# TritonDataCenter/node-cueball

Hardware: AMD Instinct MI355X
Metric: pool claims/sec (8-backend synthetic TCP set) (higher is better)
Workload: dtype n/a; 1 GPU; model=ConnectionPool claim/release (config: headline), global_batch=20000, seq_len=1, parallelism=1 worker processes (event loops), backends=8, spares=8, maximum=16, concurrency=16

## Files before the change

cueball_amd/_native/speed.cpp:

```cpp

#define PY_SSIZE_T_CLEAN
#include <Python.h>
#include <structmember.h>
#include <cmath>
#include <cstring>
#include <ctime>

#include "lathist.h"

#ifndef CUEBALL_HANDLE_HOOKS
#define CUEBALL_HANDLE_HOOKS 1
#endif
#ifndef CUEBALL_SLOT_HOOKS
#define CUEBALL_SLOT_HOOKS 1
#endif
#ifndef CUEBALL_LAZY_SCOPES
#define CUEBALL_LAZY_SCOPES 1
#endif
#ifndef CUEBALL_VECTORCALL
#define CUEBALL_VECTORCALL 1
#endif
#if !defined(Py_TPFLAGS_HAVE_VECTORCALL) && defined(_Py_TPFLAGS_HAVE_VECTORCALL)
#define Py_TPFLAGS_HAVE_VECTORCALL _Py_TPFLAGS_HAVE_VECTORCALL
#endif

namespace {

PyObject *s_stateChanged;
PyObject *s_listener;
PyObject *s_on;
PyObject *s_remove_listener;
PyObject *s_call_soon;
PyObject *s_call_later;
PyObject *s_cancel;
PyObject *s_state_prefix;
PyObject *s_dot;
PyObject *s_underscore;
PyObject *s_flush_name;
PyObject *s_internal;
PyObject *s_is_closed;

PyObject *g_get_loop;
PyObject *g_fsm_error;
PyObject *g_entry_name_cache;
PyObject *g_flush_batches;
PyObject *g_tracer;
PyObject *g_remove_desc;

static inline PyObject *
resolve_loop(PyObject *loop)
{
    if (loop != NULL && loop != Py_None) {
        Py_INCREF(loop);
        return loop;
    }
    return PyObject_CallOneArg(g_get_loop, Py_None);
}


typedef struct {
    PyObject_HEAD
    PyObject *ev_events;
    PyObject *ev_dict;
    PyObject *ev_weakrefs;
    unsigned long ev_gen;
    unsigned long ev_lk_gen;
    long ev_lk_cnt[4];
    Py_ssize_t ev_lk_len[4];
    int ev_lk_ok;
} Emitter;

extern PyTypeObject EmitterType;
extern PyTypeObject ConnErrCbType;
extern PyTypeObject KitCbType;

static inline int
listener_is_own_internal(PyObject *listener)
{
    PyTypeObject *tp = Py_TYPE(listener);
    return tp == &ConnErrCbType || tp == &KitCbType;
}

#define SMALL_LIST_KEEP 8

static inline int
list_append_keep(PyObject *ls, PyObject *item)
{
    PyListObject *l = (PyListObject *)ls;
    Py_ssize_t n = Py_SIZE(l);
    if (n < l->allocated) {
        Py_INCREF(item);
        l->ob_item[n] = item;
        Py_SET_SIZE(l, n + 1);
        return 0;
    }
    return PyList_Append(ls, item);
}

static inline int
list_remove_at_keep(PyObject *ls, Py_ssize_t i)
{
    PyListObject *l = (PyListObject *)ls;
    Py_ssize_t n = Py_SIZE(l);
    if (l->allocated > SMALL_LIST_KEEP)
        return PyList_SetSlice(ls, i, i + 1, NULL);
    PyObject *item = l->ob_item[i];
    for (Py_ssize_t j = i; j + 1 < n; j++)
        l->ob_item[j] = l->ob_item[j + 1];
    Py_SET_SIZE(l, n - 1);
    Py_DECREF(item);
    return 0;
}

int
Emitter_init(PyObject *self_, PyObject *args, PyObject *kwds)
{
    Emitter *self = (Emitter *)self_;
    (void)args; (void)kwds;
    if (self->ev_events == NULL) {
        self->ev_events = PyDict_New();
        if (self->ev_events == NULL)
            return -1;
    }
    return 0;
}

int
Emitter_traverse(PyObject *self_, visitproc visit, void *arg)
{
    Emitter *self = (Emitter *)self_;
    Py_VISIT(self->ev_events);
    Py_VISIT(self->ev_dict);
    return 0;
}

int
Emitter_clear_(PyObject *self_)
{
    Emitter *self = (Emitter *)self_;
    Py_CLEAR(self->ev_events);
    Py_CLEAR(self->ev_dict);
    return 0;
}

void
Emitter_dealloc(PyObject *self_)
{
    Emitter *self = (Emitter *)self_;
    PyTypeObject *tp = Py_TYPE(self_);
    PyObject_GC_UnTrack(self_);
    if (self->ev_weakrefs != NULL)
        PyObject_ClearWeakRefs(self_);
    Emitter_clear_(self_);
    tp->tp_free(self_);
}

PyObject *
emitter_add(Emitter *self, PyObject *event, PyObject *listener)
{
    if (self->ev_events == NULL) {
        self->ev_events = PyDict_New();
        if (self->ev_events == NULL)
            return NULL;
    }
    PyObject *ls = PyDict_GetItemWithError(self->ev_events, event);
    if (ls == NULL) {
        if (PyErr_Occurred())
            return NULL;
        ls = PyList_New(0);
        if (ls == NULL)
            return NULL;
        if (PyDict_SetItem(self->ev_events, event, ls) < 0) {
            Py_DECREF(ls);
// ... 670 lines not shown
PyObject *
Scope_dispose(PyObject *self_, PyObject *noargs)
{
    Scope *self = (Scope *)self_;
    (void)noargs;
    self->sc_active = 0;
    PyObject *regs[3 * SCOPE_INLINE_REGS];
    int nreg = self->sc_nreg;
    self->sc_nreg = 0;
    for (int i = 0; i < 3 * nreg; i++)
        regs[i] = self->sc_reg[i];
    PyObject *ls = self->sc_listeners;
    self->sc_listeners = NULL;
    int failed = 0;
    for (int i = 0; i < nreg; i++) {
        if (!failed &&
            scope_unregister(regs[3 * i], regs[3 * i + 1],
                             regs[3 * i + 2]) < 0)
            failed = 1;
        Py_DECREF(regs[3 * i]);
        Py_DECREF(regs[3 * i + 1]);
        Py_DECREF(regs[3 * i + 2]);
    }
    if (failed) {
        Py_XDECREF(ls);
        return NULL;
    }
    if (ls != NULL) {
        Py_ssize_t n = PyList_GET_SIZE(ls);
        for (Py_ssize_t i = 0; i + 2 < n; i += 3) {
            if (scope_unregister(PyList_GET_ITEM(ls, i),
                                 PyList_GET_ITEM(ls, i + 1),
                                 PyList_GET_ITEM(ls, i + 2)) < 0) {
                Py_DECREF(ls);
                return NULL;
            }
        }
        Py_DECREF(ls);
    }
    PyObject *ts = self->sc_timers;
    self->sc_timers = NULL;
    if (ts != NULL) {
        Py_ssize_t n = PyList_GET_SIZE(ts);
        for (Py_ssize_t i = 0; i < n; i++) {
            PyObject *r = PyObject_CallMethodObjArgs(
                PyList_GET_ITEM(ts, i), s_cancel, NULL);
            if (r == NULL) {
                Py_DECREF(ts);
                return NULL;
            }
            Py_DECREF(r);
        }
        Py_DECREF(ts);
    }
    Py_RETURN_NONE;
}

PyObject *
Scope_get_active(PyObject *self_, void *closure)
{
    (void)closure;
    return PyBool_FromLong(((Scope *)self_)->sc_active);
}

int
Scope_traverse(PyObject *self_, visitproc visit, void *arg)
{
    Scope *self = (Scope *)self_;
    Py_VISIT(self->sc_fsm);
    Py_VISIT(self->sc_listeners);
    Py_VISIT(self->sc_timers);
    for (int i = 0; i < 3 * self->sc_nreg; i++)
        Py_VISIT(self->sc_reg[i]);
    return 0;
}

int
Scope_clear_(PyObject *self_)
{
    Scope *self = (Scope *)self_;
    Py_CLEAR(self->sc_fsm);
    Py_CLEAR(self->sc_listeners);
    Py_CLEAR(self->sc_timers);
    int nreg = self->sc_nreg;
    self->sc_nreg = 0;
    for (int i = 0; i < 3 * nreg; i++)
        Py_CLEAR(self->sc_reg[i]);
    return 0;
}

void
Scope_dealloc(PyObject *self_)
{
    PyObject_GC_UnTrack(self_);
    Scope_clear_(self_);
    if (scope_freelist_n < SCOPE_FREELIST_MAX)
        scope_freelist[scope_freelist_n++] = (Scope *)self_;
    else
        PyObject_GC_Del(self_);
}

PyMethodDef Scope_methods[] = {
    {"on", (PyCFunction)(void (*)(void))Scope_on, METH_FASTCALL, NULL},
    {"timeout", (PyCFunction)(void (*)(void))Scope_timeout, METH_FASTCALL,
     NULL},
    {"interval", (PyCFunction)(void (*)(void))Scope_interval,
     METH_FASTCALL, NULL},
    {"immediate", Scope_immediate, METH_O, NULL},
    {"callback", Scope_callback, METH_O, NULL},
    {"valid_transitions", Scope_valid_transitions, METH_O, NULL},
    {"goto_state", Scope_goto_state, METH_O, NULL},
    {"_dispose", Scope_dispose, METH_NOARGS, NULL},
    {NULL, NULL, 0, NULL},
};

PyGetSetDef Scope_getset[] = {
    {(char *)"active", Scope_get_active, NULL, NULL, NULL},
    {NULL, NULL, NULL, NULL, NULL},
};

PyTypeObject ScopeType = {
    PyVarObject_HEAD_INIT(NULL, 0)
    "cueball_amd._speed.StateScope",
    sizeof(Scope),
    0,
    Scope_dealloc,
    0, 0, 0, 0, 0, 0, 0, 0, 0, 0, 0, 0, 0, 0,
    Py_TPFLAGS_DEFAULT | Py_TPFLAGS_HAVE_GC,
    "FSM state scope (native)",
    Scope_traverse,
    Scope_clear_,
    0, 0, 0, 0,
    Scope_methods,
    0,
    Scope_getset,
};


struct FSMOb {
    Emitter base;
    PyObject *f_loop;
    PyObject *f_state;
    PyObject *f_scope;
    PyObject *f_valid;
    PyObject *f_pending;
    PyObject **f_eq;
    Py_ssize_t f_eq_head, f_eq_len, f_eq_cap;
    PyObject *f_eq_inl[4];
    PyObject *f_hist[8];
    unsigned long f_hist_n;
    PyObject *f_flush_bound;
    PyObject *f_fastkit;
    PyObject *f_watchkit;
    int f_entering;
    int f_emit_scheduled;
};

int slotkit_maybe_entry(PyObject *kit_, FSMOb *fsm, PyObject *target);
int slotkit_smgr_hook(PyObject *kit_, PyObject *st, unsigned long serial);
unsigned long slotkit_slot_serial(PyObject *kit_);
int ch_emit_state_changed(FSMOb *self, PyObject *st);

static inline Scope *
fsm_need_scope(FSMOb *self)
{
    if (self->f_scope == NULL)
        self->f_scope = (PyObject *)scope_new((PyObject *)self);
    return (Scope *)self->f_scope;
}

extern PyObject *t_empty;
extern PyTypeObject CHType;
extern PyTypeObject CTType;
void ch_terminal_cleanup(FSMOb *self);

typedef PyObject *(*ch_entry_fn)(PyObject *, PyObject *);
ch_entry_fn ch_direct_entry(FSMOb *self, PyObject *target);

extern PyTypeObject FSMType;

PyObject *
fsm_get_loop_of(FSMOb *fsm)
{
    return fsm->f_loop;
}

#define FSM_EQ_INLINE 4
#define FSM_HISTORY 8

static void
fsm_eq_compact(FSMOb *f)
{
    if (f->f_eq_head == 0)
        return;
    Py_ssize_t n = f->f_eq_len - f->f_eq_head;
    memmove(f->f_eq, f->f_eq + f->f_eq_head, n * sizeof(PyObject *));
    f->f_eq_head = 0;
    f->f_eq_len = n;
}

static int
fsm_eq_push(FSMOb *f, PyObject *st)
{
    if (f->f_eq == NULL) {
        f->f_eq = f->f_eq_inl;
        f->f_eq_cap = FSM_EQ_INLINE;
        f->f_eq_head = f->f_eq_len = 0;
    }
    if (f->f_eq_len == f->f_eq_cap) {
        if (f->f_eq_head > 0) {
            fsm_eq_compact(f);
        } else {
            Py_ssize_t ncap = f->f_eq_cap * 2;
            PyObject **items;
            if (f->f_eq == f->f_eq_inl) {
                items = (PyObject **)PyMem_Malloc(
                    ncap * sizeof(PyObject *));
                if (items != NULL)
                    memcpy(items, f->f_eq_inl, sizeof(f->f_eq_inl));
            } else {
                items = (PyObject **)PyMem_Realloc(
                    f->f_eq, ncap * sizeof(PyObject *));
            }
            if (items == NULL) {
                PyErr_NoMemory();
                return -1;
            }
            f->f_eq = items;
            f->f_eq_cap = ncap;
        }
    }
    Py_INCREF(st);
    f->f_eq[f->f_eq_len++] = st;
    return 0;
}

static void
fsm_eq_clear(FSMOb *f)
{
    PyObject **items = f->f_eq;
    Py_ssize_t head = f->f_eq_head, len = f->f_eq_len;
    f->f_eq = NULL;
    f->f_eq_head = f->f_eq_len = f->f_eq_cap = 0;
    if (items == NULL)
        return;
    for (Py_ssize_t i = head; i < len; i++)
        Py_DECREF(items[i]);
    if (items != f->f_eq_inl)
        PyMem_Free(items);
}

int fsm_schedule_flush(FSMOb *self);

#define FSM_FLUSH_CAP 64

int
fsm_flush_core(FSMOb *self)
{
    self->f_emit_scheduled = 0;
    int n = 0;
    int is_handle = PyObject_TypeCheck((PyObject *)self, &CHType);
    while (self->f_eq_head < self->f_eq_len && n++ < FSM_FLUSH_CAP) {
        PyObject *st = self->f_eq[self->f_eq_head++];
        if (self->f_eq_head == self->f_eq_len)
            self->f_eq_head = self->f_eq_len = 0;
        int r;
        if (is_handle) {
            r = ch_emit_state_changed(self, st);
        } else {
            PyObject *eargs[2] = {s_stateChanged, st};
            unsigned long serial = self->f_watchkit == NULL ? 0
                : slotkit_slot_serial(self->f_watchkit);
            r = emitter_emit_core(&self->base, eargs[0], eargs + 1, 1);
            if (r >= 0 && serial != 0 && self->f_watchkit != NULL &&
                slotkit_smgr_hook(self->f_watchkit, st, serial) < 0)
                r = -1;
        }
        Py_DECREF(st);
        if (r < 0) {
            fsm_eq_compact(self);
            return -1;
        }
    }
    fsm_eq_compact(self);
    if (self->f_eq_len > 0 && !self->f_emit_scheduled)
        return fsm_schedule_flush(self);
    return 0;
}

PyObject *
FSM_flush_state_changed(PyObject *self_, PyObject *noargs)
{
    (void)noargs;
    if (fsm_flush_core((FSMOb *)self_) < 0)
        return NULL;
    Py_RETURN_NONE;
}

#define FLUSH_DRAIN_CAP 48

typedef struct {
    PyObject_HEAD
    PyObject *fb_loop;
    PyObject *fb_list;
    Py_ssize_t fb_pos;
    vectorcallfunc fb_vectorcall;
} FlushBatch;

extern PyTypeObject FlushBatchType;

static void
flushbatch_detach(FlushBatch *self)
{
    PyObject *cur = PyDict_GetItemWithError(g_flush_batches, self->fb_loop);
    if (cur == (PyObject *)self)
        (void)PyDict_DelItem(g_flush_batches, self->fb_loop);
    else if (cur == NULL)
        PyErr_Clear();
}

static PyObject *
flushbatch_run(PyObject *self_)
{
    FlushBatch *self = (FlushBatch *)self_;
    int rounds = 0;
    while (self->fb_pos < PyList_GET_SIZE(self->fb_list) &&
           rounds < FLUSH_DRAIN_CAP) {
        FSMOb *fsm = (FSMOb *)PyList_GET_ITEM(self->fb_list,
                                              self->fb_pos);
        self->fb_pos++;
        rounds++;
        if (fsm_flush_core(fsm) < 0) {
            for (Py_ssize_t i = self->fb_pos;
                 i < PyList_GET_SIZE(self->fb_list); i++) {
                FSMOb *f = (FSMOb *)PyList_GET_ITEM(self->fb_list, i);
                f->f_emit_scheduled = 0;
            }
            flushbatch_detach(self);
            return NULL;
        }
    }
    if (self->fb_pos < PyList_GET_SIZE(self->fb_list)) {
        if (PyList_SetSlice(self->fb_list, 0, self->fb_pos, NULL) < 0) {
            flushbatch_detach(self);
            return NULL;
        }
        self->fb_pos = 0;
        PyObject *h = PyObject_CallMethodObjArgs(
            self->fb_loop, s_call_soon, self_, NULL);
        if (h == NULL) {
            flushbatch_detach(self);
            return NULL;
        }
        Py_DECREF(h);
        Py_RETURN_NONE;
    }
    flushbatch_detach(self);
    Py_RETURN_NONE;
}

PyObject *
FlushBatch_call(PyObject *self_, PyObject *args, PyObject *kwds)
{
    (void)args; (void)kwds;
    return flushbatch_run(self_);
}

static PyObject *
FlushBatch_vectorcall(PyObject *self_, PyObject *const *args, size_t nargsf,
                      PyObject *kwnames)
{
    (void)args; (void)nargsf; (void)kwnames;
    return flushbatch_run(self_);
}

int
FlushBatch_traverse(PyObject *self_, visitproc visit, void *arg)
{
    FlushBatch *self = (FlushBatch *)self_;
    Py_VISIT(self->fb_loop);
    Py_VISIT(self->fb_list);
    return 0;
}

int
FlushBatch_clear_(PyObject *self_)
{
    FlushBatch *self = (FlushBatch *)self_;
    Py_CLEAR(self->fb_loop);
    Py_CLEAR(self->fb_list);
    return 0;
}

void
FlushBatch_dealloc(PyObject *self_)
{
    PyObject_GC_UnTrack(self_);
    FlushBatch_clear_(self_);
    PyObject_GC_Del(self_);
}

PyTypeObject FlushBatchType = {
    PyVarObject_HEAD_INIT(NULL, 0)
    "cueball_amd._speed._FlushBatch",
    sizeof(FlushBatch),
    0,
    FlushBatch_dealloc,
    0, 0, 0, 0, 0, 0, 0, 0, 0,
    FlushBatch_call,
    0, 0, 0, 0,
    Py_TPFLAGS_DEFAULT | Py_TPFLAGS_HAVE_GC,
    0,
    FlushBatch_traverse,
    FlushBatch_clear_,
};

int
fsm_queue_state_changed(FSMOb *self, PyObject *state)
{
    if (fsm_eq_push(self, state) < 0)
        return -1;
    return fsm_schedule_flush(self);
}

int
fsm_schedule_flush(FSMOb *self)
{
    if (self->f_emit_scheduled)
        return 0;
    self->f_emit_scheduled = 1;
    PyObject *batch = PyDict_GetItemWithError(g_flush_batches, self->f_loop);
    if (batch == NULL) {
        if (PyErr_Occurred())
            return -1;
        FlushBatch *fb = PyObject_GC_New(FlushBatch, &FlushBatchType);
        if (fb == NULL)
            return -1;
        Py_INCREF(self->f_loop);
        fb->fb_loop = self->f_loop;
        fb->fb_pos = 0;
        fb->fb_vectorcall = FlushBatch_vectorcall;
        fb->fb_list = PyList_New(0);
        PyObject_GC_Track((PyObject *)fb);
        if (fb->fb_list == NULL) {
            Py_DECREF(fb);
            return -1;
        }
        if (PyDict_SetItem(g_flush_batches, self->f_loop,
                           (PyObject *)fb) < 0) {
            Py_DECREF(fb);
            return -1;
        }
        PyObject *h = PyObject_CallMethodObjArgs(
            self->f_loop, s_call_soon, (PyObject *)fb, NULL);
        if (h == NULL) {
            Py_DECREF(fb);
            return -1;
        }
        Py_DECREF(h);
        batch = (PyObject *)fb;
        Py_DECREF(fb);
    }
    if (PyList_Append(((FlushBatch *)batch)->fb_list,
                      (PyObject *)self) < 0)
        return -1;
    return 0;
}

PyObject *
entry_attr_name(PyObject *state)
{
    PyObject *name = PyDict_GetItemWithError(g_entry_name_cache, state);
    if (name != NULL) {
        Py_INCREF(name);
        return name;
    }
    if (PyErr_Occurred())
        return NULL;
    PyObject *replaced = PyObject_CallMethod(state, "replace", "OO",
                                             s_dot, s_underscore);
    if (replaced == NULL)
        return NULL;
    name = PyUnicode_Concat(s_state_prefix, replaced);
    Py_DECREF(replaced);
    if (name == NULL)
        return NULL;
    PyUnicode_InternInPlace(&name);
    if (PyDict_SetItem(g_entry_name_cache, state, name) < 0) {
        Py_DECREF(name);
        return NULL;
    }
    return name;
}

int
check_valid(FSMOb *self, PyObject *from, PyObject *state)
{
    if (self->f_valid == NULL)
        return 0;
    int c = PySequence_Contains(self->f_valid, state);
    if (c < 0)
        return -1;
    if (!c) {
        PyErr_Format(g_fsm_error,
                     "%s: invalid transition %R -> %R (valid: %R)",
                     Py_TYPE(self)->tp_name,
                     from ? from : Py_None, state, self->f_valid);
        return -1;
    }
    return 0;
}

int
fsm_enter_loop(FSMOb *self, PyObject *state)
{
    PyObject *next_state = state;
    Py_INCREF(next_state);
    while (next_state != NULL) {
        PyObject *target = next_state;
        next_state = NULL;
        if (self->f_scope != NULL) {
            PyObject *old = self->f_scope;
            self->f_scope = NULL;
            PyObject *r = Scope_dispose(old, NULL);
            Py_DECREF(old);
            if (r == NULL) {
                Py_DECREF(target);
                return -1;
            }
            Py_DECREF(r);
        }
        Py_CLEAR(self->f_valid);
        Py_INCREF(target);
        Py_XSETREF(self->f_state, target);
        Py_INCREF(target);
        Py_XSETREF(self->f_hist[self->f_hist_n % FSM_HISTORY], target);
        self->f_hist_n++;
#if !CUEBALL_LAZY_SCOPES
        if (fsm_need_scope(self) == NULL) {
            Py_DECREF(target);
            return -1;
        }
#endif

        if (g_tracer != NULL && g_tracer != Py_None) {
            PyObject *targs[2] = {(PyObject *)self, target};
            PyObject *tr = PyObject_Vectorcall(g_tracer, targs, 2, NULL);
            if (tr == NULL) {
                Py_DECREF(target);
                return -1;
            }
            Py_DECREF(tr);
        }

        int handled = 0;
        if (self->f_fastkit != NULL) {
            self->f_entering = 1;
            handled = slotkit_maybe_entry(self->f_fastkit, self, target);
            self->f_entering = 0;
            if (handled < 0) {
                Py_DECREF(target);
                return -1;
            }
        }
        PyObject *r;
        ch_entry_fn direct = handled ? NULL : ch_direct_entry(self, target);
        if (handled) {
            r = Py_None;
            Py_INCREF(r);
        } else if (direct != NULL) {
            self->f_entering = 1;
            r = direct((PyObject *)self, NULL);
            self->f_entering = 0;
        } else {
            PyObject *attr = entry_attr_name(target);
            if (attr == NULL) {
                Py_DECREF(target);
                return -1;
            }
            PyObject *entry = PyObject_GetAttr((PyObject *)self, attr);
            Py_DECREF(attr);
            if (entry == NULL) {
                PyErr_Clear();
                PyErr_Format(g_fsm_error,
                             "%s has no state-entry function for %R",
                             Py_TYPE(self)->tp_name, target);
                Py_DECREF(target);
                return -1;
            }
            PyObject *scope = (PyObject *)fsm_need_scope(self);
            if (scope == NULL) {
                Py_DECREF(entry);
                Py_DECREF(target);
                return -1;
            }
            Py_INCREF(scope);
            self->f_entering = 1;
            r = PyObject_CallOneArg(entry, scope);
            Py_DECREF(entry);
            Py_DECREF(scope);
            self->f_entering = 0;
        }
        PyObject *pend = self->f_pending;
        self->f_pending = NULL;
        if (r == NULL) {
            Py_XDECREF(pend);
            Py_DECREF(target);
            return -1;
        }
        Py_DECREF(r);
        if (fsm_queue_state_changed(self, target) < 0) {
            Py_XDECREF(pend);
            Py_DECREF(target);
            return -1;
        }
        if (pend != NULL) {
            if (check_valid(self, target, pend) < 0) {
                Py_DECREF(pend);
                Py_DECREF(target);
                return -1;
            }
            next_state = pend;
        }
        Py_DECREF(target);
    }
    if (self->f_valid == t_empty &&
        PyObject_TypeCheck((PyObject *)self, &CHType))
        ch_terminal_cleanup(self);
    return 0;
}

int
fsm_goto_state(FSMOb *self, PyObject *state)
{
    if (check_valid(self, self->f_state, state) < 0)
        return -1;
    if (self->f_entering) {
        if (self->f_pending != NULL) {
            int eq = PyObject_RichCompareBool(self->f_pending, state, Py_EQ);
            if (eq < 0)
                return -1;
            if (!eq) {
                PyErr_Format(g_fsm_error,
                             "%s: conflicting deferred transitions %R and "
                             "%R from %R", Py_TYPE(self)->tp_name,
                             self->f_pending, state,
                             self->f_state ? self->f_state : Py_None);
                return -1;
            }
            return 0;
        }
        Py_INCREF(state);
        self->f_pending = state;
        return 0;
    }
    return fsm_enter_loop(self, state);
}

int
FSM_init(PyObject *self_, PyObject *args, PyObject *kwds)
{
    FSMOb *self = (FSMOb *)self_;
    PyObject *initial = NULL, *loop = Py_None;
    static const char *kwlist[] = {"initial_state", "loop", NULL};
    if (!PyArg_ParseTupleAndKeywords(args, kwds, "U|O",
                                     const_cast<char **>(kwlist),
                                     &initial, &loop))
        return -1;
    if (Emitter_init(self_, NULL, NULL) < 0)
        return -1;
    PyObject *resolved = resolve_loop(loop);
    if (resolved == NULL)
        return -1;
    Py_XSETREF(self->f_loop, resolved);
    Py_CLEAR(self->f_state);
    Py_CLEAR(self->f_valid);
    Py_CLEAR(self->f_pending);
    self->f_entering = 0;
    return fsm_goto_state(self, initial);
}

PyObject *
FSM_get_state(PyObject *self_, PyObject *noargs)
{
    FSMOb *self = (FSMOb *)self_;
    (void)noargs;
    if (self->f_state == NULL) {
        PyErr_SetString(g_fsm_error, "FSM has no state yet");
        return NULL;
    }
    Py_INCREF(self->f_state);
    return self->f_state;
}

PyObject *
FSM_is_in_state(PyObject *self_, PyObject *state)
{
    FSMOb *self = (FSMOb *)self_;
    if (self->f_state == NULL)
        Py_RETURN_FALSE;
    int eq = PyUnicode_Compare(self->f_state, state);
    if (eq == -1 && PyErr_Occurred())
        return NULL;
    if (eq == 0)
        Py_RETURN_TRUE;
    Py_ssize_t sl = PyUnicode_GET_LENGTH(state);
    Py_ssize_t cl = PyUnicode_GET_LENGTH(self->f_state);
    if (cl > sl) {
        int m = PyUnicode_Tailmatch(self->f_state, state, 0, sl, -1);
        if (m < 0)
            return NULL;
        if (m && PyUnicode_ReadChar(self->f_state, sl) == '.')
            Py_RETURN_TRUE;
    }
    Py_RETURN_FALSE;
}

PyObject *
FSM_get_state_history(PyObject *self_, PyObject *noargs)
{
    FSMOb *self = (FSMOb *)self_;
    (void)noargs;
    Py_ssize_t count = self->f_hist_n < FSM_HISTORY
        ? (Py_ssize_t)self->f_hist_n : FSM_HISTORY;
    PyObject *out = PyList_New(count);
    if (out == NULL)
        return NULL;
    unsigned long first = self->f_hist_n - (unsigned long)count;
    for (Py_ssize_t i = 0; i < count; i++) {
        PyObject *st = self->f_hist[(first + (unsigned long)i) %
                                    FSM_HISTORY];
        Py_INCREF(st);
        PyList_SET_ITEM(out, i, st);
    }
    return out;
}

PyObject *
FSM_goto_state_py(PyObject *self_, PyObject *state)
{
    if (!PyUnicode_Check(state)) {
        PyErr_SetString(PyExc_TypeError, "state must be a str");
        return NULL;
    }
    if (fsm_goto_state((FSMOb *)self_, state) < 0)
        return NULL;
    Py_RETURN_NONE;
}

PyObject *
FSM_get__fsm_state(PyObject *self_, void *closure)
{
    FSMOb *self = (FSMOb *)self_;
    (void)closure;
    if (self->f_state == NULL)
        Py_RETURN_NONE;
    Py_INCREF(self->f_state);
    return self->f_state;
}

PyObject *
FSM_get__fsm_valid(PyObject *self_, void *closure)
{
    FSMOb *self = (FSMOb *)self_;
    (void)closure;
    if (self->f_valid == NULL)
        Py_RETURN_NONE;
    Py_INCREF(self->f_valid);
    return self->f_valid;
}

int
FSM_set__fsm_valid(PyObject *self_, PyObject *value, void *closure)
{
    FSMOb *self = (FSMOb *)self_;
    (void)closure;
    if (value == NULL || value == Py_None) {
        Py_CLEAR(self->f_valid);
        return 0;
    }
// ... 22 lines not shown
} IntervalOb;

extern PyTypeObject IntervalType;

PyObject *
Interval_call(PyObject *self_, PyObject *args, PyObject *kwds)
{
    IntervalOb *self = (IntervalOb *)self_;
    (void)args; (void)kwds;
    if (self->iv_stopped || !((Scope *)self->iv_scope)->sc_active)
        Py_RETURN_NONE;
    PyObject *r = PyObject_CallNoArgs(self->iv_cb);
    if (r == NULL)
        return NULL;
    Py_DECREF(r);
    if (!self->iv_stopped && ((Scope *)self->iv_scope)->sc_active) {
        FSMOb *fsm = (FSMOb *)((Scope *)self->iv_scope)->sc_fsm;
        PyObject *h = PyObject_CallMethodObjArgs(
            fsm->f_loop, s_call_later, self->iv_secs, self_, NULL);
        if (h == NULL)
            return NULL;
        Py_XSETREF(self->iv_handle, h);
    }
    Py_RETURN_NONE;
}

PyObject *
Interval_cancel(PyObject *self_, PyObject *noargs)
{
    IntervalOb *self = (IntervalOb *)self_;
    (void)noargs;
    self->iv_stopped = 1;
    if (self->iv_handle != NULL) {
        PyObject *r = PyObject_CallMethodObjArgs(self->iv_handle, s_cancel,
                                                 NULL);
        if (r == NULL)
            return NULL;
        Py_DECREF(r);
    }
    Py_RETURN_NONE;
}

int
Interval_traverse(PyObject *self_, visitproc visit, void *arg)
{
    IntervalOb *self = (IntervalOb *)self_;
    Py_VISIT(self->iv_scope);
    Py_VISIT(self->iv_cb);
    Py_VISIT(self->iv_handle);
    return 0;
}

int
Interval_clear_(PyObject *self_)
{
    IntervalOb *self = (IntervalOb *)self_;
    Py_CLEAR(self->iv_scope);
    Py_CLEAR(self->iv_cb);
    Py_CLEAR(self->iv_secs);
    Py_CLEAR(self->iv_handle);
    return 0;
}

void
Interval_dealloc(PyObject *self_)
{
    PyObject_GC_UnTrack(self_);
    Interval_clear_(self_);
    PyObject_GC_Del(self_);
}

PyMethodDef Interval_methods[] = {
    {"cancel", Interval_cancel, METH_NOARGS, NULL},
    {NULL, NULL, 0, NULL},
};

PyTypeObject IntervalType = {
    PyVarObject_HEAD_INIT(NULL, 0)
    "cueball_amd._speed._Interval",
    sizeof(IntervalOb),
    0,
    Interval_dealloc,
    0, 0, 0, 0, 0, 0, 0, 0, 0,
    Interval_call,
    0, 0, 0, 0,
    Py_TPFLAGS_DEFAULT | Py_TPFLAGS_HAVE_GC,
    0,
    Interval_traverse,
    Interval_clear_,
    0, 0, 0, 0,
    Interval_methods,
};

PyObject *
Scope_interval(PyObject *self_, PyObject *const *args, Py_ssize_t nargs)
{
    Scope *self = (Scope *)self_;
    if (nargs != 2) {
        PyErr_SetString(PyExc_TypeError, "S.interval(ms, cb)");
        return NULL;
    }
    if (scope_check_active(self, "S.interval()") < 0)
        return NULL;
    double ms = PyFloat_AsDouble(args[0]);
    if (ms == -1.0 && PyErr_Occurred())
        return NULL;
    IntervalOb *iv = PyObject_GC_New(IntervalOb, &IntervalType);
    if (iv == NULL)
        return NULL;
    Py_INCREF(self_);
    iv->iv_scope = self_;
    Py_INCREF(args[1]);
    iv->iv_cb = args[1];
    iv->iv_secs = PyFloat_FromDouble(ms / 1000.0);
    iv->iv_handle = NULL;
    iv->iv_stopped = 0;
    PyObject_GC_Track((PyObject *)iv);
    if (iv->iv_secs == NULL) {
        Py_DECREF(iv);
        return NULL;
    }
    FSMOb *fsm = (FSMOb *)self->sc_fsm;
    PyObject *h = PyObject_CallMethodObjArgs(fsm->f_loop, s_call_later,
                                             iv->iv_secs, (PyObject *)iv,
                                             NULL);
    if (h == NULL) {
        Py_DECREF(iv);
        return NULL;
    }
    iv->iv_handle = h;
    int rc = scope_add_timer(self, (PyObject *)iv);
    Py_DECREF(iv);
    if (rc < 0)
        return NULL;
    Py_RETURN_NONE;
}

int
FSM_traverse(PyObject *self_, visitproc visit, void *arg)
{
    FSMOb *self = (FSMOb *)self_;
    Py_VISIT(self->f_loop);
    Py_VISIT(self->f_state);
    Py_VISIT(self->f_scope);
    Py_VISIT(self->f_valid);
    Py_VISIT(self->f_pending);
    for (Py_ssize_t i = self->f_eq_head; i < self->f_eq_len; i++)
        Py_VISIT(self->f_eq[i]);
    for (int i = 0; i < FSM_HISTORY; i++)
        Py_VISIT(self->f_hist[i]);
    Py_VISIT(self->f_flush_bound);
    Py_VISIT(self->f_fastkit);
    Py_VISIT(self->f_watchkit);
    return Emitter_traverse(self_, visit, arg);
}

int
FSM_clear_(PyObject *self_)
{
    FSMOb *self = (FSMOb *)self_;
    Py_CLEAR(self->f_loop);
    Py_CLEAR(self->f_state);
    Py_CLEAR(self->f_scope);
    Py_CLEAR(self->f_valid);
    Py_CLEAR(self->f_pending);
    fsm_eq_clear(self);
    for (int i = 0; i < FSM_HISTORY; i++)
        Py_CLEAR(self->f_hist[i]);
    self->f_hist_n = 0;
    Py_CLEAR(self->f_flush_bound);
    Py_CLEAR(self->f_fastkit);
    Py_CLEAR(self->f_watchkit);
    return Emitter_clear_(self_);
}

void
FSM_dealloc(PyObject *self_)
{
    FSMOb *self = (FSMOb *)self_;
    PyTypeObject *tp = Py_TYPE(self_);
    PyObject_GC_UnTrack(self_);
    if (self->base.ev_weakrefs != NULL)
        PyObject_ClearWeakRefs(self_);
    FSM_clear_(self_);
    tp->tp_free(self_);
}

static PyObject *
FSM_set_fast_kit(PyObject *self_, PyObject *kit)
{
    FSMOb *self = (FSMOb *)self_;
    if (kit == Py_None) {
        Py_CLEAR(self->f_fastkit);
    } else {
        Py_INCREF(kit);
        Py_XSETREF(self->f_fastkit, kit);
    }
    Py_RETURN_NONE;
}

PyMethodDef FSM_methods[] = {
    {"get_state", FSM_get_state, METH_NOARGS, NULL},
    {"is_in_state", FSM_is_in_state, METH_O, NULL},
    {"get_state_history", FSM_get_state_history, METH_NOARGS, NULL},
    {"goto_state", FSM_goto_state_py, METH_O, NULL},
    {"_flush_state_changed", FSM_flush_state_changed, METH_NOARGS, NULL},
    {"_set_fast_kit", FSM_set_fast_kit, METH_O, NULL},
    {NULL, NULL, 0, NULL},
};

PyMemberDef FSM_members[] = {
    {(char *)"_loop", T_OBJECT, offsetof(FSMOb, f_loop), READONLY, NULL},
    {NULL, 0, 0, 0, NULL},
};

PyGetSetDef FSM_getset[] = {
    {(char *)"_fsm_state", FSM_get__fsm_state, NULL, NULL, NULL},
    {(char *)"_fsm_valid", FSM_get__fsm_valid, FSM_set__fsm_valid, NULL,
     NULL},
    {NULL, NULL, NULL, NULL, NULL},
};

PyTypeObject FSMType = {
    PyVarObject_HEAD_INIT(NULL, 0)
    "cueball_amd._speed.FSM",
    sizeof(FSMOb),
    0,
    FSM_dealloc,
    0, 0, 0, 0, 0, 0, 0, 0, 0, 0, 0, 0, 0, 0,
    Py_TPFLAGS_DEFAULT | Py_TPFLAGS_BASETYPE | Py_TPFLAGS_HAVE_GC,
    "Moore machine (native)",
    FSM_traverse,
    FSM_clear_,
    0, 0, 0, 0,
    FSM_methods,
    FSM_members,
    FSM_getset,
    &EmitterType,
    0, 0, 0,
    0,
    FSM_init,
    0,
    PyType_GenericNew,
};


typedef struct {
    FSMOb base;
    PyObject *sl_handle;
    PyObject *sl_prev_handle;
    PyObject *sl_wanted;
    PyObject *sl_monitor;
    PyObject *sl_idleq_node;
    PyObject *sl_initq_node;
} SlotOb;

extern PyTypeObject SlotBaseType;

static inline int
slot_field_set(PyObject **field)
{
    return *field != NULL && *field != Py_None;
}

static inline int
slot_field_true(PyObject **field)
{
    PyObject *v = *field;
    if (v == Py_True)
        return 1;
    if (v == NULL || v == Py_False || v == Py_None)
        return 0;
    Py_INCREF(v);
    int t = PyObject_IsTrue(v);
    Py_DECREF(v);
    return t;
}

static inline void
slot_field_store(PyObject **field, PyObject *value)
{
    Py_XINCREF(value);
    Py_XSETREF(*field, value);
}

int
Slot_traverse(PyObject *self_, visitproc visit, void *arg)
{
    SlotOb *self = (SlotOb *)self_;
    Py_VISIT(self->sl_handle);
    Py_VISIT(self->sl_prev_handle);
    Py_VISIT(self->sl_wanted);
    Py_VISIT(self->sl_monitor);
    Py_VISIT(self->sl_idleq_node);
    Py_VISIT(self->sl_initq_node);
    return FSM_traverse(self_, visit, arg);
}

int
Slot_clear_(PyObject *self_)
{
    SlotOb *self = (SlotOb *)self_;
    Py_CLEAR(self->sl_handle);
    Py_CLEAR(self->sl_prev_handle);
    Py_CLEAR(self->sl_wanted);
    Py_CLEAR(self->sl_monitor);
    Py_CLEAR(self->sl_idleq_node);
    Py_CLEAR(self->sl_initq_node);
    return FSM_clear_(self_);
}

void
Slot_dealloc(PyObject *self_)
{
    SlotOb *self = (SlotOb *)self_;
    PyTypeObject *tp = Py_TYPE(self_);
    PyObject_GC_UnTrack(self_);
    if (self->base.base.ev_weakrefs != NULL)
        PyObject_ClearWeakRefs(self_);
    Slot_clear_(self_);
    tp->tp_free(self_);
}

PyMemberDef Slot_members[] = {
    {(char *)"csf_handle", T_OBJECT, offsetof(SlotOb, sl_handle), 0, NULL},
    {(char *)"csf_prev_handle", T_OBJECT, offsetof(SlotOb, sl_prev_handle),
     0, NULL},
    {(char *)"csf_wanted", T_OBJECT, offsetof(SlotOb, sl_wanted), 0, NULL},
    {(char *)"csf_monitor", T_OBJECT, offsetof(SlotOb, sl_monitor), 0,
     NULL},
    {(char *)"p_idleq_node", T_OBJECT, offsetof(SlotOb, sl_idleq_node), 0,
     NULL},
    {(char *)"p_initq_node", T_OBJECT, offsetof(SlotOb, sl_initq_node), 0,
     NULL},
    {NULL, 0, 0, 0, NULL},
};

PyTypeObject SlotBaseType = {
    PyVarObject_HEAD_INIT(NULL, 0)
    "cueball_amd._speed.SlotBase",
    sizeof(SlotOb),
    0,
    Slot_dealloc,
    0, 0, 0, 0, 0, 0, 0, 0, 0, 0, 0, 0, 0, 0,
    Py_TPFLAGS_DEFAULT | Py_TPFLAGS_BASETYPE | Py_TPFLAGS_HAVE_GC,
    "connection slot FSM (native fields)",
    Slot_traverse,
    Slot_clear_,
    0, 0, 0, 0,
    0,
    Slot_members,
    0,
    &FSMType,
    0, 0, 0,
    0,
    0,
    0,
    PyType_GenericNew,
};



typedef struct {
    PyObject_HEAD
    lathist::Hist h;
} LatHistOb;

extern PyTypeObject LatHistType;

static PyObject *
LatHist_new(PyTypeObject *type, PyObject *args, PyObject *kwds)
{
// ... 228 lines not shown
{
#if defined(CLOCK_MONOTONIC)
    if (pl->pl_direct) {
        struct timespec ts;
        if (clock_gettime(CLOCK_MONOTONIC, &ts) == 0)
            return (double)ts.tv_sec * 1000.0 + (double)ts.tv_nsec * 1e-6;
    }
#endif
    PyObject *t = PyObject_CallMethodObjArgs(pl->pl_loop, s_time, NULL);
    if (t == NULL) {
        *err = 1;
        return 0.0;
    }
    double secs = PyFloat_AsDouble(t);
    Py_DECREF(t);
    if (secs == -1.0 && PyErr_Occurred()) {
        *err = 1;
        return 0.0;
    }
    return secs * 1000.0;
}

static PyObject *
PoolLat_new(PyTypeObject *type, PyObject *args, PyObject *kwds)
{
    PyObject *loop;
    int direct = 0;
    static const char *kwlist[] = {"loop", "direct", NULL};
    if (!PyArg_ParseTupleAndKeywords(args, kwds, "O|p",
                                     const_cast<char **>(kwlist),
                                     &loop, &direct))
        return NULL;
    PoolLatOb *self = PyObject_GC_New(PoolLatOb, type);
    if (self == NULL)
        return NULL;
    Py_INCREF(loop);
    self->pl_loop = loop;
#if defined(CLOCK_MONOTONIC)
    self->pl_direct = direct;
#else
    self->pl_direct = 0;
#endif
    self->pl_wait = (LatHistOb *)LatHist_new(&LatHistType, NULL, NULL);
    self->pl_hold = (LatHistOb *)LatHist_new(&LatHistType, NULL, NULL);
    self->pl_connect = (LatHistOb *)LatHist_new(&LatHistType, NULL, NULL);
    PyObject_GC_Track((PyObject *)self);
    if (self->pl_wait == NULL || self->pl_hold == NULL ||
        self->pl_connect == NULL) {
        Py_DECREF((PyObject *)self);
        return NULL;
    }
    return (PyObject *)self;
}

static int
PoolLat_traverse(PyObject *self_, visitproc visit, void *arg)
{
    Py_VISIT(((PoolLatOb *)self_)->pl_loop);
    return 0;
}

static int
PoolLat_clear_(PyObject *self_)
{
    Py_CLEAR(((PoolLatOb *)self_)->pl_loop);
    return 0;
}

static void
PoolLat_dealloc(PyObject *self_)
{
    PoolLatOb *self = (PoolLatOb *)self_;
    PyObject_GC_UnTrack(self_);
    Py_CLEAR(self->pl_loop);
    Py_CLEAR(self->pl_wait);
    Py_CLEAR(self->pl_hold);
    Py_CLEAR(self->pl_connect);
    PyObject_GC_Del(self_);
}

static PyMemberDef PoolLat_members[] = {
    {(char *)"loop", T_OBJECT, offsetof(PoolLatOb, pl_loop), READONLY,
     NULL},
    {(char *)"wait", T_OBJECT, offsetof(PoolLatOb, pl_wait), READONLY,
     NULL},
    {(char *)"hold", T_OBJECT, offsetof(PoolLatOb, pl_hold), READONLY,
     NULL},
    {(char *)"connect", T_OBJECT, offsetof(PoolLatOb, pl_connect),
     READONLY, NULL},
    {(char *)"direct", T_INT, offsetof(PoolLatOb, pl_direct), READONLY,
     NULL},
    {NULL, 0, 0, 0, NULL},
};

PyTypeObject PoolLatType = {
    PyVarObject_HEAD_INIT(NULL, 0)
    "cueball_amd._speed.PoolLatency",
    sizeof(PoolLatOb),
};

static void
latency_types_init(void)
{
    LatHistType.tp_flags = Py_TPFLAGS_DEFAULT;
    LatHistType.tp_methods = LatHist_methods;
    LatHistType.tp_getset = LatHist_getset;
    LatHistType.tp_new = LatHist_new;

    PoolLatType.tp_dealloc = PoolLat_dealloc;
    PoolLatType.tp_flags = Py_TPFLAGS_DEFAULT | Py_TPFLAGS_HAVE_GC;
    PoolLatType.tp_traverse = PoolLat_traverse;
    PoolLatType.tp_clear = PoolLat_clear_;
    PoolLatType.tp_members = PoolLat_members;
    PoolLatType.tp_new = PoolLat_new;
}


PyObject *g_err_claim_timeout;
PyObject *g_err_cueball;
PyObject *g_err_misused;
PyObject *g_capture_stack;

PyObject *s_claim;
PyObject *s_warn;
PyObject *s_incr;
PyObject *s_claim_timeout_evt;
PyObject *s_is_in_state;
PyObject *s_time;
PyObject *s_waiting, *s_claiming, *s_claimed, *s_released, *s_closed,
         *s_cancelled, *s_failed, *s_idle, *s_error_evt;
PyObject *t_waiting_valid;
PyObject *t_claiming_valid;
PyObject *t_claimed_valid;
PyObject *t_empty;
PyObject *s_leak_events[4];

int g_stack_on = 1;
PyObject *g_stack_placeholder;
PyObject *g_inf;

static inline PyObject *
capture_stack(void)
{
    if (!g_stack_on && g_stack_placeholder != NULL) {
        Py_INCREF(g_stack_placeholder);
        return g_stack_placeholder;
    }
    return PyObject_CallNoArgs(g_capture_stack);
}

extern PyObject *s_busy_st;
PyObject *slotkit_conn_err_cb(PyObject *slot, PyObject *handle);

typedef struct {
    FSMOb base;
    PyObject *chb_pool;
    PyObject *chb_claim_stack;
    PyObject *chb_callback;
    PyObject *chb_log;
    PyObject *chb_slot;
    PyObject *chb_release_stack;
    PyObject *chb_connection;
    PyObject *chb_last_error;
    PyObject *chb_waiter_node;
    PoolLatOb *chb_lat;
    double chb_claim_timeout;
    double chb_started;
    double chb_claimed_at;
    long chb_pre[4];
    int chb_have_pre;
    int chb_throw_error;
    int chb_cancelled;
    int chb_leak_check;
    int chb_pinger;
    int chb_lat_open;
    PyObject *chb_idleq, *chb_waiters, *chb_initq;
    int chb_tk_on;
    int chb_tk_err_on_empty;
    unsigned long chb_bk_serial;
    Py_ssize_t chb_bk_pos;
} CHOb;

extern PyTypeObject CHType;

long
c_count_listeners(PyObject *emitter, PyObject *event)
{
    if (!PyObject_TypeCheck(emitter, &EmitterType))
        return -2;
    Emitter *em = (Emitter *)emitter;
    if (em->ev_events == NULL)
        return 0;
    PyObject *ls = PyDict_GetItemWithError(em->ev_events, event);
    if (ls == NULL)
        return PyErr_Occurred() ? -1 : 0;
    long count = 0;
    Py_ssize_t n = PyList_GET_SIZE(ls);
    for (Py_ssize_t i = 0; i < n; i++) {
        PyObject *h = PyList_GET_ITEM(ls, i);
        if (!PyCallable_Check(h))
            continue;
        PyObject *marker = NULL;
        if (_PyObject_LookupAttr(h, s_internal, &marker) < 0)
            return -1;
        if (marker != NULL) {
            int truthy = PyObject_IsTrue(marker);
            Py_DECREF(marker);
            if (truthy < 0)
                return -1;
            if (truthy)
                continue;
        }
        PyObject *target = NULL;
        if (Py_TYPE(h) == &OnceWrapperType) {
            target = ((OnceWrapper *)h)->ow_listener;
            Py_INCREF(target);
        } else if (_PyObject_LookupAttr(h, s_listener, &target) < 0) {
            return -1;
        }
        if (target != NULL && target != h) {
            if (_PyObject_LookupAttr(target, s_internal, &marker) < 0) {
                Py_DECREF(target);
                return -1;
            }
            if (marker != NULL) {
                int truthy = PyObject_IsTrue(marker);
                Py_DECREF(marker);
                if (truthy < 0) {
                    Py_DECREF(target);
                    return -1;
                }
                if (truthy) {
                    Py_DECREF(target);
                    continue;
                }
            }
        }
        Py_XDECREF(target);
        count++;
    }
    return count;
}

int
emitter_leak_counts(PyObject *conn, long out[4])
{
    if (!PyObject_TypeCheck(conn, &EmitterType))
        return -2;
    Emitter *em = (Emitter *)conn;
    Py_ssize_t lens[4];
    for (int i = 0; i < 4; i++) {
        PyObject *ls = NULL;
        if (em->ev_events != NULL) {
            ls = PyDict_GetItemWithError(em->ev_events, s_leak_events[i]);
            if (ls == NULL && PyErr_Occurred())
                return -1;
        }
        lens[i] = (ls != NULL && PyList_Check(ls)) ? PyList_GET_SIZE(ls)
                                                   : -1;
    }
    if (em->ev_lk_ok && em->ev_lk_gen == em->ev_gen &&
        memcmp(lens, em->ev_lk_len, sizeof(lens)) == 0) {
        memcpy(out, em->ev_lk_cnt, sizeof(em->ev_lk_cnt));
        return 0;
    }
    unsigned long gen = em->ev_gen;
    for (int i = 0; i < 4; i++) {
        long c = c_count_listeners(conn, s_leak_events[i]);
        if (c < 0)
            return -1;
        out[i] = c;
    }
    em->ev_lk_ok = 0;
    if (gen == em->ev_gen) {
        memcpy(em->ev_lk_cnt, out, sizeof(em->ev_lk_cnt));
        memcpy(em->ev_lk_len, lens, sizeof(lens));
        em->ev_lk_gen = gen;
        em->ev_lk_ok = 1;
    }
    return 0;
}

typedef struct {
    PyObject_HEAD
    PyObject *ce_handle;
} ConnErrCb;

extern PyTypeObject ConnErrCbType;

PyObject *conn_err_fire(CHOb *h, PyObject *err);

PyObject *
ConnErrCb_call(PyObject *self_, PyObject *args, PyObject *kwds)
{
    CHOb *h = (CHOb *)((ConnErrCb *)self_)->ce_handle;
    (void)kwds;
    PyObject *err = (PyTuple_GET_SIZE(args) > 0)
        ? PyTuple_GET_ITEM(args, 0) : Py_None;
    return conn_err_fire(h, err);
}

PyObject *
conn_err_fire(CHOb *h, PyObject *err)
{
    long cnt = c_count_listeners(h->chb_connection, s_error_evt);
    if (cnt == -1)
        return NULL;
    if (cnt == 0 && h->chb_throw_error) {
        if (PyExceptionInstance_Check(err)) {
            PyErr_SetObject((PyObject *)Py_TYPE(err), err);
        } else {
            PyErr_SetObject(PyExc_RuntimeError, err);
        }
        return NULL;
    }
    PyObject *msg = PyUnicode_FromString(
        "connection emitted error while claimed");
    if (msg == NULL)
        return NULL;
    PyObject *r = PyObject_CallMethodObjArgs(h->chb_log, s_warn, msg,
                                             NULL);
    Py_DECREF(msg);
    if (r == NULL)
        return NULL;
    Py_DECREF(r);
    PyObject *evt = PyUnicode_FromString("error-while-claimed");
    if (evt == NULL)
        return NULL;
    r = PyObject_CallMethodObjArgs(h->chb_pool, s_incr, evt, NULL);
    Py_DECREF(evt);
    if (r == NULL)
        return NULL;
    Py_DECREF(r);
    Py_RETURN_NONE;
}

int
ConnErrCb_traverse(PyObject *self_, visitproc visit, void *arg)
{
    Py_VISIT(((ConnErrCb *)self_)->ce_handle);
    return 0;
}

int
ConnErrCb_clear_(PyObject *self_)
{
    Py_CLEAR(((ConnErrCb *)self_)->ce_handle);
    return 0;
}

void
ConnErrCb_dealloc(PyObject *self_)
{
    PyObject_GC_UnTrack(self_);
    ConnErrCb_clear_(self_);
    PyObject_GC_Del(self_);
}

PyObject *
ConnErrCb_get_internal(PyObject *self_, void *closure)
{
    (void)self_; (void)closure;
    Py_RETURN_TRUE;
}

PyGetSetDef ConnErrCb_getset[] = {
    {(char *)"_cueball_internal", ConnErrCb_get_internal, NULL, NULL, NULL},
    {NULL, NULL, NULL, NULL, NULL},
};

PyTypeObject ConnErrCbType = {
    PyVarObject_HEAD_INIT(NULL, 0)
    "cueball_amd._speed._ConnErrCb",
    sizeof(ConnErrCb),
    0,
    ConnErrCb_dealloc,
    0, 0, 0, 0, 0, 0, 0, 0, 0,
    ConnErrCb_call,
    0, 0, 0, 0,
    Py_TPFLAGS_DEFAULT | Py_TPFLAGS_HAVE_GC,
    0,
    ConnErrCb_traverse,
    ConnErrCb_clear_,
    0, 0, 0, 0, 0, 0,
    ConnErrCb_getset,
};

typedef struct {
    PyObject_HEAD
    PyObject *fc_handle;
} FailCb;

extern PyTypeObject FailCbType;

PyObject *
FailCb_call(PyObject *self_, PyObject *args, PyObject *kwds)
{
    CHOb *h = (CHOb *)((FailCb *)self_)->fc_handle;
    (void)args; (void)kwds;
    PyObject *err = h->chb_last_error ? h->chb_last_error : Py_None;
    return PyObject_CallOneArg(h->chb_callback, err);
}

int
FailCb_traverse(PyObject *self_, visitproc visit, void *arg)
{
    Py_VISIT(((FailCb *)self_)->fc_handle);
    return 0;
}

int
FailCb_clear_(PyObject *self_)
{
    Py_CLEAR(((FailCb *)self_)->fc_handle);
    return 0;
}

void
FailCb_dealloc(PyObject *self_)
{
    PyObject_GC_UnTrack(self_);
    FailCb_clear_(self_);
    PyObject_GC_Del(self_);
}

PyTypeObject FailCbType = {
    PyVarObject_HEAD_INIT(NULL, 0)
    "cueball_amd._speed._FailCb",
    sizeof(FailCb),
    0,
    FailCb_dealloc,
    0, 0, 0, 0, 0, 0, 0, 0, 0,
    FailCb_call,
    0, 0, 0, 0,
    Py_TPFLAGS_DEFAULT | Py_TPFLAGS_HAVE_GC,
    0,
    FailCb_traverse,
    FailCb_clear_,
};


int
ch_state_is(CHOb *self, PyObject *state)
{
    return self->base.f_state == state ||
        (self->base.f_state != NULL &&
         PyUnicode_Compare(self->base.f_state, state) == 0);
}

PyObject *
ch_err_format(PyObject *cls, const char *msg)
{
    PyErr_SetString(cls, msg);
    return NULL;
}


PyObject *
CH_try_(PyObject *self_, PyObject *slot)
{
    CHOb *self = (CHOb *)self_;
    if (!ch_state_is(self, s_waiting))
        return ch_err_format(g_fsm_error,
            "ClaimHandle.try_ only in \"waiting\"");
    PyObject *r = PyObject_CallMethodObjArgs(slot, s_is_in_state, s_idle,
                                             NULL);
    if (r == NULL)
        return NULL;
    int idle = PyObject_IsTrue(r);
    Py_DECREF(r);
    if (!idle)
        return ch_err_format(g_fsm_error,
            "ClaimHandle.try_ needs an idle slot");
// ... 50 lines not shown
ch_do_claim_timeout(CHOb *self)
{
    PyObject *err = PyObject_CallOneArg(g_err_claim_timeout,
                                        self->chb_pool);
    if (err == NULL)
        return -1;
    Py_XSETREF(self->chb_last_error, err);
    PyObject *r = PyObject_CallMethodObjArgs(
        self->chb_pool, s_incr, s_claim_timeout_evt, NULL);
    if (r == NULL)
        return -1;
    Py_DECREF(r);
    return fsm_goto_state(&self->base, s_failed);
}

PyObject *
CH_timeout(PyObject *self_, PyObject *noargs)
{
    CHOb *self = (CHOb *)self_;
    (void)noargs;
    if (!ch_state_is(self, s_waiting))
        return ch_err_format(g_fsm_error, "timeout only in waiting");
    if (ch_do_claim_timeout(self) < 0)
        return NULL;
    Py_RETURN_NONE;
}

PyObject *
CH__on_claim_timeout(PyObject *self_, PyObject *noargs)
{
    return CH_timeout(self_, noargs);
}

PyObject *
CH_fail(PyObject *self_, PyObject *err)
{
    CHOb *self = (CHOb *)self_;
    if (ch_state_is(self, s_waiting)) {
        Py_INCREF(err);
        Py_XSETREF(self->chb_last_error, err);
        if (fsm_goto_state(&self->base, s_failed) < 0)
            return NULL;
    }
    Py_RETURN_NONE;
}

int
ch_relinquish(CHOb *self, PyObject *target_state)
{
    if (!ch_state_is(self, s_claimed)) {
        if (ch_state_is(self, s_released) || ch_state_is(self, s_closed)) {
            PyObject *by = NULL;
            PyObject *stack = self->chb_release_stack;
            if (stack != NULL && PyList_Check(stack) &&
                PyList_GET_SIZE(stack) >= 1) {
                by = PyList_GET_ITEM(stack, PyList_GET_SIZE(stack) - 1);
            }
            PyObject *msg = PyUnicode_FromFormat(
                "Connection not claimed by this handle, released by %S",
                by ? by : Py_None);
            if (msg == NULL)
                return -1;
            PyObject *err = PyObject_CallOneArg(g_err_cueball, msg);
            Py_DECREF(msg);
            if (err == NULL)
                return -1;
            PyErr_SetObject(g_err_cueball, err);
            Py_DECREF(err);
            return -1;
        }
        PyObject *msg = PyUnicode_FromFormat(
            "ClaimHandle.release() called while in state \"%S\"",
            self->base.f_state ? self->base.f_state : Py_None);
        if (msg == NULL)
            return -1;
        PyErr_SetObject(g_err_cueball, msg);
        Py_DECREF(msg);
        return -1;
    }
    PyObject *stack = capture_stack();
    if (stack == NULL)
        return -1;
    Py_XSETREF(self->chb_release_stack, stack);
    return fsm_goto_state(&self->base, target_state);
}

PyObject *
CH_release(PyObject *self_, PyObject *noargs)
{
    (void)noargs;
    if (ch_relinquish((CHOb *)self_, s_released) < 0)
        return NULL;
    Py_RETURN_NONE;
}

PyObject *
CH_close(PyObject *self_, PyObject *noargs)
{
    (void)noargs;
    if (ch_relinquish((CHOb *)self_, s_closed) < 0)
        return NULL;
    Py_RETURN_NONE;
}

PyObject *
CH_disable_release_leak_check(PyObject *self_, PyObject *noargs)
{
    (void)noargs;
    ((CHOb *)self_)->chb_leak_check = 0;
    Py_RETURN_NONE;
}


PyObject *
CH_state_waiting(PyObject *self_, PyObject *scope)
{
    CHOb *self = (CHOb *)self_;
    Py_INCREF(t_waiting_valid);
    Py_XSETREF(self->base.f_valid, t_waiting_valid);
    Py_CLEAR(self->chb_slot);
    self->chb_bk_serial = 0;
    if (isfinite(self->chb_claim_timeout)) {
        if (scope == NULL)
            scope = (PyObject *)fsm_need_scope(&self->base);
        if (scope == NULL)
            return NULL;
        PyObject *ms = PyFloat_FromDouble(self->chb_claim_timeout);
        if (ms == NULL)
            return NULL;
        PyObject *cb = PyObject_GetAttrString(self_, "_on_claim_timeout");
        if (cb == NULL) {
            Py_DECREF(ms);
            return NULL;
        }
        PyObject *args[2] = {ms, cb};
        PyObject *r = Scope_timeout(scope, args, 2);
        Py_DECREF(ms);
        Py_DECREF(cb);
        if (r == NULL)
            return NULL;
        Py_DECREF(r);
    }
    Py_RETURN_NONE;
}

PyObject *
CH_state_claiming(PyObject *self_, PyObject *scope)
{
    CHOb *self = (CHOb *)self_;
    (void)scope;
    Py_INCREF(t_claiming_valid);
    Py_XSETREF(self->base.f_valid, t_claiming_valid);
    PyObject *slot = self->chb_slot;
    if (slot != NULL && PyObject_TypeCheck(slot, &SlotBaseType) &&
        ((FSMOb *)slot)->f_fastkit != NULL) {
        FSMOb *sf = (FSMOb *)slot;
        PyObject *fs = sf->f_state;
        if (!(fs == s_idle ||
              (fs != NULL && PyUnicode_Compare(fs, s_idle) == 0))) {
            PyErr_SetString(g_fsm_error, "claim only in idle");
            return NULL;
        }
        if (slot_field_set(&((SlotOb *)slot)->sl_handle)) {
            PyErr_SetString(g_fsm_error, "slot already has a handle");
            return NULL;
        }
        slot_field_store(&((SlotOb *)slot)->sl_handle, self_);
        if (fsm_goto_state(sf, s_busy_st) < 0)
            return NULL;
        Py_RETURN_NONE;
    }
    PyObject *r = PyObject_CallMethodObjArgs(slot, s_claim,
                                             self_, NULL);
    if (r == NULL)
        return NULL;
    Py_DECREF(r);
    Py_RETURN_NONE;
}

PyObject *
CH_state_claimed(PyObject *self_, PyObject *scope)
{
    CHOb *self = (CHOb *)self_;
    Py_INCREF(t_claimed_valid);
    Py_XSETREF(self->base.f_valid, t_claimed_valid);

    if (self->chb_cancelled) {
        if (fsm_goto_state(&self->base, s_released) < 0)
            return NULL;
        Py_RETURN_NONE;
    }

    PyObject *conn = self->chb_connection;
    int lk = emitter_leak_counts(conn, self->chb_pre);
    if (lk == -1)
        return NULL;
    if (lk == -2)
        self->chb_pre[0] = self->chb_pre[1] = self->chb_pre[2] =
            self->chb_pre[3] = 0;
    self->chb_have_pre = 1;

    PyObject *ec = slotkit_conn_err_cb(self->chb_slot, self_);
    if (ec != NULL) {
        Py_INCREF(ec);
    } else {
        ConnErrCb *nec = PyObject_GC_New(ConnErrCb, &ConnErrCbType);
        if (nec == NULL)
            return NULL;
        Py_INCREF(self_);
        nec->ce_handle = self_;
        PyObject_GC_Track((PyObject *)nec);
        ec = (PyObject *)nec;
    }
    if (scope == NULL)
        scope = (PyObject *)fsm_need_scope(&self->base);
    if (scope == NULL) {
        Py_DECREF(ec);
        return NULL;
    }
    PyObject *args[3] = {conn, s_error_evt, ec};
    PyObject *r = Scope_on(scope, args, 3);
    Py_DECREF(ec);
    if (r == NULL)
        return NULL;
    Py_DECREF(r);

    if (self->chb_lat != NULL && !self->chb_pinger) {
        int err = 0;
        double now = poollat_now_ms(self->chb_lat, &err);
        if (err)
            return NULL;
        self->chb_lat->pl_wait->h.record_ms(now - self->chb_started);
        self->chb_claimed_at = now;
        self->chb_lat_open = 1;
    }

    PyObject *cbargs[3] = {Py_None, self_, conn};
    r = PyObject_Vectorcall(self->chb_callback, cbargs, 3, NULL);
    if (r == NULL)
        return NULL;
    Py_DECREF(r);
    Py_RETURN_NONE;
}

static int
ch_record_hold(CHOb *self)
{
    if (!self->chb_lat_open)
        return 0;
    self->chb_lat_open = 0;
    int err = 0;
    double now = poollat_now_ms(self->chb_lat, &err);
    if (err)
        return -1;
    self->chb_lat->pl_hold->h.record_ms(now - self->chb_claimed_at);
    return 0;
}

PyObject *
CH_state_released(PyObject *self_, PyObject *scope)
{
    CHOb *self = (CHOb *)self_;
    (void)scope;
    Py_INCREF(t_empty);
    Py_XSETREF(self->base.f_valid, t_empty);
    if (ch_record_hold(self) < 0)
        return NULL;
    if (!self->chb_leak_check || !self->chb_have_pre)
        Py_RETURN_NONE;
    PyObject *conn = self->chb_connection;
    long after[4];
    int lk = emitter_leak_counts(conn, after);
    if (lk == -1)
        return NULL;
    if (lk == -2)
        Py_RETURN_NONE;
    for (int i = 0; i < 4; i++) {
        long c = after[i];
        if (c > self->chb_pre[i]) {
            PyObject *msg = PyUnicode_FromFormat(
                "connection claimer looks like it leaked event handlers "
                "(event=%S before=%ld after=%ld)",
                s_leak_events[i], self->chb_pre[i], c);
            if (msg == NULL)
                return NULL;
            PyObject *r = PyObject_CallMethodObjArgs(self->chb_log, s_warn,
                                                     msg, NULL);
            Py_DECREF(msg);
            if (r == NULL)
                return NULL;
            Py_DECREF(r);
        }
    }
    Py_RETURN_NONE;
}

PyObject *
CH_state_closed(PyObject *self_, PyObject *scope)
{
    CHOb *self = (CHOb *)self_;
    (void)scope;
    Py_INCREF(t_empty);
    Py_XSETREF(self->base.f_valid, t_empty);
    if (ch_record_hold(self) < 0)
        return NULL;
    Py_RETURN_NONE;
}

PyObject *
CH_state_cancelled(PyObject *self_, PyObject *scope)
{
    CHOb *self = (CHOb *)self_;
    (void)scope;
    Py_INCREF(t_empty);
    Py_XSETREF(self->base.f_valid, t_empty);
    Py_RETURN_NONE;
}

PyObject *
CH_state_failed(PyObject *self_, PyObject *scope)
{
    CHOb *self = (CHOb *)self_;
    (void)scope;
    Py_INCREF(t_empty);
    Py_XSETREF(self->base.f_valid, t_empty);
    FailCb *fc = PyObject_GC_New(FailCb, &FailCbType);
    if (fc == NULL)
        return NULL;
    Py_INCREF(self_);
    fc->fc_handle = self_;
    PyObject_GC_Track((PyObject *)fc);
    PyObject *h = PyObject_CallMethodObjArgs(self->base.f_loop,
                                             s_call_soon,
                                             (PyObject *)fc, NULL);
    Py_DECREF(fc);
    if (h == NULL)
        return NULL;
    Py_DECREF(h);
    Py_RETURN_NONE;
}


PyObject *
CH_get_misused(PyObject *self_, void *closure)
{
    (void)self_; (void)closure;
    PyObject *err = PyObject_CallNoArgs(g_err_misused);
    if (err == NULL)
        return NULL;
    PyErr_SetObject(g_err_misused, err);
    Py_DECREF(err);
    return NULL;
}

PyObject *
CH_on(PyObject *self_, PyObject *const *args, Py_ssize_t nargs)
{
    if (nargs >= 1 && PyUnicode_Check(args[0])) {
        if (PyUnicode_CompareWithASCIIString(args[0], "readable") == 0 ||
            PyUnicode_CompareWithASCIIString(args[0], "close") == 0) {
            PyObject *err = PyObject_CallNoArgs(g_err_misused);
            if (err == NULL)
                return NULL;
            PyErr_SetObject(g_err_misused, err);
            Py_DECREF(err);
            return NULL;
        }
    }
    return Emitter_on(self_, args, nargs);
}

PyObject *
CH_once(PyObject *self_, PyObject *const *args, Py_ssize_t nargs)
{
    if (nargs >= 1 && PyUnicode_Check(args[0])) {
        if (PyUnicode_CompareWithASCIIString(args[0], "readable") == 0 ||
            PyUnicode_CompareWithASCIIString(args[0], "close") == 0) {
            PyObject *err = PyObject_CallNoArgs(g_err_misused);
            if (err == NULL)
                return NULL;
            PyErr_SetObject(g_err_misused, err);
            Py_DECREF(err);
            return NULL;
        }
    }
    return Emitter_once(self_, args, nargs);
}

PyObject *
CH_remove_listener(PyObject *self_, PyObject *const *args, Py_ssize_t nargs)
{
    CHOb *self = (CHOb *)self_;
    if (nargs != 2) {
        PyErr_SetString(PyExc_TypeError, "remove_listener(event, listener)");
        return NULL;
    }
    Py_ssize_t at;
    if (emitter_remove_core(&self->base.base, args, &at) < 0)
        return NULL;
    if (at >= 0 && at < self->chb_bk_pos &&
        (args[0] == s_stateChanged ||
         (PyUnicode_Check(args[0]) &&
          PyUnicode_Compare(args[0], s_stateChanged) == 0)))
        self->chb_bk_pos--;
    Py_RETURN_NONE;
}

PyObject *
CH_remove_all_listeners(PyObject *self_, PyObject *const *args,
                        Py_ssize_t nargs)
{
    ((CHOb *)self_)->chb_bk_pos = 0;
    return Emitter_remove_all_listeners(self_, args, nargs);
}


int
CH_traverse(PyObject *self_, visitproc visit, void *arg)
{
    CHOb *self = (CHOb *)self_;
    Py_VISIT(self->chb_pool);
    Py_VISIT(self->chb_claim_stack);
    Py_VISIT(self->chb_callback);
    Py_VISIT(self->chb_log);
    Py_VISIT(self->chb_slot);
    Py_VISIT(self->chb_release_stack);
    Py_VISIT(self->chb_connection);
    Py_VISIT(self->chb_last_error);
    Py_VISIT(self->chb_waiter_node);
    Py_VISIT((PyObject *)self->chb_lat);
    Py_VISIT(self->chb_idleq);
    Py_VISIT(self->chb_waiters);
    Py_VISIT(self->chb_initq);
    return FSM_traverse(self_, visit, arg);
}

int
CH_clear_(PyObject *self_)
{
    CHOb *self = (CHOb *)self_;
    Py_CLEAR(self->chb_pool);
    Py_CLEAR(self->chb_claim_stack);
    Py_CLEAR(self->chb_callback);
    Py_CLEAR(self->chb_log);
    Py_CLEAR(self->chb_slot);
    Py_CLEAR(self->chb_release_stack);
    Py_CLEAR(self->chb_connection);
    Py_CLEAR(self->chb_last_error);
    Py_CLEAR(self->chb_waiter_node);
    Py_CLEAR(self->chb_lat);
    Py_CLEAR(self->chb_idleq);
    Py_CLEAR(self->chb_waiters);
    Py_CLEAR(self->chb_initq);
    return FSM_clear_(self_);
}

void
CH_dealloc(PyObject *self_)
{
    CHOb *self = (CHOb *)self_;
    PyTypeObject *tp = Py_TYPE(self_);
    PyObject_GC_UnTrack(self_);
    if (self->base.base.ev_weakrefs != NULL)
        PyObject_ClearWeakRefs(self_);
    CH_clear_(self_);
    tp->tp_free(self_);
}

PyObject *
CH__setup(PyObject *self_, PyObject *const *args, Py_ssize_t nargs)
{
    CHOb *self = (CHOb *)self_;
    if (nargs != 7) {
        PyErr_SetString(PyExc_TypeError,
            "_setup(pool, stack, cb, log, timeout, throw_error, loop)");
        return NULL;
    }
    Py_INCREF(args[0]); Py_XSETREF(self->chb_pool, args[0]);
    Py_INCREF(args[1]); Py_XSETREF(self->chb_claim_stack, args[1]);
    Py_INCREF(args[2]); Py_XSETREF(self->chb_callback, args[2]);
    Py_INCREF(args[3]); Py_XSETREF(self->chb_log, args[3]);
    self->chb_claim_timeout = PyFloat_AsDouble(args[4]);
    if (self->chb_claim_timeout == -1.0 && PyErr_Occurred())
        return NULL;
    int throw_error = PyObject_IsTrue(args[5]);
    if (throw_error < 0)
        return NULL;
    self->chb_throw_error = throw_error;
    self->chb_cancelled = 0;
    self->chb_leak_check = 1;
    self->chb_pinger = 0;
    self->chb_have_pre = 0;
    self->chb_lat_open = 0;
    PyObject *lat = NULL;
    if (_PyObject_LookupAttr(args[0], s_p_lat, &lat) < 0)
        return NULL;
    if (lat != NULL && Py_TYPE(lat) != &PoolLatType)
        Py_CLEAR(lat);
    Py_XSETREF(self->chb_lat, (PoolLatOb *)lat);

    PyObject *resolved = resolve_loop(args[6]);
    if (resolved == NULL)
        return NULL;
    Py_XSETREF(self->base.f_loop, resolved);
#if !CUEBALL_HANDLE_HOOKS
    if (Emitter_init(self_, NULL, NULL) < 0)
        return NULL;
#endif
    self->chb_tk_on = 0;
    self->chb_bk_serial = 0;
    if (fsm_goto_state(&self->base, s_waiting) < 0)
        return NULL;
    if (self->chb_lat != NULL && self->chb_lat->pl_direct &&
        self->chb_lat->pl_loop == self->base.f_loop) {
        int err = 0;
        self->chb_started = poollat_now_ms(self->chb_lat, &err);
        if (err)
            return NULL;
        Py_RETURN_NONE;
    }
    PyObject *t = PyObject_CallMethodObjArgs(self->base.f_loop, s_time,
                                             NULL);
    if (t == NULL)
        return NULL;
    double secs = PyFloat_AsDouble(t);
    Py_DECREF(t);
    if (secs == -1.0 && PyErr_Occurred())
        return NULL;
    self->chb_started = secs * 1000.0;
    Py_RETURN_NONE;
}

PyMethodDef CH_methods[] = {
    {"_setup", (PyCFunction)(void (*)(void))CH__setup, METH_FASTCALL, NULL},
    {"try_", CH_try_, METH_O, NULL},
    {"accept", CH_accept, METH_O, NULL},
    {"reject", CH_reject, METH_NOARGS, NULL},
    {"cancel", CH_cancel, METH_NOARGS, NULL},
    {"timeout", CH_timeout, METH_NOARGS, NULL},
    {"_on_claim_timeout", CH__on_claim_timeout, METH_NOARGS, NULL},
    {"fail", CH_fail, METH_O, NULL},
    {"release", CH_release, METH_NOARGS, NULL},
    {"close", CH_close, METH_NOARGS, NULL},
    {"disable_release_leak_check", CH_disable_release_leak_check,
     METH_NOARGS, NULL},
    {"on", (PyCFunction)(void (*)(void))CH_on, METH_FASTCALL, NULL},
    {"once", (PyCFunction)(void (*)(void))CH_once, METH_FASTCALL, NULL},
    {"remove_listener", (PyCFunction)(void (*)(void))CH_remove_listener,
     METH_FASTCALL, NULL},
    {"remove_all_listeners",
     (PyCFunction)(void (*)(void))CH_remove_all_listeners, METH_FASTCALL,
     NULL},
    {"state_waiting", CH_state_waiting, METH_O, NULL},
    {"state_claiming", CH_state_claiming, METH_O, NULL},
    {"state_claimed", CH_state_claimed, METH_O, NULL},
    {"state_released", CH_state_released, METH_O, NULL},
    {"state_closed", CH_state_closed, METH_O, NULL},
    {"state_cancelled", CH_state_cancelled, METH_O, NULL},
    {"state_failed", CH_state_failed, METH_O, NULL},
    {NULL, NULL, 0, NULL},
};

PyMemberDef CH_members[] = {
    {(char *)"ch_pool", T_OBJECT, offsetof(CHOb, chb_pool), 0, NULL},
    {(char *)"ch_claim_stack", T_OBJECT, offsetof(CHOb, chb_claim_stack),
     0, NULL},
    {(char *)"ch_callback", T_OBJECT, offsetof(CHOb, chb_callback), 0,
     NULL},
    {(char *)"ch_log", T_OBJECT, offsetof(CHOb, chb_log), 0, NULL},
    {(char *)"ch_slot", T_OBJECT, offsetof(CHOb, chb_slot), 0, NULL},
    {(char *)"ch_release_stack", T_OBJECT,
     offsetof(CHOb, chb_release_stack), 0, NULL},
    {(char *)"ch_connection", T_OBJECT, offsetof(CHOb, chb_connection),
     0, NULL},
    {(char *)"ch_last_error", T_OBJECT, offsetof(CHOb, chb_last_error),
     0, NULL},
    {(char *)"ch_waiter_node", T_OBJECT, offsetof(CHOb, chb_waiter_node),
     0, NULL},
    {(char *)"ch_claim_timeout", T_DOUBLE,
     offsetof(CHOb, chb_claim_timeout), 0, NULL},
    {(char *)"ch_started", T_DOUBLE, offsetof(CHOb, chb_started), 0, NULL},
    {(char *)"ch_cancelled", T_INT, offsetof(CHOb, chb_cancelled), 0,
     NULL},
    {(char *)"ch_throw_error", T_INT, offsetof(CHOb, chb_throw_error), 0,
     NULL},
    {(char *)"ch_do_release_leak_check", T_INT,
     offsetof(CHOb, chb_leak_check), 0, NULL},
    {(char *)"ch_pinger", T_INT, offsetof(CHOb, chb_pinger), 0, NULL},
    {NULL, 0, 0, 0, NULL},
};

PyGetSetDef CH_getset[] = {
    {(char *)"readable", CH_get_misused, NULL, NULL, NULL},
    {(char *)"writable", CH_get_misused, NULL, NULL, NULL},
    {NULL, NULL, NULL, NULL, NULL},
};

PyTypeObject CHType = {
    PyVarObject_HEAD_INIT(NULL, 0)
    "cueball_amd._speed.ClaimHandleBase",
    sizeof(CHOb),
    0,
    CH_dealloc,
    0, 0, 0, 0, 0, 0, 0, 0, 0, 0, 0, 0, 0, 0,
    Py_TPFLAGS_DEFAULT | Py_TPFLAGS_BASETYPE | Py_TPFLAGS_HAVE_GC,
    "pool claim handle (native core)",
    CH_traverse,
    CH_clear_,
    0, 0, 0, 0,
    CH_methods,
    CH_members,
    CH_getset,
    &FSMType,
    0, 0, 0,
    0,
    0,
    0,
    PyType_GenericNew,
};

struct ChEntry {
    PyObject **ce_state;
    const char *ce_method;
    ch_entry_fn ce_fn;
    PyObject *ce_attr;
    PyObject *ce_desc;
};

ChEntry ch_entries[] = {
    {&s_waiting, "state_waiting", CH_state_waiting, NULL, NULL},
    {&s_claiming, "state_claiming", CH_state_claiming, NULL, NULL},
    {&s_claimed, "state_claimed", CH_state_claimed, NULL, NULL},
    {&s_released, "state_released", CH_state_released, NULL, NULL},
    {&s_closed, "state_closed", CH_state_closed, NULL, NULL},
    {&s_cancelled, "state_cancelled", CH_state_cancelled, NULL, NULL},
    {&s_failed, "state_failed", CH_state_failed, NULL, NULL},
};
const int ch_n_entries = (int)(sizeof(ch_entries) / sizeof(ch_entries[0]));

int
ch_entries_init(void)
{
    for (int i = 0; i < ch_n_entries; i++) {
        ChEntry *e = &ch_entries[i];
        e->ce_attr = PyUnicode_InternFromString(e->ce_method);
        if (e->ce_attr == NULL)
            return -1;
        e->ce_desc = PyDict_GetItemWithError(CHType.tp_dict, e->ce_attr);
        if (e->ce_desc == NULL)
            return -1;
        Py_INCREF(e->ce_desc);
    }
    return 0;
}

ch_entry_fn
ch_direct_entry(FSMOb *self, PyObject *target)
{
    PyTypeObject *tp = Py_TYPE(self);
    if (!PyType_IsSubtype(tp, &CHType))
        return NULL;
    for (int i = 0; i < ch_n_entries; i++) {
        ChEntry *e = &ch_entries[i];
        if (*e->ce_state != target)
            continue;
        if (_PyType_Lookup(tp, e->ce_attr) != e->ce_desc)
            return NULL;
        PyObject *d = self->base.ev_dict;
        if (d != NULL && PyDict_GET_SIZE(d) > 0 &&
            PyDict_GetItemWithError(d, e->ce_attr) != NULL)
            return NULL;
        if (PyErr_Occurred())
            PyErr_Clear();
        return e->ce_fn;
    }
    return NULL;
}

PyObject *
speed_set_stack_traces(PyObject *mod, PyObject *const *args,
                       Py_ssize_t nargs)
{
    (void)mod;
    if (nargs != 2) {
        PyErr_SetString(PyExc_TypeError,
                        "_set_stack_traces(enabled, placeholder)");
        return NULL;
    }
    int on = PyObject_IsTrue(args[0]);
    if (on < 0)
        return NULL;
    g_stack_on = on;
    Py_INCREF(args[1]);
    Py_XSETREF(g_stack_placeholder, args[1]);
    Py_RETURN_NONE;
}

PyObject *
speed_set_claim_helpers(PyObject *mod, PyObject *const *args,
                        Py_ssize_t nargs)
{
    (void)mod;
    if (nargs != 4) {
        PyErr_SetString(PyExc_TypeError,
            "_set_claim_helpers(ClaimTimeoutError, CueballError, "
            "ClaimHandleMisusedError, capture_stack)");
        return NULL;
    }
    Py_INCREF(args[0]); Py_XSETREF(g_err_claim_timeout, args[0]);
    Py_INCREF(args[1]); Py_XSETREF(g_err_cueball, args[1]);
    Py_INCREF(args[2]); Py_XSETREF(g_err_misused, args[2]);
    Py_INCREF(args[3]); Py_XSETREF(g_capture_stack, args[3]);
    Py_RETURN_NONE;
}


PyObject *
speed_set_helpers(PyObject *mod, PyObject *const *args, Py_ssize_t nargs)
{
    (void)mod;
    if (nargs != 2) {
        PyErr_SetString(PyExc_TypeError, "_set_helpers(get_loop, FSMError)");
        return NULL;
    }
    Py_INCREF(args[0]);
    Py_XSETREF(g_get_loop, args[0]);
    Py_INCREF(args[1]);
    Py_XSETREF(g_fsm_error, args[1]);
    Py_RETURN_NONE;
}

PyObject *
speed_count_listeners(PyObject *mod, PyObject *const *args,
                      Py_ssize_t nargs)
{
    (void)mod;
    if (nargs != 2) {
        PyErr_SetString(PyExc_TypeError, "count_listeners(emitter, event)");
        return NULL;
    }
    if (!PyObject_TypeCheck(args[0], &EmitterType)) {
        PyErr_SetString(PyExc_TypeError, "emitter must be an EventEmitter");
        return NULL;
    }
    Emitter *em = (Emitter *)args[0];
    if (em->ev_events == NULL)
        return PyLong_FromLong(0);
    PyObject *ls = PyDict_GetItemWithError(em->ev_events, args[1]);
    if (ls == NULL)
        return PyErr_Occurred() ? NULL : PyLong_FromLong(0);
    Py_ssize_t n = PyList_GET_SIZE(ls);
    long count = 0;
    for (Py_ssize_t i = 0; i < n; i++) {
        PyObject *h = PyList_GET_ITEM(ls, i);
        if (!PyCallable_Check(h))
            continue;
        PyObject *marker = NULL;
        if (_PyObject_LookupAttr(h, s_internal, &marker) < 0)
            return NULL;
        if (marker != NULL) {
            int truthy = PyObject_IsTrue(marker);
            Py_DECREF(marker);
            if (truthy < 0)
                return NULL;
            if (truthy)
                continue;
        }
        PyObject *target = NULL;
        if (Py_TYPE(h) == &OnceWrapperType) {
            target = ((OnceWrapper *)h)->ow_listener;
            Py_INCREF(target);
        } else if (_PyObject_LookupAttr(h, s_listener, &target) < 0) {
            return NULL;
        }
        if (target != NULL && target != h) {
            if (_PyObject_LookupAttr(target, s_internal, &marker) < 0) {
                Py_DECREF(target);
                return NULL;
            }
            if (marker != NULL) {
                int truthy = PyObject_IsTrue(marker);
                Py_DECREF(marker);
                if (truthy < 0) {
                    Py_DECREF(target);
                    return NULL;
                }
                if (truthy) {
                    Py_DECREF(target);
                    continue;
                }
            }
        }
        Py_XDECREF(target);
        count++;
    }
    return PyLong_FromLong(count);
}


typedef struct NQueue NQueue;

typedef struct QNode {
    PyObject_HEAD
    PyObject *value;
    struct QNode *q_next;
    struct QNode *q_prev;
    NQueue *q_queue;
} QNode;

struct NQueue {
    PyObject_HEAD
    QNode *q_first;
    QNode *q_last;
    Py_ssize_t q_len;
// ... 201 lines not shown
        n = nxt;
    }
    Py_RETURN_NONE;
}

static PyObject *
NQueue_iter(PyObject *self_)
{
    NQueue *q = (NQueue *)self_;
    PyObject *list = PyList_New(0);
    if (list == NULL)
        return NULL;
    for (QNode *n = q->q_first; n != NULL; n = n->q_next) {
        if (PyList_Append(list, n->value ? n->value : Py_None) < 0) {
            Py_DECREF(list);
            return NULL;
        }
    }
    PyObject *it = PyObject_GetIter(list);
    Py_DECREF(list);
    return it;
}

static Py_ssize_t
NQueue_len(PyObject *self_)
{
    return ((NQueue *)self_)->q_len;
}

static PyObject *
NQueue_get_len(PyObject *self_, void *closure)
{
    (void)closure;
    return PyLong_FromSsize_t(((NQueue *)self_)->q_len);
}

static int
NQueue_traverse(PyObject *self_, visitproc visit, void *arg)
{
    NQueue *q = (NQueue *)self_;
    for (QNode *n = q->q_first; n != NULL; n = n->q_next)
        Py_VISIT((PyObject *)n);
    return 0;
}

static int
NQueue_clear_(PyObject *self_)
{
    NQueue *q = (NQueue *)self_;
    while (q->q_first != NULL) {
        QNode *n = q->q_first;
        Py_INCREF((PyObject *)n);
        nqueue_unlink(q, n);
        Py_DECREF((PyObject *)n);
    }
    return 0;
}

static void
NQueue_dealloc(PyObject *self_)
{
    PyObject_GC_UnTrack(self_);
    NQueue_clear_(self_);
    PyObject_GC_Del(self_);
}

static PyObject *
NQueue_new(PyTypeObject *type, PyObject *args, PyObject *kwds)
{
    (void)args; (void)kwds;
    NQueue *q = PyObject_GC_New(NQueue, type);
    if (q == NULL)
        return NULL;
    q->q_first = NULL;
    q->q_last = NULL;
    q->q_len = 0;
    PyObject_GC_Track((PyObject *)q);
    return (PyObject *)q;
}

static PyMethodDef NQueue_methods[] = {
    {"push", NQueue_push, METH_O, NULL},
    {"shift", NQueue_shift, METH_NOARGS, NULL},
    {"peek", NQueue_peek, METH_NOARGS, NULL},
    {"is_empty", NQueue_is_empty, METH_NOARGS, NULL},
    {"for_each", NQueue_for_each, METH_O, NULL},
    {NULL, NULL, 0, NULL},
};

static PyGetSetDef NQueue_getset[] = {
    {"_len", NQueue_get_len, NULL, NULL, NULL},
    {"length", NQueue_get_len, NULL, NULL, NULL},
    {NULL, NULL, NULL, NULL, NULL},
};

static PySequenceMethods NQueue_as_sequence = {
    NQueue_len,
};

PyTypeObject NQueueType = {
    PyVarObject_HEAD_INIT(NULL, 0)
    "cueball_amd._speed.Queue",
    sizeof(NQueue),
};

static void
queue_types_init(void)
{
    QNodeType.tp_dealloc = QNode_dealloc;
    QNodeType.tp_flags = Py_TPFLAGS_DEFAULT | Py_TPFLAGS_HAVE_GC;
    QNodeType.tp_traverse = QNode_traverse;
    QNodeType.tp_clear = QNode_clear_;
    QNodeType.tp_methods = QNode_methods;
    QNodeType.tp_getset = QNode_getset;

    NQueueType.tp_dealloc = NQueue_dealloc;
    NQueueType.tp_as_sequence = &NQueue_as_sequence;
    NQueueType.tp_flags = Py_TPFLAGS_DEFAULT | Py_TPFLAGS_HAVE_GC;
    NQueueType.tp_traverse = NQueue_traverse;
    NQueueType.tp_clear = NQueue_clear_;
    NQueueType.tp_iter = NQueue_iter;
    NQueueType.tp_methods = NQueue_methods;
    NQueueType.tp_getset = NQueue_getset;
    NQueueType.tp_new = NQueue_new;
}


PyObject *s_running_st;
PyObject *s_p_idleq_node;
PyObject *s_p_total_conns;
PyObject *s_p_busy_hwm;
PyObject *s_p_demand_hwm;
PyObject *s_ticket_slow;
PyObject *s_p_idleq;
PyObject *s_p_waiters;
PyObject *s_p_initq;

typedef struct {
    PyObject *ct_pool;
    PyObject *ct_handle;
    NQueue *ct_idleq;
    NQueue *ct_waiters;
    NQueue *ct_initq;
    int ct_err_on_empty;
} TicketCore;

typedef struct {
    PyObject_HEAD
    TicketCore core;
} CTOb;

extern PyTypeObject CTType;

static void
ct_bind_queues(TicketCore *t, PyObject *pool)
{
    PyObject *iq = PyObject_GetAttr(pool, s_p_idleq);
    PyObject *wq = iq ? PyObject_GetAttr(pool, s_p_waiters) : NULL;
    PyObject *nq = wq ? PyObject_GetAttr(pool, s_p_initq) : NULL;
    if (nq == NULL) {
        PyErr_Clear();
        Py_XDECREF(iq);
        Py_XDECREF(wq);
        return;
    }
    if (PyObject_TypeCheck(iq, &NQueueType) &&
        PyObject_TypeCheck(wq, &NQueueType) &&
        PyObject_TypeCheck(nq, &NQueueType)) {
        t->ct_idleq = (NQueue *)iq;
        t->ct_waiters = (NQueue *)wq;
        t->ct_initq = (NQueue *)nq;
    } else {
        Py_DECREF(iq);
        Py_DECREF(wq);
        Py_DECREF(nq);
    }
}

static int
ct_note_demand(TicketCore *t)
{
    Py_ssize_t nw = t->ct_waiters->q_len;
    Py_ssize_t ni = t->ct_initq->q_len;
    Py_ssize_t spares = t->ct_idleq->q_len + ni - nw;
    if (spares < 0)
        spares = 0;
    PyObject *tot = PyObject_GetAttr(t->ct_pool, s_p_total_conns);
    if (tot == NULL)
        return -1;
    long total = PyLong_AsLong(tot);
    Py_DECREF(tot);
    if (total == -1 && PyErr_Occurred())
        return -1;
    long busy = total - (long)spares;
    if (busy < 0)
        busy = 0;
    long extras = (long)(nw - ni);
    if (extras < 0)
        extras = 0;

    PyObject *cur = PyObject_GetAttr(t->ct_pool, s_p_busy_hwm);
    if (cur == NULL)
        return -1;
    long curv = PyLong_AsLong(cur);
    Py_DECREF(cur);
    if (curv == -1 && PyErr_Occurred())
        return -1;
    if (busy > curv) {
        PyObject *nv = PyLong_FromLong(busy);
        if (nv == NULL)
            return -1;
        int r = PyObject_SetAttr(t->ct_pool, s_p_busy_hwm, nv);
        Py_DECREF(nv);
        if (r < 0)
            return -1;
    }
    cur = PyObject_GetAttr(t->ct_pool, s_p_demand_hwm);
    if (cur == NULL)
        return -1;
    curv = PyLong_AsLong(cur);
    Py_DECREF(cur);
    if (curv == -1 && PyErr_Occurred())
        return -1;
    if (busy + extras > curv) {
        PyObject *nv = PyLong_FromLong(busy + extras);
        if (nv == NULL)
            return -1;
        int r = PyObject_SetAttr(t->ct_pool, s_p_demand_hwm, nv);
        Py_DECREF(nv);
        if (r < 0)
            return -1;
    }
    return 0;
}

PyObject *s_p_counters;
PyObject *s_p_rebal_scheduled;
PyObject *s_max_claim_queue;
PyObject *s_queued_claim;
extern PyObject *s_rebalance;

static int
ct_enqueue_waiter(TicketCore *t)
{
    QNode *n = nqueue_push(t->ct_waiters, t->ct_handle);
    if (n == NULL)
        return -1;
    Py_XSETREF(((CHOb *)t->ct_handle)->chb_waiter_node, (PyObject *)n);
    if (ct_note_demand(t) < 0)
        return -1;

    PyObject *counters = PyObject_GetAttr(t->ct_pool, s_p_counters);
    if (counters == NULL)
        return -1;
    if (!PyDict_Check(counters)) {
        Py_DECREF(counters);
        PyErr_SetString(PyExc_TypeError, "p_counters must be a dict");
        return -1;
    }
    PyObject *cur = PyDict_GetItemWithError(counters, s_max_claim_queue);
    if (cur == NULL && PyErr_Occurred()) {
        Py_DECREF(counters);
        return -1;
    }
    long curv = -1;
    if (cur != NULL) {
        curv = PyLong_AsLong(cur);
        if (curv == -1 && PyErr_Occurred()) {
            Py_DECREF(counters);
            return -1;
        }
    }
    if ((long)t->ct_waiters->q_len > curv) {
        PyObject *nv = PyLong_FromSsize_t(t->ct_waiters->q_len);
        if (nv == NULL || PyDict_SetItem(counters, s_max_claim_queue,
                                         nv) < 0) {
            Py_XDECREF(nv);
            Py_DECREF(counters);
            return -1;
        }
        Py_DECREF(nv);
    }
    cur = PyDict_GetItemWithError(counters, s_queued_claim);
    if (cur == NULL && PyErr_Occurred()) {
        Py_DECREF(counters);
        return -1;
    }
    long qc = 0;
    if (cur != NULL) {
        qc = PyLong_AsLong(cur);
        if (qc == -1 && PyErr_Occurred()) {
            Py_DECREF(counters);
            return -1;
        }
    }
    PyObject *nv = PyLong_FromLong(qc + 1);
    if (nv == NULL ||
        PyDict_SetItem(counters, s_queued_claim, nv) < 0) {
        Py_XDECREF(nv);
        Py_DECREF(counters);
        return -1;
    }
    Py_DECREF(nv);
    Py_DECREF(counters);

    PyObject *sched = PyObject_GetAttr(t->ct_pool, s_p_rebal_scheduled);
    if (sched == NULL)
        return -1;
    int pending = PyObject_IsTrue(sched);
    Py_DECREF(sched);
    if (pending < 0)
        return -1;
    if (!pending) {
        PyObject *r = PyObject_CallMethodObjArgs(t->ct_pool,
                                                 s_rebalance, NULL);
        if (r == NULL)
            return -1;
        Py_DECREF(r);
    }
    return 0;
}

static int
ct_slow(TicketCore *t)
{
    PyObject *r = PyObject_CallMethodObjArgs(
        t->ct_pool, s_ticket_slow, t->ct_handle,
        t->ct_err_on_empty ? Py_True : Py_False, NULL);
    if (r == NULL)
        return -1;
    Py_DECREF(r);
    return 0;
}

static int
ct_try_next(TicketCore *t)
{
    CHOb *h = (CHOb *)t->ct_handle;
    if (!ch_state_is(h, s_waiting))
        return 0;
    if (t->ct_idleq == NULL)
        return ct_slow(t);
    PyObject *pst = ((FSMOb *)t->ct_pool)->f_state;
    if (!(pst == s_running_st ||
          (pst != NULL && PyUnicode_Compare(pst, s_running_st) == 0)))
        return ct_slow(t);

    NQueue *q = t->ct_idleq;
    while (q->q_len > 0) {
        QNode *n = q->q_first;
        PyObject *fsm = n->value;
        Py_XINCREF(fsm);
        Py_INCREF((PyObject *)n);
        nqueue_unlink(q, n);
        Py_DECREF((PyObject *)n);
        if (fsm == NULL)
            continue;
        if (PyObject_TypeCheck(fsm, &SlotBaseType)) {
            slot_field_store(&((SlotOb *)fsm)->sl_idleq_node, Py_None);
        } else if (PyObject_SetAttr(fsm, s_p_idleq_node, Py_None) < 0) {
            Py_DECREF(fsm);
            return -1;
        }
        int isidle;
        if (PyObject_TypeCheck(fsm, &FSMType)) {
            PyObject *fs = ((FSMOb *)fsm)->f_state;
            isidle = (fs == s_idle ||
                      (fs != NULL &&
                       PyUnicode_Compare(fs, s_idle) == 0));
        } else {
            PyObject *r = PyObject_CallMethodObjArgs(
                fsm, s_is_in_state, s_idle, NULL);
            if (r == NULL) {
                Py_DECREF(fsm);
                return -1;
            }
            isidle = PyObject_IsTrue(r);
            Py_DECREF(r);
        }
        if (!isidle) {
            Py_DECREF(fsm);
            continue;
        }
        PyObject *r = CH_try_((PyObject *)h, fsm);
        Py_DECREF(fsm);
        if (r == NULL)
            return -1;
        Py_DECREF(r);
        return ct_note_demand(t);
    }
    if (!t->ct_err_on_empty)
        return ct_enqueue_waiter(t);
    return ct_slow(t);
}

static int
ch_ticket_try_next(CHOb *h)
{
    TicketCore v = {h->chb_pool, (PyObject *)h, (NQueue *)h->chb_idleq,
                    (NQueue *)h->chb_waiters, (NQueue *)h->chb_initq,
                    h->chb_tk_err_on_empty};
    PyObject *pool = v.ct_pool;
    Py_INCREF(pool);
    int r = ct_try_next(&v);
    Py_DECREF(pool);
    return r;
}

static PyObject *
CT_call(PyObject *self_, PyObject *args, PyObject *kwds)
{
    TicketCore *t = &((CTOb *)self_)->core;
    (void)kwds;
    PyObject *st;
    if (PyTuple_GET_SIZE(args) != 1) {
        PyErr_SetString(PyExc_TypeError, "ClaimTicket(state)");
        return NULL;
    }
    st = PyTuple_GET_ITEM(args, 0);
    if (st == s_waiting ||
        (PyUnicode_Check(st) && PyUnicode_Compare(st, s_waiting) == 0)) {
        if (ct_try_next(t) < 0)
            return NULL;
    }
    Py_RETURN_NONE;
}

static int
CT_traverse(PyObject *self_, visitproc visit, void *arg)
{
    TicketCore *t = &((CTOb *)self_)->core;
    Py_VISIT(t->ct_pool);
    Py_VISIT(t->ct_handle);
    Py_VISIT((PyObject *)t->ct_idleq);
    Py_VISIT((PyObject *)t->ct_waiters);
    Py_VISIT((PyObject *)t->ct_initq);
    return 0;
}

static int
CT_clear_(PyObject *self_)
{
    TicketCore *t = &((CTOb *)self_)->core;
    Py_CLEAR(t->ct_pool);
    Py_CLEAR(t->ct_handle);
    Py_CLEAR(t->ct_idleq);
    Py_CLEAR(t->ct_waiters);
    Py_CLEAR(t->ct_initq);
    return 0;
}

static void
CT_dealloc(PyObject *self_)
{
    PyObject_GC_UnTrack(self_);
    CT_clear_(self_);
    PyObject_GC_Del(self_);
}

static PyObject *
CT_new(PyTypeObject *type, PyObject *args, PyObject *kwds)
{
    PyObject *pool, *handle, *err_on_empty;
    (void)kwds;
    if (!PyArg_ParseTuple(args, "OOO", &pool, &handle, &err_on_empty))
        return NULL;
    if (!PyObject_TypeCheck(pool, &FSMType)) {
        PyErr_SetString(PyExc_TypeError, "pool must be a native FSM");
        return NULL;
    }
    if (!PyObject_TypeCheck(handle, &CHType)) {
        PyErr_SetString(PyExc_TypeError,
                        "handle must be a ClaimHandleBase");
        return NULL;
    }
    CTOb *tob = PyObject_GC_New(CTOb, type);
    if (tob == NULL)
        return NULL;
    TicketCore *t = &tob->core;
    Py_INCREF(pool);
    t->ct_pool = pool;
    Py_INCREF(handle);
    t->ct_handle = handle;
    t->ct_idleq = NULL;
    t->ct_waiters = NULL;
    t->ct_initq = NULL;
    t->ct_err_on_empty = PyObject_IsTrue(err_on_empty);
    PyObject_GC_Track((PyObject *)tob);
    ct_bind_queues(t, pool);
    return (PyObject *)tob;
}

PyTypeObject CTType = {
    PyVarObject_HEAD_INIT(NULL, 0)
    "cueball_amd._speed.ClaimTicket",
    sizeof(CTOb),
};

static PyObject *speed_claim_fast(PyObject *mod, PyObject *const *args,
                                  Py_ssize_t nargs);

static PyObject *
speed_pool_claim(PyObject *mod, PyObject *const *args, Py_ssize_t nargs)
{
    (void)mod;
    if (nargs != 5) {
        PyErr_SetString(PyExc_TypeError,
                        "pool_claim(cls, pool, cb, log, loop)");
        return NULL;
    }
    PyObject *pool = args[1];
    if (!PyObject_TypeCheck(pool, &FSMType)) {
        PyErr_SetString(PyExc_TypeError, "pool must be a native FSM");
        return NULL;
    }
    PyObject *counters = PyObject_GetAttr(pool, s_p_counters);
    if (counters == NULL)
        return NULL;
    if (PyDict_Check(counters)) {
        PyObject *cur = PyDict_GetItemWithError(counters, s_claim);
        if (cur == NULL && PyErr_Occurred()) {
            Py_DECREF(counters);
            return NULL;
        }
        long v = 0;
        if (cur != NULL) {
            v = PyLong_AsLong(cur);
            if (v == -1 && PyErr_Occurred()) {
                Py_DECREF(counters);
                return NULL;
            }
        }
        PyObject *nv = PyLong_FromLong(v + 1);
        if (nv == NULL ||
            PyDict_SetItem(counters, s_claim, nv) < 0) {
            Py_XDECREF(nv);
            Py_DECREF(counters);
            return NULL;
        }
        Py_DECREF(nv);
    }
    Py_DECREF(counters);

    PyObject *pst = ((FSMOb *)pool)->f_state;
    int bad = 0;
    if (pst == NULL) {
        bad = 1;
    } else if (!(pst == s_running_st ||
                 PyUnicode_Compare(pst, s_running_st) == 0)) {
        bad = !(PyUnicode_CompareWithASCIIString(pst, "starting") == 0);
    }
    if (bad)
        Py_RETURN_TRUE;

    PyObject *stack = capture_stack();
    if (stack == NULL)
        return NULL;
    PyObject *cfargs[8] = {args[0], pool, stack, args[2], args[3],
                           g_inf, args[4], Py_False};
    PyObject *h = speed_claim_fast(NULL, cfargs, 8);
    Py_DECREF(stack);
    return h;
}

PyObject *CH__setup(PyObject *self_, PyObject *const *args,
                    Py_ssize_t nargs);

static PyObject *
speed_claim_fast(PyObject *mod, PyObject *const *args, Py_ssize_t nargs)
{
    (void)mod;
    if (nargs != 8) {
        PyErr_SetString(PyExc_TypeError,
            "claim_fast(cls, pool, stack, cb, log, timeout, loop, "
            "err_on_empty)");
        return NULL;
    }
    PyTypeObject *cls = (PyTypeObject *)args[0];
    if (!PyType_Check(args[0]) ||
        !PyType_IsSubtype(cls, &CHType)) {
        PyErr_SetString(PyExc_TypeError,
                        "cls must be a ClaimHandleBase subclass");
        return NULL;
    }
    PyObject *pool = args[1];
    if (!PyObject_TypeCheck(pool, &FSMType)) {
        PyErr_SetString(PyExc_TypeError, "pool must be a native FSM");
        return NULL;
    }
    int err_on_empty = PyObject_IsTrue(args[7]);
    if (err_on_empty < 0)
        return NULL;

    PyObject *handle = cls->tp_alloc(cls, 0);
    if (handle == NULL)
        return NULL;
    PyObject *setup_args[7] = {pool, args[2], args[3], args[4],
                               args[5], Py_True, args[6]};
    PyObject *r = CH__setup(handle, setup_args, 7);
    if (r == NULL) {
        Py_DECREF(handle);
        return NULL;
    }
    Py_DECREF(r);

#if CUEBALL_HANDLE_HOOKS
    {
        CHOb *h = (CHOb *)handle;
        TicketCore q = {NULL, NULL, NULL, NULL, NULL, 0};
        ct_bind_queues(&q, pool);
        Py_XSETREF(h->chb_idleq, (PyObject *)q.ct_idleq);
        Py_XSETREF(h->chb_waiters, (PyObject *)q.ct_waiters);
        Py_XSETREF(h->chb_initq, (PyObject *)q.ct_initq);
        h->chb_tk_err_on_empty = err_on_empty;
        h->chb_tk_on = 1;
    }
#else
    CTOb *tob = PyObject_GC_New(CTOb, &CTType);
    if (tob == NULL) {
        Py_DECREF(handle);
        return NULL;
    }
    TicketCore *t = &tob->core;
    Py_INCREF(pool);
    t->ct_pool = pool;
    Py_INCREF(handle);
    t->ct_handle = handle;
    t->ct_idleq = NULL;
    t->ct_waiters = NULL;
    t->ct_initq = NULL;
    t->ct_err_on_empty = err_on_empty;
    PyObject_GC_Track((PyObject *)tob);
    ct_bind_queues(t, pool);
    r = emitter_add((Emitter *)handle, s_stateChanged, (PyObject *)tob);
    Py_DECREF((PyObject *)tob);
    if (r == NULL) {
        Py_DECREF(handle);
        return NULL;
    }
    Py_DECREF(r);
#endif
    return handle;
}

static void
ct_type_init(void)
{
    CTType.tp_dealloc = CT_dealloc;
    CTType.tp_call = CT_call;
    CTType.tp_flags = Py_TPFLAGS_DEFAULT | Py_TPFLAGS_HAVE_GC;
    CTType.tp_traverse = CT_traverse;
    CTType.tp_clear = CT_clear_;
    CTType.tp_new = CT_new;
}

void
ch_terminal_cleanup(FSMOb *self)
{
    PyObject *wn = ((CHOb *)self)->chb_waiter_node;
    if (wn != NULL) {
        ((CHOb *)self)->chb_waiter_node = NULL;
        if (PyObject_TypeCheck(wn, &QNodeType) &&
            ((QNode *)wn)->q_queue != NULL)
            nqueue_unlink(((QNode *)wn)->q_queue, (QNode *)wn);
        Py_DECREF(wn);
    }
    if (self->f_scope != NULL) {
        PyObject *old = self->f_scope;
        self->f_scope = NULL;
        PyObject *r = Scope_dispose(old, NULL);
        Py_DECREF(old);
        if (r == NULL)
            PyErr_Clear();
        else
            Py_DECREF(r);
    }
#if CUEBALL_HANDLE_HOOKS
    ((CHOb *)self)->chb_tk_on = 0;
#else
    Emitter *em = &self->base;
    if (em->ev_events == NULL)
        return;
    PyObject *ls = PyDict_GetItemWithError(em->ev_events, s_stateChanged);
    if (ls == NULL) {
        PyErr_Clear();
        return;
    }
    if (!PyList_Check(ls))
        return;
    for (Py_ssize_t i = PyList_GET_SIZE(ls) - 1; i >= 0; i--) {
        if (PyObject_TypeCheck(PyList_GET_ITEM(ls, i), &CTType)) {
            if (PyList_SetSlice(ls, i, i + 1, NULL) < 0) {
                PyErr_Clear();
                return;
            }
        }
    }
#endif
}


PyObject *s_connected_st;
PyObject *s_busy_st;
PyObject *s_stopping_st;
PyObject *s_stopped_st;
PyObject *s_retrying_st;
PyObject *s_connecting_st;
PyObject *s_killing_st;
PyObject *s_unwanted_evt;
PyObject *s_sm_socket;
PyObject *t_busy_valid;
PyObject *t_idle_valid;

typedef struct SlotKit SlotKit;

enum { KCB_BUSY_SMGR = 0, KCB_BUSY_HDL, KCB_IDLE_SMGR, KCB_IDLE_UNWANTED,
       KCB_CONN_ERR, KCB_N };

typedef struct {
    PyObject_HEAD
    SlotKit *kc_kit;
    int kc_which;
    vectorcallfunc kc_vectorcall;
} KitCb;

struct SlotKit {
    PyObject_HEAD
    FSMOb *k_slot;
    PyObject *k_smgr;
    PyObject *k_observed;
    unsigned long k_busy_serial;
    unsigned long k_idle_serial;
    PyObject *k_cbs[KCB_N];
};

extern PyTypeObject SlotKitType;
extern PyTypeObject KitCbType;

PyObject *
slotkit_conn_err_cb(PyObject *slot, PyObject *handle)
{
    if (slot == NULL || !PyObject_TypeCheck(slot, &SlotBaseType))
        return NULL;
    PyObject *kit = ((FSMOb *)slot)->f_fastkit;
    if (kit == NULL || Py_TYPE(kit) != &SlotKitType ||
        ((SlotKit *)kit)->k_slot != (FSMOb *)slot ||
        ((SlotOb *)slot)->sl_handle != handle)
        return NULL;
    return ((SlotKit *)kit)->k_cbs[KCB_CONN_ERR];
}

static int
kit_goto(SlotKit *k, unsigned long serial, PyObject *state)
{
    if (serial == 0 || k->k_slot->f_hist_n != serial)
        return 0;
    return fsm_goto_state(k->k_slot, state);
}

static int
kit_busy_on_release(SlotKit *k)
{
    unsigned long S = k->k_busy_serial;
    PyObject *st = k->k_observed;
    int wanted = slot_field_true(&((SlotOb *)k->k_slot)->sl_wanted);
    if (wanted < 0)
        return -1;
    if (st == s_connected_st ||
        (st != NULL && PyUnicode_Compare(st, s_connected_st) == 0))
        return kit_goto(k, S, wanted ? s_idle : s_stopping_st);
    if (st == s_closed || PyUnicode_Compare(st, s_closed) == 0)
        return kit_goto(k, S, wanted ? s_connecting_st : s_stopped_st);
    if (st == s_error_evt || PyUnicode_Compare(st, s_error_evt) == 0)
        return kit_goto(k, S, s_retrying_st);
    PyErr_Format(g_fsm_error,
                 "Handle released while smgr was in unhandled state %R",
                 st ? st : Py_None);
    return -1;
}

static int
kit_busy_on_close(SlotKit *k)
{
    unsigned long S = k->k_busy_serial;
    PyObject *st = k->k_observed;
    if (st == s_connected_st ||
        (st != NULL && PyUnicode_Compare(st, s_connected_st) == 0))
        return kit_goto(k, S, s_killing_st);
    return kit_goto(k, S, s_retrying_st);
}

static int
kit_idle_smgr_changed(SlotKit *k, PyObject *st)
{
    unsigned long S = k->k_idle_serial;
    int wanted = slot_field_true(&((SlotOb *)k->k_slot)->sl_wanted);
    if (wanted < 0)
        return -1;
    if (st == s_error_evt || PyUnicode_Compare(st, s_error_evt) == 0)
        return kit_goto(k, S, wanted ? s_retrying_st : s_stopped_st);
    if (st == s_closed || PyUnicode_Compare(st, s_closed) == 0)
        return kit_goto(k, S, wanted ? s_connecting_st : s_stopped_st);
    PyErr_Format(g_fsm_error,
                 "Unhandled smgr state transition: connected => %R", st);
    return -1;
}

static int
kit_idle_unwanted(SlotKit *k)
{
    unsigned long S = k->k_idle_serial;
    PyObject *sst = ((FSMOb *)k->k_smgr)->f_state;
    if (sst == s_connected_st ||
        (sst != NULL && PyUnicode_Compare(sst, s_connected_st) == 0))
        return kit_goto(k, S, s_stopping_st);
    if (sst == s_error_evt || sst == s_closed ||
        (sst != NULL && (PyUnicode_Compare(sst, s_error_evt) == 0 ||
                         PyUnicode_Compare(sst, s_closed) == 0)))
        return kit_goto(k, S, s_stopped_st);
    return 0;
}

static PyObject *
kitcb_fire(PyObject *self_, PyObject *st)
{
    KitCb *cb = (KitCb *)self_;
    SlotKit *k = cb->kc_kit;
    int r = 0;
    switch (cb->kc_which) {
    case KCB_BUSY_SMGR:
        if (st != NULL) {
            Py_INCREF(st);
            Py_XSETREF(k->k_observed, st);
        }
        break;
    case KCB_BUSY_HDL:
        if (st == s_released ||
            (st != NULL && PyUnicode_Compare(st, s_released) == 0))
            r = kit_busy_on_release(k);
        else if (st == s_closed ||
                 (st != NULL && PyUnicode_Compare(st, s_closed) == 0))
            r = kit_busy_on_close(k);
        break;
    case KCB_IDLE_SMGR:
        r = kit_idle_smgr_changed(k, st);
        break;
    case KCB_IDLE_UNWANTED:
        r = kit_idle_unwanted(k);
        break;
    case KCB_CONN_ERR: {
        PyObject *hdl = ((SlotOb *)k->k_slot)->sl_handle;
        if (hdl == NULL || !PyObject_TypeCheck(hdl, &CHType))
            break;
        Py_INCREF(hdl);
        PyObject *res = conn_err_fire((CHOb *)hdl,
                                      st != NULL ? st : Py_None);
        Py_DECREF(hdl);
        return res;
    }
    }
    if (r < 0)
        return NULL;
    Py_RETURN_NONE;
}

static PyObject *
KitCb_call(PyObject *self_, PyObject *args, PyObject *kwds)
{
    (void)kwds;
    return kitcb_fire(self_, PyTuple_GET_SIZE(args) >= 1
                      ? PyTuple_GET_ITEM(args, 0) : NULL);
}

static PyObject *
KitCb_vectorcall(PyObject *self_, PyObject *const *args, size_t nargsf,
                 PyObject *kwnames)
{
    (void)kwnames;
    return kitcb_fire(self_, PyVectorcall_NARGS(nargsf) >= 1 ? args[0]
                                                             : NULL);
}

static int
KitCb_traverse(PyObject *self_, visitproc visit, void *arg)
{
    Py_VISIT((PyObject *)((KitCb *)self_)->kc_kit);
    return 0;
}

static int
KitCb_clear_(PyObject *self_)
{
    Py_CLEAR(((KitCb *)self_)->kc_kit);
    return 0;
}

static void
KitCb_dealloc(PyObject *self_)
{
    PyObject_GC_UnTrack(self_);
    KitCb_clear_(self_);
    PyObject_GC_Del(self_);
}

PyTypeObject KitCbType = {
    PyVarObject_HEAD_INIT(NULL, 0)
    "cueball_amd._speed._SlotKitCb",
    sizeof(KitCb),
};


static int
kit_state_busy(SlotKit *k)
{
    FSMOb *slot = k->k_slot;
    Py_INCREF(t_busy_valid);
    Py_XSETREF(slot->f_valid, t_busy_valid);

    PyObject *hdl = ((SlotOb *)slot)->sl_handle;
    if (hdl == NULL)
        hdl = Py_None;
    Py_INCREF(hdl);
    Py_INCREF(s_connected_st);
    Py_XSETREF(k->k_observed, s_connected_st);
    k->k_busy_serial = slot->f_hist_n;

#if !CUEBALL_SLOT_HOOKS
    {
        Scope *scope = fsm_need_scope(slot);
        if (scope == NULL ||
            scope_on_c(scope, k->k_smgr, s_stateChanged,
                       k->k_cbs[KCB_BUSY_SMGR]) < 0) {
            Py_DECREF(hdl);
            return -1;
        }
    }
#endif
    int armed = 0;
#if CUEBALL_HANDLE_HOOKS
    if (PyObject_TypeCheck(hdl, &CHType)) {
        CHOb *h = (CHOb *)hdl;
        PyObject *ls = h->base.base.ev_events == NULL ? NULL :
            PyDict_GetItemWithError(h->base.base.ev_events, s_stateChanged);
        if (ls == NULL && PyErr_Occurred()) {
            Py_DECREF(hdl);
            return -1;
        }
        h->chb_bk_pos = (ls != NULL && PyList_Check(ls))
            ? PyList_GET_SIZE(ls) : 0;
        h->chb_bk_serial = k->k_busy_serial;
        armed = 1;
    }
#endif
    if (!armed) {
        Scope *scope = fsm_need_scope(slot);
        if (scope == NULL ||
            scope_on_c(scope, hdl, s_stateChanged,
                       k->k_cbs[KCB_BUSY_HDL]) < 0) {
            Py_DECREF(hdl);
            return -1;
        }
    }

    PyObject *sst = ((FSMOb *)k->k_smgr)->f_state;
    int connected = (sst == s_connected_st ||
                     (sst != NULL &&
                      PyUnicode_Compare(sst, s_connected_st) == 0));
    PyObject *r;
    if (connected) {
        PyObject *sock = PyObject_GetAttr(k->k_smgr, s_sm_socket);
        if (sock == NULL) {
            Py_DECREF(hdl);
            return -1;
        }
        r = CH_accept(hdl, sock);
        Py_DECREF(sock);
        Py_DECREF(hdl);
        if (r == NULL)
            return -1;
        Py_DECREF(r);
    } else {
        r = CH_reject(hdl, NULL);
        Py_DECREF(hdl);
        if (r == NULL)
            return -1;
        Py_DECREF(r);
        slot_field_store(&((SlotOb *)slot)->sl_handle, Py_None);
        if (kit_busy_on_release(k) < 0)
            return -1;
    }
    return 1;
}

static int
kit_state_idle(SlotKit *k)
{
    FSMOb *slot = k->k_slot;
    int monitor = slot_field_true(&((SlotOb *)slot)->sl_monitor);
    if (monitor < 0)
        return -1;
    if (monitor)
        return 0;
    int wanted = slot_field_true(&((SlotOb *)slot)->sl_wanted);
    if (wanted < 0)
        return -1;
    if (!wanted)
        return 0;

    Py_INCREF(t_idle_valid);
    Py_XSETREF(slot->f_valid, t_idle_valid);
    k->k_idle_serial = slot->f_hist_n;

    SlotOb *so = (SlotOb *)slot;
    if (slot_field_set(&so->sl_handle)) {
        PyObject *old_prev = so->sl_prev_handle;
        so->sl_prev_handle = so->sl_handle;
        Py_INCREF(Py_None);
        so->sl_handle = Py_None;
        Py_XDECREF(old_prev);
    }

#if !CUEBALL_SLOT_HOOKS
    Scope *scope = fsm_need_scope(slot);
    if (scope == NULL)
        return -1;
    if (scope_on_c(scope, k->k_smgr, s_stateChanged,
                   k->k_cbs[KCB_IDLE_SMGR]) < 0)
        return -1;
    if (scope_on_c(scope, (PyObject *)slot, s_unwanted_evt,
                   k->k_cbs[KCB_IDLE_UNWANTED]) < 0)
        return -1;
#endif
    return 1;
}

int
slotkit_maybe_entry(PyObject *kit_, FSMOb *fsm, PyObject *target)
{
    SlotKit *k = (SlotKit *)kit_;
    if (k->k_slot != fsm)
        return 0;
    if (target == s_busy_st ||
        (PyUnicode_Check(target) &&
         PyUnicode_Compare(target, s_busy_st) == 0))
        return kit_state_busy(k);
    if (target == s_idle ||
        (PyUnicode_Check(target) &&
         PyUnicode_Compare(target, s_idle) == 0))
        return kit_state_idle(k);
    return 0;
}


static inline int
str_is(PyObject *a, PyObject *b)
{
    return a == b || (a != NULL && PyUnicode_Check(a) &&
                      PyUnicode_Compare(a, b) == 0);
}

unsigned long
slotkit_slot_serial(PyObject *kit_)
{
    SlotKit *k = (SlotKit *)kit_;
    if (Py_TYPE(kit_) != &SlotKitType || k->k_slot == NULL)
        return 0;
    return k->k_slot->f_hist_n;
}

int
slotkit_smgr_hook(PyObject *kit_, PyObject *st, unsigned long serial)
{
#if CUEBALL_SLOT_HOOKS
    SlotKit *k = (SlotKit *)kit_;
    if (Py_TYPE(kit_) != &SlotKitType || k->k_slot == NULL)
        return 0;
    unsigned long now = k->k_slot->f_hist_n;
    if (now == 0 || now != serial)
        return 0;
    if (now == k->k_busy_serial) {
        Py_INCREF(st);
        Py_XSETREF(k->k_observed, st);
        return 0;
    }
    if (now == k->k_idle_serial) {
        Py_INCREF(kit_);
        int r = kit_idle_smgr_changed(k, st);
        Py_DECREF(kit_);
        return r;
    }
#else
    (void)kit_; (void)st;
#endif
    return 0;
}

static int
ch_slot_hook(CHOb *h, PyObject *st)
{
    PyObject *slot = h->chb_slot;
    if (h->chb_bk_serial == 0 || slot == NULL ||
        !PyObject_TypeCheck(slot, &SlotBaseType))
        return 0;
    PyObject *kit_ = ((FSMOb *)slot)->f_fastkit;
    if (kit_ == NULL || Py_TYPE(kit_) != &SlotKitType)
        return 0;
    SlotKit *k = (SlotKit *)kit_;
    if (k->k_slot != (FSMOb *)slot ||
        k->k_busy_serial != h->chb_bk_serial ||
        k->k_slot->f_hist_n != h->chb_bk_serial)
        return 0;
    int r = 0;
    Py_INCREF(kit_);
    if (str_is(st, s_released))
        r = kit_busy_on_release(k);
    else if (str_is(st, s_closed))
        r = kit_busy_on_close(k);
    Py_DECREF(kit_);
    return r;
}

int
ch_emit_state_changed(FSMOb *self, PyObject *st)
{
    CHOb *h = (CHOb *)self;
    PyObject *ls = NULL;
    if (self->base.ev_events != NULL) {
        ls = PyDict_GetItemWithError(self->base.ev_events, s_stateChanged);
        if (ls == NULL && PyErr_Occurred())
            return -1;
    }
    Py_ssize_t n = ls != NULL ? PyList_GET_SIZE(ls) : 0;
    int hook = h->chb_bk_serial != 0 &&
        (str_is(st, s_released) || str_is(st, s_closed));
    Py_ssize_t pos = !hook ? -1 : h->chb_bk_pos < n ? h->chb_bk_pos : n;
    PyObject *snap = NULL;
    if (n > 0) {
        snap = PyList_GetSlice(ls, 0, n);
        if (snap == NULL)
            return -1;
    }
    if (h->chb_tk_on && str_is(st, s_waiting)) {
        if (ch_ticket_try_next(h) < 0) {
            Py_XDECREF(snap);
            return -1;
        }
    }
    if (n == 0)
        return hook ? ch_slot_hook(h, st) : 0;
    for (Py_ssize_t i = 0; i <= n; i++) {
        if (i == pos && ch_slot_hook(h, st) < 0) {
            Py_DECREF(snap);
            return -1;
        }
        if (i == n)
            break;
        PyObject *r = PyObject_Vectorcall(PyList_GET_ITEM(snap, i), &st, 1,
                                          NULL);
        if (r == NULL) {
            Py_DECREF(snap);
            return -1;
        }
        Py_DECREF(r);
    }
    Py_DECREF(snap);
    return 1;
}

static PyObject *
Slot_emit(PyObject *self_, PyObject *const *args, Py_ssize_t nargs)
{
    if (nargs < 1) {
        PyErr_SetString(PyExc_TypeError, "emit(event, *args)");
        return NULL;
    }
    FSMOb *slot = (FSMOb *)self_;
    unsigned long serial = slot->f_hist_n;
    int r = emitter_emit_core((Emitter *)self_, args[0], args + 1,
                              nargs - 1);
    if (r < 0)
        return NULL;
#if CUEBALL_SLOT_HOOKS
    PyObject *kit_ = slot->f_fastkit;
    if (kit_ != NULL && Py_TYPE(kit_) == &SlotKitType &&
        str_is(args[0], s_unwanted_evt)) {
        SlotKit *k = (SlotKit *)kit_;
        if (k->k_slot == slot && serial != 0 &&
            slot->f_hist_n == serial && serial == k->k_idle_serial) {
            Py_INCREF(kit_);
            int hr = kit_idle_unwanted(k);
            Py_DECREF(kit_);
            if (hr < 0)
                return NULL;
            r = 1;
        }
    }
#endif
    return PyBool_FromLong(r);
}

static PyObject *
Slot_event_names(PyObject *self_, PyObject *noargs)
{
    PyObject *names = Emitter_event_names(self_, noargs);
#if CUEBALL_SLOT_HOOKS
    if (names == NULL)
        return NULL;
    FSMOb *slot = (FSMOb *)self_;
    PyObject *kit_ = slot->f_fastkit;
    if (kit_ != NULL && Py_TYPE(kit_) == &SlotKitType &&
        ((SlotKit *)kit_)->k_slot == slot && slot->f_hist_n != 0 &&
        slot->f_hist_n == ((SlotKit *)kit_)->k_idle_serial) {
        int has = PySequence_Contains(names, s_unwanted_evt);
        if (has < 0 || (!has && PyList_Append(names, s_unwanted_evt) < 0)) {
            Py_DECREF(names);
            return NULL;
        }
    }
#endif
    return names;
}

static PyMethodDef Slot_methods[] = {
    {"emit", (PyCFunction)(void (*)(void))Slot_emit, METH_FASTCALL, NULL},
    {"event_names", Slot_event_names, METH_NOARGS, NULL},
    {NULL, NULL, 0, NULL},
};


#define CODEL_INTERVAL_MS 100.0

typedef struct {
    PyObject_HEAD
    PyObject *cd_loop;
    double cd_targdelay;
    double cd_first_above_time;
    double cd_drop_next;
    long cd_count;
    int cd_dropping;
    double cd_last_empty;
} CoDelOb;

extern PyTypeObject CoDelType;

static double
codel_now(CoDelOb *self, int *err)
{
    PyObject *t = PyObject_CallMethodObjArgs(self->cd_loop, s_time, NULL);
    if (t == NULL) {
        *err = 1;
        return 0.0;
    }
    double secs = PyFloat_AsDouble(t);
    Py_DECREF(t);
    if (secs == -1.0 && PyErr_Occurred()) {
// ... 153 lines not shown
    CoDel_clear_(self_);
    PyObject_GC_Del(self_);
}

static PyObject *
CoDel_new(PyTypeObject *type, PyObject *args, PyObject *kwds)
{
    PyObject *target, *loop = Py_None;
    static const char *kwlist[] = {"target_claim_delay", "loop", NULL};
    if (!PyArg_ParseTupleAndKeywords(args, kwds, "O|O",
                                     const_cast<char **>(kwlist),
                                     &target, &loop))
        return NULL;
    double targ;
    if (PyFloat_Check(target) || PyLong_Check(target)) {
        targ = PyFloat_AsDouble(target);
        if (targ == -1.0 && PyErr_Occurred())
            return NULL;
    } else {
        PyErr_SetString(PyExc_ValueError,
                        "target_claim_delay must be finite");
        return NULL;
    }
    if (!std::isfinite(targ)) {
        PyErr_SetString(PyExc_ValueError,
                        "target_claim_delay must be finite");
        return NULL;
    }
    PyObject *resolved = PyObject_CallOneArg(g_get_loop, loop);
    if (resolved == NULL)
        return NULL;
    CoDelOb *self = PyObject_GC_New(CoDelOb, type);
    if (self == NULL) {
        Py_DECREF(resolved);
        return NULL;
    }
    self->cd_loop = resolved;
    self->cd_targdelay = targ;
    self->cd_first_above_time = 0.0;
    self->cd_drop_next = 0.0;
    self->cd_count = 0;
    self->cd_dropping = 0;
    self->cd_last_empty = 0.0;
    PyObject_GC_Track((PyObject *)self);
    int err = 0;
    double now = codel_now(self, &err);
    if (err) {
        Py_DECREF((PyObject *)self);
        return NULL;
    }
    self->cd_last_empty = now;
    return (PyObject *)self;
}

static PyMethodDef CoDel_methods[] = {
    {"overloaded", CoDel_overloaded, METH_O, NULL},
    {"can_drop", (PyCFunction)(void (*)(void))CoDel_can_drop,
     METH_FASTCALL, NULL},
    {"get_drop_next", CoDel_get_drop_next, METH_O, NULL},
    {"empty", CoDel_empty, METH_NOARGS, NULL},
    {"get_max_idle", CoDel_get_max_idle, METH_NOARGS, NULL},
    {NULL, NULL, 0, NULL},
};

static PyMemberDef CoDel_members[] = {
    {(char *)"cd_targdelay", T_DOUBLE, offsetof(CoDelOb, cd_targdelay),
     READONLY, NULL},
    {(char *)"cd_first_above_time", T_DOUBLE,
     offsetof(CoDelOb, cd_first_above_time), 0, NULL},
    {(char *)"cd_drop_next", T_DOUBLE, offsetof(CoDelOb, cd_drop_next),
     0, NULL},
    {(char *)"cd_count", T_LONG, offsetof(CoDelOb, cd_count), 0, NULL},
    {(char *)"cd_last_empty", T_DOUBLE,
     offsetof(CoDelOb, cd_last_empty), 0, NULL},
    {NULL, 0, 0, 0, NULL},
};

static PyGetSetDef CoDel_getset[] = {
    {(char *)"cd_dropping", CoDel_get_dropping, NULL, NULL, NULL},
    {NULL, NULL, NULL, NULL, NULL},
};

PyTypeObject CoDelType = {
    PyVarObject_HEAD_INIT(NULL, 0)
    "cueball_amd._speed.ControlledDelay",
    sizeof(CoDelOb),
};

static void
codel_type_init(void)
{
    CoDelType.tp_dealloc = CoDel_dealloc;
    CoDelType.tp_flags = Py_TPFLAGS_DEFAULT | Py_TPFLAGS_HAVE_GC;
    CoDelType.tp_traverse = CoDel_traverse;
    CoDelType.tp_clear = CoDel_clear_;
    CoDelType.tp_methods = CoDel_methods;
    CoDelType.tp_members = CoDel_members;
    CoDelType.tp_getset = CoDel_getset;
    CoDelType.tp_new = CoDel_new;
}


PyObject *s_p_backends;
PyObject *s_p_dead;
PyObject *s_connected_to_backend;
PyObject *s_slot_state_changed;
PyObject *s_remove_node;
PyObject *s_rebalance;
PyObject *s_set_unwanted;

typedef struct {
    PyObject_HEAD
    PyObject *sd_pool;
    PyObject *sd_fsm;
    PyObject *sd_key;
    NQueue *sd_idleq;
    NQueue *sd_waiters;
    PyObject *sd_codel;
    int sd_has_codel;
    vectorcallfunc sd_vectorcall;
} SlotDispatch;

extern PyTypeObject SlotDispatchType;

static int
sd_fallback(SlotDispatch *d, PyObject *st)
{
    PyObject *r = PyObject_CallMethodObjArgs(
        d->sd_pool, s_slot_state_changed, d->sd_fsm, d->sd_key, st,
        NULL);
    if (r == NULL)
        return -1;
    Py_DECREF(r);
    return 0;
}

static PyObject *
slotdispatch_run(PyObject *self_, PyObject *st)
{
    SlotDispatch *d = (SlotDispatch *)self_;
    FSMOb *fsm = (FSMOb *)d->sd_fsm;

    SlotOb *so = (SlotOb *)d->sd_fsm;
    int in_initq = slot_field_set(&so->sl_initq_node);

    if (!in_initq &&
        (st == s_busy_st ||
         (PyUnicode_Check(st) &&
          PyUnicode_Compare(st, s_busy_st) == 0))) {
        if (!slot_field_set(&so->sl_idleq_node)) {
            PyObject *hdl = so->sl_handle;
            int pinger = 0;
            if (hdl != NULL && hdl != Py_None &&
                PyObject_TypeCheck(hdl, &CHType))
                pinger = ((CHOb *)hdl)->chb_pinger;
            if (!pinger)
                Py_RETURN_NONE;
        }
        if (sd_fallback(d, st) < 0)
            return NULL;
        Py_RETURN_NONE;
    }

    if (!in_initq && (!d->sd_has_codel || d->sd_codel != NULL) &&
        (st == s_idle ||
         (PyUnicode_Check(st) &&
          PyUnicode_Compare(st, s_idle) == 0))) {
        PyObject *dead = PyObject_GetAttr(d->sd_pool, s_p_dead);
        if (dead == NULL)
            return NULL;
        int isdead = PyDict_Check(dead) ?
            PyDict_Contains(dead, d->sd_key) : 1;
        Py_DECREF(dead);
        if (isdead != 0) {
            if (isdead < 0)
                return NULL;
            if (sd_fallback(d, st) < 0)
                return NULL;
            Py_RETURN_NONE;
        }
        PyObject *eargs[3] = {s_connected_to_backend, d->sd_key,
                              d->sd_fsm};
        if (emitter_emit_core((Emitter *)d->sd_pool, eargs[0],
                              eargs + 1, 2) < 0)
            return NULL;
        PyObject *fs = fsm->f_state;
        if (!(fs == s_idle ||
              (fs != NULL && PyUnicode_Compare(fs, s_idle) == 0))) {
            if (slot_field_set(&so->sl_idleq_node)) {
                PyObject *idn = so->sl_idleq_node;
                Py_INCREF(idn);
                PyObject *rr = PyObject_CallMethodObjArgs(
                    idn, s_remove_node, NULL);
                Py_DECREF(idn);
                if (rr == NULL)
                    return NULL;
                Py_DECREF(rr);
                slot_field_store(&so->sl_idleq_node, Py_None);
                PyObject *rb = PyObject_CallMethodObjArgs(
                    d->sd_pool, s_rebalance, NULL);
                if (rb == NULL)
                    return NULL;
                Py_DECREF(rb);
            }
            Py_RETURN_NONE;
        }
        {
            PyObject *backends = PyObject_GetAttr(d->sd_pool,
                                                  s_p_backends);
            if (backends == NULL)
                return NULL;
            int wanted = PyDict_Check(backends) ?
                PyDict_Contains(backends, d->sd_key) : 0;
            Py_DECREF(backends);
            if (wanted < 0)
                return NULL;
            if (!wanted) {
                PyObject *su = PyObject_CallMethodObjArgs(
                    d->sd_fsm, s_set_unwanted, NULL);
                if (su == NULL)
                    return NULL;
                Py_DECREF(su);
                Py_RETURN_NONE;
            }
        }
        while (d->sd_waiters->q_len > 0) {
            PyObject *hdl = nqueue_shift_value(d->sd_waiters);
            if (hdl == NULL)
                return NULL;
            if (!PyObject_TypeCheck(hdl, &CHType)) {
                Py_DECREF(hdl);
                continue;
            }
            int drop = 0;
            if (d->sd_codel != NULL) {
                drop = codel_overloaded_c((CoDelOb *)d->sd_codel,
                                          ((CHOb *)hdl)->chb_started);
                if (drop < 0) {
                    Py_DECREF(hdl);
                    return NULL;
                }
            }
            if (!ch_state_is((CHOb *)hdl, s_waiting)) {
                Py_DECREF(hdl);
                continue;
            }
            if (drop) {
                PyObject *r = CH_timeout(hdl, NULL);
                Py_DECREF(hdl);
                if (r == NULL)
                    return NULL;
                Py_DECREF(r);
                continue;
            }
            PyObject *r = CH_try_(hdl, d->sd_fsm);
            Py_DECREF(hdl);
            if (r == NULL)
                return NULL;
            Py_DECREF(r);
            Py_RETURN_NONE;
        }
        if (d->sd_codel != NULL &&
            codel_empty_c((CoDelOb *)d->sd_codel) < 0)
            return NULL;
        QNode *n = nqueue_push(d->sd_idleq, d->sd_fsm);
        if (n == NULL)
            return NULL;
        Py_XSETREF(so->sl_idleq_node, (PyObject *)n);
        Py_RETURN_NONE;
    }

    if (sd_fallback(d, st) < 0)
        return NULL;
    Py_RETURN_NONE;
}

static PyObject *
SlotDispatch_call(PyObject *self_, PyObject *args, PyObject *kwds)
{
    (void)kwds;
    if (PyTuple_GET_SIZE(args) != 1) {
        PyErr_SetString(PyExc_TypeError, "SlotDispatch(state)");
        return NULL;
    }
    return slotdispatch_run(self_, PyTuple_GET_ITEM(args, 0));
}

static PyObject *
SlotDispatch_vectorcall(PyObject *self_, PyObject *const *args,
                        size_t nargsf, PyObject *kwnames)
{
    if (PyVectorcall_NARGS(nargsf) != 1 ||
        (kwnames != NULL && PyTuple_GET_SIZE(kwnames) != 0)) {
        PyErr_SetString(PyExc_TypeError, "SlotDispatch(state)");
        return NULL;
    }
    return slotdispatch_run(self_, args[0]);
}

static int
SlotDispatch_traverse(PyObject *self_, visitproc visit, void *arg)
{
    SlotDispatch *d = (SlotDispatch *)self_;
    Py_VISIT(d->sd_pool);
    Py_VISIT(d->sd_fsm);
    Py_VISIT(d->sd_key);
    Py_VISIT((PyObject *)d->sd_idleq);
    Py_VISIT((PyObject *)d->sd_waiters);
    Py_VISIT(d->sd_codel);
    return 0;
}

static int
SlotDispatch_clear_(PyObject *self_)
{
    SlotDispatch *d = (SlotDispatch *)self_;
    Py_CLEAR(d->sd_pool);
    Py_CLEAR(d->sd_fsm);
    Py_CLEAR(d->sd_key);
    Py_CLEAR(d->sd_idleq);
    Py_CLEAR(d->sd_waiters);
    Py_CLEAR(d->sd_codel);
    return 0;
}

static void
SlotDispatch_dealloc(PyObject *self_)
{
    PyObject_GC_UnTrack(self_);
    SlotDispatch_clear_(self_);
    PyObject_GC_Del(self_);
}

static PyObject *
SlotDispatch_new(PyTypeObject *type, PyObject *args, PyObject *kwds)
{
    PyObject *pool, *fsm, *key, *has_codel;
    (void)kwds;
    if (!PyArg_ParseTuple(args, "OOOO", &pool, &fsm, &key, &has_codel))
        return NULL;
    if (!PyObject_TypeCheck(pool, &EmitterType) ||
        !PyObject_TypeCheck(fsm, &SlotBaseType)) {
        PyErr_SetString(PyExc_TypeError,
                        "SlotDispatch(pool, slot, key, has_codel)");
        return NULL;
    }
    PyObject *iq = PyObject_GetAttrString(pool, "p_idleq");
    PyObject *wq = iq ? PyObject_GetAttrString(pool, "p_waiters") : NULL;
    if (wq == NULL || !PyObject_TypeCheck(iq, &NQueueType) ||
        !PyObject_TypeCheck(wq, &NQueueType)) {
        Py_XDECREF(iq);
        Py_XDECREF(wq);
        if (!PyErr_Occurred())
            PyErr_SetString(PyExc_TypeError,
                            "pool queues must be native");
        return NULL;
    }
    SlotDispatch *d = PyObject_GC_New(SlotDispatch, type);
    if (d == NULL) {
        Py_DECREF(iq);
        Py_DECREF(wq);
        return NULL;
    }
    Py_INCREF(pool);
    d->sd_pool = pool;
    Py_INCREF(fsm);
    d->sd_fsm = fsm;
    Py_INCREF(key);
    d->sd_key = key;
    d->sd_idleq = (NQueue *)iq;
    d->sd_waiters = (NQueue *)wq;
    d->sd_has_codel = PyObject_IsTrue(has_codel);
    d->sd_codel = NULL;
    d->sd_vectorcall = SlotDispatch_vectorcall;
    PyObject_GC_Track((PyObject *)d);
    if (d->sd_has_codel) {
        PyObject *cd = PyObject_GetAttrString(pool, "p_codel");
        if (cd == NULL) {
            PyErr_Clear();
        } else if (PyObject_TypeCheck(cd, &CoDelType)) {
            d->sd_codel = cd;
        } else {
            Py_DECREF(cd);
        }
    }
    return (PyObject *)d;
}

PyTypeObject SlotDispatchType = {
    PyVarObject_HEAD_INIT(NULL, 0)
    "cueball_amd._speed.SlotDispatch",
    sizeof(SlotDispatch),
};


static int
SlotKit_traverse(PyObject *self_, visitproc visit, void *arg)
{
    SlotKit *k = (SlotKit *)self_;
    Py_VISIT((PyObject *)k->k_slot);
    Py_VISIT(k->k_smgr);
    Py_VISIT(k->k_observed);
    for (int i = 0; i < KCB_N; i++)
        Py_VISIT(k->k_cbs[i]);
    return 0;
}

static int
SlotKit_clear_(PyObject *self_)
{
    SlotKit *k = (SlotKit *)self_;
    Py_CLEAR(k->k_slot);
    Py_CLEAR(k->k_smgr);
    Py_CLEAR(k->k_observed);
    for (int i = 0; i < KCB_N; i++)
        Py_CLEAR(k->k_cbs[i]);
    return 0;
}

static void
SlotKit_dealloc(PyObject *self_)
{
    PyObject_GC_UnTrack(self_);
    SlotKit_clear_(self_);
    PyObject_GC_Del(self_);
}

static PyObject *
SlotKit_new(PyTypeObject *type, PyObject *args, PyObject *kwds)
{
    PyObject *slot, *smgr;
    (void)kwds;
    if (!PyArg_ParseTuple(args, "OO", &slot, &smgr))
        return NULL;
    if (!PyObject_TypeCheck(slot, &SlotBaseType) ||
        !PyObject_TypeCheck(smgr, &FSMType)) {
        PyErr_SetString(PyExc_TypeError,
                        "SlotKit(slot, smgr): a SlotBase and a native "
                        "FSM required");
        return NULL;
    }
    SlotKit *k = PyObject_GC_New(SlotKit, type);
    if (k == NULL)
        return NULL;
    Py_INCREF(slot);
    k->k_slot = (FSMOb *)slot;
    Py_INCREF(smgr);
    k->k_smgr = smgr;
    k->k_observed = NULL;
    k->k_busy_serial = 0;
    k->k_idle_serial = 0;
    for (int i = 0; i < KCB_N; i++)
        k->k_cbs[i] = NULL;
    PyObject_GC_Track((PyObject *)k);
    for (int i = 0; i < KCB_N; i++) {
        KitCb *cb = PyObject_GC_New(KitCb, &KitCbType);
        if (cb == NULL) {
            Py_DECREF((PyObject *)k);
            return NULL;
        }
        Py_INCREF((PyObject *)k);
        cb->kc_kit = k;
        cb->kc_which = i;
        cb->kc_vectorcall = KitCb_vectorcall;
        PyObject_GC_Track((PyObject *)cb);
        k->k_cbs[i] = (PyObject *)cb;
    }
#if CUEBALL_SLOT_HOOKS
    Py_INCREF((PyObject *)k);
    Py_XSETREF(((FSMOb *)smgr)->f_watchkit, (PyObject *)k);
#endif
    return (PyObject *)k;
}

PyTypeObject SlotKitType = {
    PyVarObject_HEAD_INIT(NULL, 0)
    "cueball_amd._speed.SlotKit",
    sizeof(SlotKit),
};

static void
slotkit_types_init(void)
{
    KitCbType.tp_dealloc = KitCb_dealloc;
    KitCbType.tp_call = KitCb_call;
    KitCbType.tp_flags = Py_TPFLAGS_DEFAULT | Py_TPFLAGS_HAVE_GC;
    KitCbType.tp_traverse = KitCb_traverse;
    KitCbType.tp_clear = KitCb_clear_;
    KitCbType.tp_getset = ConnErrCb_getset;

    SlotKitType.tp_dealloc = SlotKit_dealloc;
    SlotKitType.tp_flags = Py_TPFLAGS_DEFAULT | Py_TPFLAGS_HAVE_GC;
    SlotKitType.tp_traverse = SlotKit_traverse;
    SlotKitType.tp_clear = SlotKit_clear_;
    SlotKitType.tp_new = SlotKit_new;

    SlotDispatchType.tp_dealloc = SlotDispatch_dealloc;
    SlotDispatchType.tp_call = SlotDispatch_call;
    SlotDispatchType.tp_flags = Py_TPFLAGS_DEFAULT | Py_TPFLAGS_HAVE_GC;
    SlotDispatchType.tp_traverse = SlotDispatch_traverse;
    SlotDispatchType.tp_clear = SlotDispatch_clear_;
    SlotDispatchType.tp_new = SlotDispatch_new;

    SlotBaseType.tp_methods = Slot_methods;
#if CUEBALL_VECTORCALL
    KitCbType.tp_vectorcall_offset = offsetof(KitCb, kc_vectorcall);
    KitCbType.tp_flags |= Py_TPFLAGS_HAVE_VECTORCALL;
    SlotDispatchType.tp_vectorcall_offset =
        offsetof(SlotDispatch, sd_vectorcall);
    SlotDispatchType.tp_flags |= Py_TPFLAGS_HAVE_VECTORCALL;
    FlushBatchType.tp_vectorcall_offset = offsetof(FlushBatch, fb_vectorcall);
    FlushBatchType.tp_flags |= Py_TPFLAGS_HAVE_VECTORCALL;
#endif
}


PyObject *s_p_codel;
PyObject *s_p_claim_log;

typedef struct {
    PyObject_HEAD
    PyObject *cm_func;
    PyObject *cm_handle_cls;
    PyObject *cm_doc;
    PyObject *cm_name;
    PyObject *cm_qualname;
    PyObject *cm_module;
    vectorcallfunc cm_vectorcall;
} ClaimMethod;

extern PyTypeObject ClaimMethodType;

static PyObject *
ClaimMethod_vectorcall(PyObject *self_, PyObject *const *args,
                       size_t nargsf, PyObject *kwnames)
{
    ClaimMethod *cm = (ClaimMethod *)self_;
    if (PyVectorcall_NARGS(nargsf) == 3 &&
        (kwnames == NULL || PyTuple_GET_SIZE(kwnames) == 0)) {
        PyObject *pool = args[0], *opt = args[1], *cb = args[2];
        if (cb != Py_None &&
            (opt == Py_None ||
             (PyDict_CheckExact(opt) && PyDict_GET_SIZE(opt) == 0)) &&
            PyObject_TypeCheck(pool, &FSMType)) {
            PyObject *pst = ((FSMOb *)pool)->f_state;
            int open = pst != NULL &&
                (pst == s_running_st ||
                 PyUnicode_Compare(pst, s_running_st) == 0 ||
                 PyUnicode_CompareWithASCIIString(pst, "starting") == 0);
            PyObject *codel = open ? PyObject_GetAttr(pool, s_p_codel)
                                   : NULL;
            if (open && codel == NULL)
                return NULL;
            Py_XDECREF(codel);
            if (open && codel == Py_None) {
                PyObject *log = PyObject_GetAttr(pool, s_p_claim_log);
                if (log == NULL)
                    return NULL;
                PyObject *pargs[5] = {cm->cm_handle_cls, pool, cb, log,
                                      ((FSMOb *)pool)->f_loop};
                PyObject *h = speed_pool_claim(NULL, pargs, 5);
                Py_DECREF(log);
                return h;
            }
        }
    }
    return PyObject_Vectorcall(cm->cm_func, args, nargsf, kwnames);
}

static PyObject *
ClaimMethod_descr_get(PyObject *self_, PyObject *obj, PyObject *type)
{
    (void)type;
    if (obj == NULL || obj == Py_None) {
        Py_INCREF(self_);
        return self_;
    }
    return PyMethod_New(self_, obj);
}

static int
ClaimMethod_traverse(PyObject *self_, visitproc visit, void *arg)
{
    ClaimMethod *cm = (ClaimMethod *)self_;
    Py_VISIT(cm->cm_func);
    Py_VISIT(cm->cm_handle_cls);
    return 0;
}

static int
ClaimMethod_clear_(PyObject *self_)
{
    ClaimMethod *cm = (ClaimMethod *)self_;
    Py_CLEAR(cm->cm_func);
    Py_CLEAR(cm->cm_handle_cls);
    Py_CLEAR(cm->cm_doc);
    Py_CLEAR(cm->cm_name);
    Py_CLEAR(cm->cm_qualname);
    Py_CLEAR(cm->cm_module);
    return 0;
}

static void
ClaimMethod_dealloc(PyObject *self_)
{
    PyObject_GC_UnTrack(self_);
    ClaimMethod_clear_(self_);
    PyObject_GC_Del(self_);
}

static PyMemberDef ClaimMethod_members[] = {
    {(char *)"__wrapped__", T_OBJECT, offsetof(ClaimMethod, cm_func),
     READONLY, NULL},
    {(char *)"__doc__", T_OBJECT, offsetof(ClaimMethod, cm_doc), READONLY,
     NULL},
    {(char *)"__name__", T_OBJECT, offsetof(ClaimMethod, cm_name), READONLY,
     NULL},
    {(char *)"__qualname__", T_OBJECT, offsetof(ClaimMethod, cm_qualname),
     READONLY, NULL},
    {(char *)"__module__", T_OBJECT, offsetof(ClaimMethod, cm_module),
     READONLY, NULL},
    {NULL, 0, 0, 0, NULL},
};

PyTypeObject ClaimMethodType = {
    PyVarObject_HEAD_INIT(NULL, 0)
    "cueball_amd._speed._ClaimMethod",
    sizeof(ClaimMethod),
};

static void
claim_method_type_init(void)
{
    ClaimMethodType.tp_dealloc = ClaimMethod_dealloc;
    ClaimMethodType.tp_vectorcall_offset =
        offsetof(ClaimMethod, cm_vectorcall);
    ClaimMethodType.tp_call = PyVectorcall_Call;
    ClaimMethodType.tp_flags = Py_TPFLAGS_DEFAULT | Py_TPFLAGS_HAVE_GC |
        Py_TPFLAGS_HAVE_VECTORCALL | Py_TPFLAGS_METHOD_DESCRIPTOR;
    ClaimMethodType.tp_traverse = ClaimMethod_traverse;
    ClaimMethodType.tp_clear = ClaimMethod_clear_;
    ClaimMethodType.tp_members = ClaimMethod_members;
    ClaimMethodType.tp_descr_get = ClaimMethod_descr_get;
}

static PyObject *
speed_claim_method(PyObject *mod, PyObject *const *args, Py_ssize_t nargs)
{
    (void)mod;
    if (nargs != 2 || !PyCallable_Check(args[0]) || !PyType_Check(args[1]) ||
        !PyType_IsSubtype((PyTypeObject *)args[1], &CHType)) {
        PyErr_SetString(PyExc_TypeError,
                        "claim_method(func, ClaimHandleBase subclass)");
        return NULL;
    }
#if !CUEBALL_VECTORCALL
    Py_INCREF(args[0]);
    return args[0];
#else
    ClaimMethod *cm = PyObject_GC_New(ClaimMethod, &ClaimMethodType);
    if (cm == NULL)
        return NULL;
    Py_INCREF(args[0]);
    cm->cm_func = args[0];
    Py_INCREF(args[1]);
    cm->cm_handle_cls = args[1];
    cm->cm_vectorcall = ClaimMethod_vectorcall;
    cm->cm_doc = PyObject_GetAttrString(args[0], "__doc__");
    cm->cm_name = PyObject_GetAttrString(args[0], "__name__");
    cm->cm_qualname = PyObject_GetAttrString(args[0], "__qualname__");
    cm->cm_module = PyObject_GetAttrString(args[0], "__module__");
    PyErr_Clear();
    PyObject_GC_Track((PyObject *)cm);
    return (PyObject *)cm;
#endif
}

PyObject *
speed_set_tracer(PyObject *mod, PyObject *fn)
{
    (void)mod;
    if (fn == Py_None) {
        Py_CLEAR(g_tracer);
    } else {
        Py_INCREF(fn);
        Py_XSETREF(g_tracer, fn);
    }
    Py_RETURN_NONE;
}

PyMethodDef speed_methods[] = {
    {"_set_claim_helpers",
     (PyCFunction)(void (*)(void))speed_set_claim_helpers, METH_FASTCALL,
     NULL},
    {"_set_tracer", speed_set_tracer, METH_O, NULL},
    {"_set_stack_traces",
     (PyCFunction)(void (*)(void))speed_set_stack_traces, METH_FASTCALL,
     NULL},
    {"count_listeners",
     (PyCFunction)(void (*)(void))speed_count_listeners, METH_FASTCALL,
     NULL},
    {"_set_helpers", (PyCFunction)(void (*)(void))speed_set_helpers,
     METH_FASTCALL, NULL},
    {"claim_fast", (PyCFunction)(void (*)(void))speed_claim_fast,
     METH_FASTCALL, NULL},
    {"pool_claim", (PyCFunction)(void (*)(void))speed_pool_claim,
     METH_FASTCALL, NULL},
    {"claim_method", (PyCFunction)(void (*)(void))speed_claim_method,
     METH_FASTCALL, NULL},
    {NULL, NULL, 0, NULL},
};

struct PyModuleDef speedmodule = {
    PyModuleDef_HEAD_INIT,
    "cueball_amd._speed",
    "Native event/FSM runtime core",
    -1,
    speed_methods,
};

}

PyMODINIT_FUNC
PyInit__speed(void)
{
    s_stateChanged = PyUnicode_InternFromString("stateChanged");
    s_listener = PyUnicode_InternFromString("listener");
    s_on = PyUnicode_InternFromString("on");
    s_remove_listener = PyUnicode_InternFromString("remove_listener");
    s_call_soon = PyUnicode_InternFromString("call_soon");
    s_call_later = PyUnicode_InternFromString("call_later");
    s_cancel = PyUnicode_InternFromString("cancel");
    s_state_prefix = PyUnicode_InternFromString("state_");
    s_dot = PyUnicode_InternFromString(".");
    s_underscore = PyUnicode_InternFromString("_");
    s_flush_name = PyUnicode_InternFromString("_flush_state_changed");
    s_internal = PyUnicode_InternFromString("_cueball_internal");
    s_is_closed = PyUnicode_InternFromString("is_closed");
    s_claim = PyUnicode_InternFromString("claim");
    s_warn = PyUnicode_InternFromString("warn");
    s_incr = PyUnicode_InternFromString("_incr_counter");
    s_claim_timeout_evt = PyUnicode_InternFromString("claim-timeout");
    s_is_in_state = PyUnicode_InternFromString("is_in_state");
    s_time = PyUnicode_InternFromString("time");
    s_waiting = PyUnicode_InternFromString("waiting");
    s_claiming = PyUnicode_InternFromString("claiming");
    s_claimed = PyUnicode_InternFromString("claimed");
    s_released = PyUnicode_InternFromString("released");
    s_closed = PyUnicode_InternFromString("closed");
    s_cancelled = PyUnicode_InternFromString("cancelled");
    s_failed = PyUnicode_InternFromString("failed");
    s_idle = PyUnicode_InternFromString("idle");
    s_error_evt = PyUnicode_InternFromString("error");
    t_waiting_valid = PyTuple_Pack(3, s_claiming, s_cancelled, s_failed);
    t_claiming_valid = PyTuple_Pack(3, s_claimed, s_waiting, s_cancelled);
    t_claimed_valid = PyTuple_Pack(2, s_released, s_closed);
    t_empty = PyTuple_New(0);
    s_leak_events[0] = PyUnicode_InternFromString("close");
    s_leak_events[1] = s_error_evt;
    s_leak_events[2] = PyUnicode_InternFromString("readable");
    s_leak_events[3] = PyUnicode_InternFromString("data");
    g_entry_name_cache = PyDict_New();
    if (g_entry_name_cache == NULL)
        return NULL;
    g_flush_batches = PyDict_New();
    if (g_flush_batches == NULL)
        return NULL;

    s_running_st = PyUnicode_InternFromString("running");
    s_p_idleq_node = PyUnicode_InternFromString("p_idleq_node");
    s_p_total_conns = PyUnicode_InternFromString("p_total_conns");
    s_p_busy_hwm = PyUnicode_InternFromString("p_busy_hwm");
    s_p_demand_hwm = PyUnicode_InternFromString("p_demand_hwm");
    s_ticket_slow = PyUnicode_InternFromString("_ticket_slow");
    s_p_idleq = PyUnicode_InternFromString("p_idleq");
    s_p_waiters = PyUnicode_InternFromString("p_waiters");
    s_p_initq = PyUnicode_InternFromString("p_initq");
    s_p_counters = PyUnicode_InternFromString("p_counters");
    s_p_rebal_scheduled = PyUnicode_InternFromString("p_rebal_scheduled");
    s_max_claim_queue = PyUnicode_InternFromString("max-claim-queue");
    s_queued_claim = PyUnicode_InternFromString("queued-claim");
    s_connected_st = PyUnicode_InternFromString("connected");
    s_busy_st = PyUnicode_InternFromString("busy");
    s_stopping_st = PyUnicode_InternFromString("stopping");
    s_stopped_st = PyUnicode_InternFromString("stopped");
    s_retrying_st = PyUnicode_InternFromString("retrying");
    s_connecting_st = PyUnicode_InternFromString("connecting");
    s_killing_st = PyUnicode_InternFromString("killing");
    s_unwanted_evt = PyUnicode_InternFromString("unwanted");
    s_sm_socket = PyUnicode_InternFromString("sm_socket");
    t_busy_valid = PyTuple_Pack(6, s_idle, s_stopping_st, s_stopped_st,
                                s_retrying_st, s_killing_st,
                                s_connecting_st);
    t_idle_valid = PyTuple_Pack(5, s_retrying_st, s_connecting_st,
                                s_stopping_st, s_stopped_st, s_busy_st);
    s_p_backends = PyUnicode_InternFromString("p_backends");
    s_p_dead = PyUnicode_InternFromString("p_dead");
    s_connected_to_backend =
        PyUnicode_InternFromString("connectedToBackend");
    s_slot_state_changed =
        PyUnicode_InternFromString("_slot_state_changed");
    s_remove_node = PyUnicode_InternFromString("remove");
    s_rebalance = PyUnicode_InternFromString("rebalance");
    s_set_unwanted = PyUnicode_InternFromString("set_unwanted");
    queue_types_init();
    ct_type_init();
    slotkit_types_init();
    codel_type_init();
    claim_method_type_init();
    s_p_codel = PyUnicode_InternFromString("p_codel");
    s_p_claim_log = PyUnicode_InternFromString("p_claim_log");
    s_p_lat = PyUnicode_InternFromString("p_lat");
    latency_types_init();
    if (PyType_Ready(&LatHistType) < 0 ||
        PyType_Ready(&PoolLatType) < 0)
        return NULL;
    if (PyType_Ready(&EmitterType) < 0 ||
        PyType_Ready(&OnceWrapperType) < 0 ||
        PyType_Ready(&GuardedCbType) < 0 ||
        PyType_Ready(&ScopeType) < 0 ||
        PyType_Ready(&IntervalType) < 0 ||
        PyType_Ready(&FlushBatchType) < 0 ||
        PyType_Ready(&ConnErrCbType) < 0 ||
        PyType_Ready(&FailCbType) < 0 ||
        PyType_Ready(&CHType) < 0 ||
        PyType_Ready(&FSMType) < 0 ||
        PyType_Ready(&SlotBaseType) < 0 ||
        PyType_Ready(&QNodeType) < 0 ||
        PyType_Ready(&NQueueType) < 0 ||
        PyType_Ready(&CTType) < 0 ||
        PyType_Ready(&KitCbType) < 0 ||
        PyType_Ready(&SlotKitType) < 0 ||
        PyType_Ready(&SlotDispatchType) < 0 ||
        PyType_Ready(&ClaimMethodType) < 0 ||
        PyType_Ready(&CoDelType) < 0)
        return NULL;

    g_remove_desc = PyDict_GetItemString(EmitterType.tp_dict,
                                         "remove_listener");
    if (g_remove_desc == NULL)
        return NULL;
    Py_INCREF(g_remove_desc);
    g_ch_remove_desc = PyDict_GetItemString(CHType.tp_dict,
                                            "remove_listener");
    if (g_ch_remove_desc == NULL)
        return NULL;
    Py_INCREF(g_ch_remove_desc);
    if (ch_entries_init() < 0)
        return NULL;
    g_inf = PyFloat_FromDouble(HUGE_VAL);
    if (g_inf == NULL)
        return NULL;

    PyObject *m = PyModule_Create(&speedmodule);
    if (m == NULL)
        return NULL;
    Py_INCREF(&EmitterType);
    PyModule_AddObject(m, "EventEmitter", (PyObject *)&EmitterType);
    Py_INCREF(&ScopeType);
    PyModule_AddObject(m, "StateScope", (PyObject *)&ScopeType);
    Py_INCREF(&FSMType);
    PyModule_AddObject(m, "FSM", (PyObject *)&FSMType);
    Py_INCREF(&SlotBaseType);
    PyModule_AddObject(m, "SlotBase", (PyObject *)&SlotBaseType);
    Py_INCREF(&CHType);
    PyModule_AddObject(m, "ClaimHandleBase", (PyObject *)&CHType);
    Py_INCREF(&NQueueType);
    PyModule_AddObject(m, "Queue", (PyObject *)&NQueueType);
    Py_INCREF(&QNodeType);
    PyModule_AddObject(m, "QueueNode", (PyObject *)&QNodeType);
    Py_INCREF(&CTType);
    PyModule_AddObject(m, "ClaimTicket", (PyObject *)&CTType);
    Py_INCREF(&SlotKitType);
    PyModule_AddObject(m, "SlotKit", (PyObject *)&SlotKitType);
    Py_INCREF(&SlotDispatchType);
    PyModule_AddObject(m, "SlotDispatch", (PyObject *)&SlotDispatchType);
    Py_INCREF(&CoDelType);
    PyModule_AddObject(m, "ControlledDelay", (PyObject *)&CoDelType);
    Py_INCREF(&LatHistType);
    PyModule_AddObject(m, "LatencyHistogram", (PyObject *)&LatHistType);
    Py_INCREF(&PoolLatType);
    PyModule_AddObject(m, "PoolLatency", (PyObject *)&PoolLatType);
    return m;
}
```

cueball_amd/connection_fsm.py:

```python

from __future__ import annotations

import math
from typing import Any, Callable, Dict, List, Optional

from . import errors as mod_errors
from . import utils as mod_utils
from .events import EventEmitter
from .fsm import FSM, FSMError, StateScope
from .logutil import CueballLogger

__all__ = ["SocketMgrFSM", "ClaimHandle", "ConnectionSlotFSM"]

try:
    import os as _os
    if _os.environ.get("CUEBALL_PURE"):
        _native_count = None
        _SlotKit = None
        _SlotFSMBase = FSM
    else:
        from ._speed import count_listeners as _native_count
        from ._speed import SlotKit as _SlotKit
        from ._speed import SlotBase as _SlotFSMBase
except ImportError:
# ... 707 lines not shown

        def on_unwanted() -> None:
            if self.csf_monitor and smgr.is_in_state("backoff"):
                S.goto_state("stopping")

        S.on(self, "unwanted", on_unwanted)
        smgr.retry()

    _IDLE_VALID = ("retrying", "connecting", "stopping", "stopped",
                   "busy")

    def state_idle(self, S: StateScope) -> None:
        S.valid_transitions(self._IDLE_VALID)
        smgr = self.csf_smgr
        self.csf_idle_scope = S

        if self.csf_handle is not None:
            self.csf_prev_handle = self.csf_handle
        self.csf_handle = None

        if self.csf_monitor is True:
            self.csf_monitor = False
            if smgr.is_in_state("connected") or smgr.is_in_state("init"):
                smgr.set_monitor(False)
            else:
                smgr.sm_monitor = False
                smgr.reset_backoff()

        S.on(smgr, "stateChanged", self._b_idle_smgr)

        if not self.csf_wanted:
            self._idle_on_unwanted()
            return
        S.on(self, "unwanted", self._b_idle_unwanted)

        if self.csf_check_timeout is not None and \
                self.csf_checker is not None:
            S.timeout(self.csf_check_timeout, self._b_idle_ping)

    def _idle_on_unwanted(self) -> None:
        S = self.csf_idle_scope
        smgr = self.csf_smgr
        if smgr.is_in_state("connected"):
            S.goto_state("stopping")
        elif smgr.is_in_state("error") or smgr.is_in_state("closed"):
            S.goto_state("stopped")

    def _idle_smgr_cb(self, st: str) -> None:
        S = self.csf_idle_scope
        if st == "error":
            if self.csf_wanted:
                S.goto_state("retrying")
            else:
                S.goto_state("stopped")
        elif st == "closed":
            if not self.csf_wanted:
                S.goto_state("stopped")
            else:
                S.goto_state("connecting")
        else:
            raise FSMError(
                'Unhandled smgr state transition: connected => "%s"' % st)

    def _idle_ping_cb(self) -> None:
        _do_ping_check(self, self.csf_checker)

    def _busy_smgr_cb(self, st: str) -> None:
        self.csf_observed = st

    def _busy_on_release(self) -> None:
        S = self.csf_busy_scope
        st = self.csf_observed
        if st == "connected":
            if self.csf_wanted:
                S.goto_state("idle")
            else:
                S.goto_state("stopping")
        elif st == "closed":
            if self.csf_wanted:
                S.goto_state("connecting")
            else:
                S.goto_state("stopped")
        elif st == "error":
            S.goto_state("retrying")
        else:
            raise FSMError(
                'Handle released while smgr was in unhandled state "%s"'
                % self.csf_smgr.get_state())

    def _busy_on_close(self) -> None:
        S = self.csf_busy_scope
        if self.csf_observed == "connected":
            S.goto_state("killing")
        else:
            S.goto_state("retrying")

    def _busy_hdl_cb(self, st: str) -> None:
        if st == "released":
            self._busy_on_release()
        elif st == "closed":
            self._busy_on_close()

    _BUSY_VALID = ("idle", "stopping", "stopped", "retrying",
                   "killing", "connecting")

    def state_busy(self, S: StateScope) -> None:
        S.valid_transitions(self._BUSY_VALID)
        smgr = self.csf_smgr
        hdl = self.csf_handle
        self.csf_observed = "connected"
        self.csf_busy_scope = S
        S.on(smgr, "stateChanged", self._b_busy_smgr)
        S.on(hdl, "stateChanged", self._b_busy_hdl)

        if smgr.is_in_state("connected"):
            hdl.accept(smgr.get_socket())
        else:
            hdl.reject()
            self.csf_handle = None
            self._busy_on_release()

    def state_killing(self, S: StateScope) -> None:
        S.valid_transitions(["retrying"])
        smgr = self.csf_smgr

        def on_smgr_state(st: str) -> None:
            if st in ("closed", "error"):
                S.goto_state("retrying")

        S.on(smgr, "stateChanged", on_smgr_state)
        if not smgr.is_in_state("closed") and not smgr.is_in_state("error"):
            smgr.close()

    def state_stopping(self, S: StateScope) -> None:
        S.valid_transitions(["stopped"])
        smgr = self.csf_smgr

        def on_smgr_state(st: str) -> None:
            if st in ("closed", "error"):
                S.goto_state("stopped")

        S.on(smgr, "stateChanged", on_smgr_state)
        if not smgr.is_in_state("closed") and not smgr.is_in_state("error"):
            smgr.close()

    def state_stopped(self, S: StateScope) -> None:
        S.valid_transitions([])
        smgr = self.csf_smgr
        if not (smgr.is_in_state("closed") or smgr.is_in_state("error")
                or smgr.is_in_state("failed")):
            raise FSMError("smgr must be stopped")


def _do_ping_check(fsm: ConnectionSlotFSM, checker: Callable) -> None:

    def ping_check_adapter(err: Optional[BaseException], hdl: ClaimHandle,
                           conn: Any = None) -> None:
        if err is not None:
            raise FSMError("ping check handle failed unexpectedly")
        checker(hdl, conn)

    handle = ClaimHandle({
        "pool": fsm.csf_pool,
        "claimStack": ["claim", "cueball._do_ping_check",
                       "cueball._do_ping_check"],
        "callback": ping_check_adapter,
        "log": fsm.csf_log,
        "claimTimeout": math.inf,
        "loop": fsm._loop,
    })
    handle.ch_pinger = True
    handle.try_(fsm)
```

cueball_amd/pool.py:

```python

from __future__ import annotations

import functools
import math
import os as _os
import random
import time as mod_time
import uuid as mod_uuid
from typing import Any, Callable, Dict, List, Mapping, Optional

from . import codel as mod_codel
from . import errors as mod_errors
from . import latency as mod_latency
from . import utils as mod_utils
from .connection_fsm import ClaimHandle, ConnectionSlotFSM
from .events import EventEmitter
from .fsm import FSM, StateScope, get_loop
from .logutil import CueballLogger, default_logger
from .pool_monitor import monitor as global_monitor
from .queue import Queue

__all__ = ["ConnectionPool", "FIRFilter", "gen_taps"]

LP_RATE = 5
# ... 1325 lines not shown
            return
        if self.is_in_state("stopping") or self.is_in_state("stopped"):
            handle.fail(mod_errors.PoolStoppingError(self))
            return
        if self.is_in_state("failed"):
            handle.fail(mod_errors.PoolFailedError(
                self, self.p_last_error))
            return
        idleq = self.p_idleq
        if avoid is not None:
            fsm = self._idle_avoiding(avoid)
            if fsm is not None:
                handle.try_(fsm)
                self._note_demand()
                return
        while idleq._len > 0:
            fsm = idleq.shift()
            fsm.p_idleq_node = None
            if not fsm.is_in_state("idle"):
                continue
            handle.try_(fsm)
            self._note_demand()
            return

        if err_on_empty and self.p_resolver.count() < 1:
            handle.fail(mod_errors.NoBackendsError(
                self, self.p_resolver.get_last_error()))

        handle.ch_waiter_node = self.p_waiters.push(handle)
        self._note_demand()
        self._hwm_counter("max-claim-queue", self.p_waiters._len)
        self._incr_counter("queued-claim")
        self.rebalance()

    def claim(self, options: Any = None, cb: Optional[Callable] = None):
        if not options and cb is not None and self.p_codel is None:
            if _native_pool_claim is not None:
                h = _native_pool_claim(ClaimHandle, self, cb,
                                       self.p_claim_log, self._loop)
                if h is not True:
                    return h
                if self._fsm_state == "failed":
                    return self._claim_shortcircuit(
                        cb, mod_errors.PoolFailedError(
                            self, self.p_last_error))
                return self._claim_shortcircuit(
                    cb, mod_errors.PoolStoppingError(self))
            err_on_empty = False
            timeout = math.inf
            avoid = None
        else:
            if callable(options) and cb is None:
                cb = options
                options = {}
            options = options or {}
            if cb is None:
                raise TypeError("claim() requires a callback")
            err_on_empty = bool(options.get("errorOnEmpty", False))
            avoid = options.get("avoidBackends")
            if avoid is not None:
                avoid = self._assert_avoid(avoid)

            if self.p_codel is not None:
                if options.get("timeout") is not None:
                    raise ValueError("options.timeout not allowed when "
                                     "targetClaimDelay has been set")
                timeout = self.p_codel.get_max_idle()
            elif options.get("timeout") is not None:
                timeout = options["timeout"]
            else:
                timeout = math.inf

        counters = self.p_counters
        counters["claim"] = counters.get("claim", 0) + 1

        st = self._fsm_state
        if st == "stopping" or st == "stopped" or \
                st == "stopping.backends":
            return self._claim_shortcircuit(
                cb, mod_errors.PoolStoppingError(self))
        if st == "failed":
            return self._claim_shortcircuit(
                cb, mod_errors.PoolFailedError(self, self.p_last_error))

        stack = mod_utils.maybe_capture_stack_trace()
        if avoid is not None:
            handle = ClaimHandle.fast(self, stack, cb, self.p_claim_log,
                                      timeout, self._loop)
            handle.on("stateChanged",
                      _AvoidClaimTicket(self, handle, err_on_empty, avoid))
            return handle
        if _native_claim_fast is not None:
            return _native_claim_fast(ClaimHandle, self, stack, cb,
                                      self.p_claim_log, timeout,
                                      self._loop, err_on_empty)
        handle = ClaimHandle.fast(self, stack, cb, self.p_claim_log,
                                  timeout, self._loop)
        handle.on("stateChanged", _ClaimTicket(self, handle, err_on_empty))
        return handle

    def _assert_avoid(self, avoid: Any) -> Optional[frozenset]:
        if isinstance(avoid, (str, bytes)) or isinstance(avoid, Mapping):
            raise TypeError("options.avoidBackends must be an iterable of "
                            "backend keys")
        try:
            keys = list(avoid)
        except TypeError:
            raise TypeError("options.avoidBackends must be an iterable of "
                            "backend keys")
        for k in keys:
            if not isinstance(k, str):
                raise TypeError("options.avoidBackends must hold backend "
                                "keys (strings)")
        known = frozenset(k for k in keys if k in self.p_backends)
        return known or None

    def _claim_shortcircuit(self, cb: Callable, err: BaseException):
        state = {"done": False}

        def fire() -> None:
            if not state["done"]:
                cb(err)
            state["done"] = True

        self._loop.call_soon(fire)
        return _CancelStub(state)

    async def claim_async(self, options: Any = None):
        import asyncio
        fut = self._loop.create_future()

        def cb(err, hdl=None, conn=None):
            if fut.cancelled():
                if hdl is not None:
                    hdl.release()
                return
            if err is not None:
                fut.set_exception(err)
            else:
                fut.set_result((hdl, conn))

        res = self.claim(options or {}, cb)
        try:
            return await fut
        except asyncio.CancelledError:
            res.cancel()
            raise


if _native_pool_claim is not None:
    from ._speed import claim_method as _claim_method
    ConnectionPool.claim = _claim_method(
        ConnectionPool.__dict__["claim"], ClaimHandle)
```

Baseline: 811,000 claims/s.

## Cache per-pool context object and exact-type fast paths in native claim path

Adds a per-pool PoolCtx object holding the idle/waiter/init queues, counters, dead map, latency tracker and log. Handles reference it instead of doing repeated attribute lookups and per-handle refcounted fields, which also shrinks the handle struct. Registers the concrete handle, slot and pool classes so type checks can use exact-type pointer compares before PyObject_TypeCheck. Adds identity-scan validation for tuple transitions and a direct native claim dispatch when codel is absent. In exchange it makes the handle/pool lifecycle and caching more complex and can serve stale data if pool attributes change after the context is built.

```diff
diff --git a/cueball_amd/_native/speed.cpp b/cueball_amd/_native/speed.cpp
--- a/cueball_amd/_native/speed.cpp
+++ b/cueball_amd/_native/speed.cpp
@@ -19,6 +19,12 @@
 #endif
 #ifndef CUEBALL_VECTORCALL
 #define CUEBALL_VECTORCALL 1
+#endif
+#ifndef CUEBALL_EXACT_TYPES
+#define CUEBALL_EXACT_TYPES 1
+#endif
+#ifndef CUEBALL_VALID_IDENTITY
+#define CUEBALL_VALID_IDENTITY 1
 #endif
 #if !defined(Py_TPFLAGS_HAVE_VECTORCALL) && defined(_Py_TPFLAGS_HAVE_VECTORCALL)
 #define Py_TPFLAGS_HAVE_VECTORCALL _Py_TPFLAGS_HAVE_VECTORCALL
@@ -995,6 +1001,7 @@
     PyObject *f_flush_bound;
     PyObject *f_fastkit;
     PyObject *f_watchkit;
+    PyObject *f_ctx;
     int f_entering;
     int f_emit_scheduled;
 };
@@ -1021,6 +1028,42 @@
 ch_entry_fn ch_direct_entry(FSMOb *self, PyObject *target);
 
 extern PyTypeObject FSMType;
+extern PyTypeObject SlotBaseType;
+
+PyTypeObject *g_handle_cls;
+PyTypeObject *g_slot_cls;
+PyTypeObject *g_pool_cls;
+
+static inline int
+is_handle(PyObject *x)
+{
+#if CUEBALL_EXACT_TYPES
+    if (Py_TYPE(x) == g_handle_cls)
+        return 1;
+#endif
+    return PyObject_TypeCheck(x, &CHType);
+}
+
+static inline int
+is_slot(PyObject *x)
+{
+#if CUEBALL_EXACT_TYPES
+    if (Py_TYPE(x) == g_slot_cls)
+        return 1;
+#endif
+    return PyObject_TypeCheck(x, &SlotBaseType);
+}
+
+static inline int
+is_fsm(PyObject *x)
+{
+#if CUEBALL_EXACT_TYPES
+    PyTypeObject *tp = Py_TYPE(x);
+    if (tp == g_pool_cls || tp == g_slot_cls || tp == g_handle_cls)
+        return 1;
+#endif
+    return PyObject_TypeCheck(x, &FSMType);
+}
 
 PyObject *
 fsm_get_loop_of(FSMOb *fsm)
@@ -1102,13 +1145,13 @@
 {
     self->f_emit_scheduled = 0;
     int n = 0;
-    int is_handle = PyObject_TypeCheck((PyObject *)self, &CHType);
+    int handle = is_handle((PyObject *)self);
     while (self->f_eq_head < self->f_eq_len && n++ < FSM_FLUSH_CAP) {
         PyObject *st = self->f_eq[self->f_eq_head++];
         if (self->f_eq_head == self->f_eq_len)
             self->f_eq_head = self->f_eq_len = 0;
         int r;
-        if (is_handle) {
+        if (handle) {
             r = ch_emit_state_changed(self, st);
         } else {
             PyObject *eargs[2] = {s_stateChanged, st};
@@ -1341,6 +1384,14 @@
 {
     if (self->f_valid == NULL)
         return 0;
+#if CUEBALL_VALID_IDENTITY
+    if (PyTuple_CheckExact(self->f_valid)) {
+        PyObject *v = self->f_valid;
+        for (Py_ssize_t i = 0, n = PyTuple_GET_SIZE(v); i < n; i++)
+            if (PyTuple_GET_ITEM(v, i) == state)
+                return 0;
+    }
+#endif
     int c = PySequence_Contains(self->f_valid, state);
     if (c < 0)
         return -1;
@@ -1468,7 +1519,7 @@
         Py_DECREF(target);
     }
     if (self->f_valid == t_empty &&
-        PyObject_TypeCheck((PyObject *)self, &CHType))
+        is_handle((PyObject *)self))
         ch_terminal_cleanup(self);
     return 0;
 }
@@ -1797,6 +1848,7 @@
     Py_VISIT(self->f_flush_bound);
     Py_VISIT(self->f_fastkit);
     Py_VISIT(self->f_watchkit);
+    Py_VISIT(self->f_ctx);
     return Emitter_traverse(self_, visit, arg);
 }
 
@@ -1816,6 +1868,7 @@
     Py_CLEAR(self->f_flush_bound);
     Py_CLEAR(self->f_fastkit);
     Py_CLEAR(self->f_watchkit);
+    Py_CLEAR(self->f_ctx);
     return Emitter_clear_(self_);
 }
 
@@ -1859,10 +1912,22 @@
     {NULL, 0, 0, 0, NULL},
 };
 
+PyObject *
+FSM_get__claim_ctx(PyObject *self_, void *closure)
+{
+    PyObject *cx = ((FSMOb *)self_)->f_ctx;
+    (void)closure;
+    if (cx == NULL)
+        Py_RETURN_NONE;
+    Py_INCREF(cx);
+    return cx;
+}
+
 PyGetSetDef FSM_getset[] = {
     {(char *)"_fsm_state", FSM_get__fsm_state, NULL, NULL, NULL},
     {(char *)"_fsm_valid", FSM_get__fsm_valid, FSM_set__fsm_valid, NULL,
      NULL},
+    {(char *)"_claim_ctx", FSM_get__claim_ctx, NULL, NULL, NULL},
     {NULL, NULL, NULL, NULL, NULL},
 };
 
@@ -2397,36 +2462,64 @@
 extern PyObject *s_busy_st;
 PyObject *slotkit_conn_err_cb(PyObject *slot, PyObject *handle);
 
+struct NQueue;
+typedef struct {
+    PyObject_HEAD
+    struct NQueue *pc_idleq;
+    struct NQueue *pc_waiters;
+    struct NQueue *pc_initq;
+    PyObject *pc_counters;
+    PyObject *pc_dead;
+    PoolLatOb *pc_lat;
+    PyObject *pc_log;
+    int pc_no_codel;
+} PoolCtx;
+
+extern PyTypeObject PoolCtxType;
+PoolCtx *pool_ctx(PyObject *pool);
+PoolCtx *pool_ctx_private(PoolCtx *base, PoolLatOb *lat, PyObject *log);
+
 typedef struct {
     FSMOb base;
     PyObject *chb_pool;
     PyObject *chb_claim_stack;
     PyObject *chb_callback;
-    PyObject *chb_log;
     PyObject *chb_slot;
     PyObject *chb_release_stack;
     PyObject *chb_connection;
     PyObject *chb_last_error;
     PyObject *chb_waiter_node;
-    PoolLatOb *chb_lat;
+    PoolCtx *chb_ctx;
     double chb_claim_timeout;
     double chb_started;
     double chb_claimed_at;
-    long chb_pre[4];
-    int chb_have_pre;
-    int chb_throw_error;
-    int chb_cancelled;
-    int chb_leak_check;
-    int chb_pinger;
-    int chb_lat_open;
-    PyObject *chb_idleq, *chb_waiters, *chb_initq;
-    int chb_tk_on;
-    int chb_tk_err_on_empty;
+    int chb_pre[4];
+    unsigned char chb_have_pre;
+    unsigned char chb_throw_error;
+    unsigned char chb_cancelled;
+    unsigned char chb_leak_check;
+    unsigned char chb_pinger;
+    unsigned char chb_lat_open;
+    unsigned char chb_tk_on;
+    unsigned char chb_tk_err_on_empty;
     unsigned long chb_bk_serial;
     Py_ssize_t chb_bk_pos;
 } CHOb;
 
 extern PyTypeObject CHType;
+
+static inline PoolLatOb *
+ch_lat(CHOb *h)
+{
+    return h->chb_ctx != NULL ? h->chb_ctx->pc_lat : NULL;
+}
+
+static inline PyObject *
+ch_log(CHOb *h)
+{
+    return h->chb_ctx != NULL && h->chb_ctx->pc_log != NULL
+        ? h->chb_ctx->pc_log : Py_None;
+}
 
 long
 c_count_listeners(PyObject *emitter, PyObject *event)
@@ -2563,7 +2656,7 @@
         "connection emitted error while claimed");
     if (msg == NULL)
         return NULL;
-    PyObject *r = PyObject_CallMethodObjArgs(h->chb_log, s_warn, msg,
+    PyObject *r = PyObject_CallMethodObjArgs(ch_log(h), s_warn, msg,
                                              NULL);
     Py_DECREF(msg);
     if (r == NULL)
@@ -2920,7 +3013,7 @@
     Py_INCREF(t_claiming_valid);
     Py_XSETREF(self->base.f_valid, t_claiming_valid);
     PyObject *slot = self->chb_slot;
-    if (slot != NULL && PyObject_TypeCheck(slot, &SlotBaseType) &&
+    if (slot != NULL && is_slot(slot) &&
         ((FSMOb *)slot)->f_fastkit != NULL) {
         FSMOb *sf = (FSMOb *)slot;
         PyObject *fs = sf->f_state;
@@ -2960,12 +3053,12 @@
     }
 
     PyObject *conn = self->chb_connection;
-    int lk = emitter_leak_counts(conn, self->chb_pre);
+    long pre[4] = {0, 0, 0, 0};
+    int lk = emitter_leak_counts(conn, pre);
     if (lk == -1)
         return NULL;
-    if (lk == -2)
-        self->chb_pre[0] = self->chb_pre[1] = self->chb_pre[2] =
-            self->chb_pre[3] = 0;
+    for (int i = 0; i < 4; i++)
+        self->chb_pre[i] = lk == -2 ? 0 : (int)pre[i];
     self->chb_have_pre = 1;
 
     PyObject *ec = slotkit_conn_err_cb(self->chb_slot, self_);
@@ -2993,12 +3086,13 @@
         return NULL;
     Py_DECREF(r);
 
-    if (self->chb_lat != NULL && !self->chb_pinger) {
+    PoolLatOb *lat = ch_lat(self);
+    if (lat != NULL && !self->chb_pinger) {
         int err = 0;
-        double now = poollat_now_ms(self->chb_lat, &err);
+        double now = poollat_now_ms(lat, &err);
         if (err)
             return NULL;
-        self->chb_lat->pl_wait->h.record_ms(now - self->chb_started);
+        lat->pl_wait->h.record_ms(now - self->chb_started);
         self->chb_claimed_at = now;
         self->chb_lat_open = 1;
     }
@@ -3017,11 +3111,14 @@
     if (!self->chb_lat_open)
         return 0;
     self->chb_lat_open = 0;
+    PoolLatOb *lat = ch_lat(self);
+    if (lat == NULL)
+        return 0;
     int err = 0;
-    double now = poollat_now_ms(self->chb_lat, &err);
+    double now = poollat_now_ms(lat, &err);
     if (err)
         return -1;
-    self->chb_lat->pl_hold->h.record_ms(now - self->chb_claimed_at);
+    lat->pl_hold->h.record_ms(now - self->chb_claimed_at);
     return 0;
 }
 
@@ -3045,14 +3142,14 @@
         Py_RETURN_NONE;
     for (int i = 0; i < 4; i++) {
         long c = after[i];
-        if (c > self->chb_pre[i]) {
+        if (c > (long)self->chb_pre[i]) {
             PyObject *msg = PyUnicode_FromFormat(
                 "connection claimer looks like it leaked event handlers "
                 "(event=%S before=%ld after=%ld)",
-                s_leak_events[i], self->chb_pre[i], c);
+                s_leak_events[i], (long)self->chb_pre[i], c);
             if (msg == NULL)
                 return NULL;
-            PyObject *r = PyObject_CallMethodObjArgs(self->chb_log, s_warn,
+            PyObject *r = PyObject_CallMethodObjArgs(ch_log(self), s_warn,
                                                      msg, NULL);
             Py_DECREF(msg);
             if (r == NULL)
@@ -3190,16 +3287,12 @@
     Py_VISIT(self->chb_pool);
     Py_VISIT(self->chb_claim_stack);
     Py_VISIT(self->chb_callback);
-    Py_VISIT(self->chb_log);
     Py_VISIT(self->chb_slot);
     Py_VISIT(self->chb_release_stack);
     Py_VISIT(self->chb_connection);
     Py_VISIT(self->chb_last_error);
     Py_VISIT(self->chb_waiter_node);
-    Py_VISIT((PyObject *)self->chb_lat);
-    Py_VISIT(self->chb_idleq);
-    Py_VISIT(self->chb_waiters);
-    Py_VISIT(self->chb_initq);
+    Py_VISIT((PyObject *)self->chb_ctx);
     return FSM_traverse(self_, visit, arg);
 }
 
@@ -3210,16 +3303,12 @@
     Py_CLEAR(self->chb_pool);
     Py_CLEAR(self->chb_claim_stack);
     Py_CLEAR(self->chb_callback);
-    Py_CLEAR(self->chb_log);
     Py_CLEAR(self->chb_slot);
     Py_CLEAR(self->chb_release_stack);
     Py_CLEAR(self->chb_connection);
     Py_CLEAR(self->chb_last_error);
     Py_CLEAR(self->chb_waiter_node);
-    Py_CLEAR(self->chb_lat);
-    Py_CLEAR(self->chb_idleq);
-    Py_CLEAR(self->chb_waiters);
-    Py_CLEAR(self->chb_initq);
+    Py_CLEAR(self->chb_ctx);
     return FSM_clear_(self_);
 }
 
@@ -3247,7 +3336,6 @@
     Py_INCREF(args[0]); Py_XSETREF(self->chb_pool, args[0]);
     Py_INCREF(args[1]); Py_XSETREF(self->chb_claim_stack, args[1]);
     Py_INCREF(args[2]); Py_XSETREF(self->chb_callback, args[2]);
-    Py_INCREF(args[3]); Py_XSETREF(self->chb_log, args[3]);
     self->chb_claim_timeout = PyFloat_AsDouble(args[4]);
     if (self->chb_claim_timeout == -1.0 && PyErr_Occurred())
         return NULL;
@@ -3260,12 +3348,26 @@
     self->chb_pinger = 0;
     self->chb_have_pre = 0;
     self->chb_lat_open = 0;
-    PyObject *lat = NULL;
-    if (_PyObject_LookupAttr(args[0], s_p_lat, &lat) < 0)
-        return NULL;
-    if (lat != NULL && Py_TYPE(lat) != &PoolLatType)
-        Py_CLEAR(lat);
-    Py_XSETREF(self->chb_lat, (PoolLatOb *)lat);
+    PoolCtx *cx = pool_ctx(args[0]);
+    if (cx != NULL && cx->pc_log == args[3]) {
+        Py_INCREF((PyObject *)cx);
+    } else {
+        PyObject *lat = NULL;
+        if (cx != NULL) {
+            lat = (PyObject *)cx->pc_lat;
+            Py_XINCREF(lat);
+        } else {
+            if (_PyObject_LookupAttr(args[0], s_p_lat, &lat) < 0)
+                return NULL;
+            if (lat != NULL && Py_TYPE(lat) != &PoolLatType)
+                Py_CLEAR(lat);
+        }
+        cx = pool_ctx_private(cx, (PoolLatOb *)lat, args[3]);
+        Py_XDECREF(lat);
+        if (cx == NULL)
+            return NULL;
+    }
+    Py_XSETREF(self->chb_ctx, cx);
 
     PyObject *resolved = resolve_loop(args[6]);
     if (resolved == NULL)
@@ -3279,10 +3381,11 @@
     self->chb_bk_serial = 0;
     if (fsm_goto_state(&self->base, s_waiting) < 0)
         return NULL;
-    if (self->chb_lat != NULL && self->chb_lat->pl_direct &&
-        self->chb_lat->pl_loop == self->base.f_loop) {
+    PoolLatOb *plat = ch_lat(self);
+    if (plat != NULL && plat->pl_direct &&
+        plat->pl_loop == self->base.f_loop) {
         int err = 0;
-        self->chb_started = poollat_now_ms(self->chb_lat, &err);
+        self->chb_started = poollat_now_ms(plat, &err);
         if (err)
             return NULL;
         Py_RETURN_NONE;
@@ -3335,7 +3438,6 @@
      0, NULL},
     {(char *)"ch_callback", T_OBJECT, offsetof(CHOb, chb_callback), 0,
      NULL},
-    {(char *)"ch_log", T_OBJECT, offsetof(CHOb, chb_log), 0, NULL},
     {(char *)"ch_slot", T_OBJECT, offsetof(CHOb, chb_slot), 0, NULL},
     {(char *)"ch_release_stack", T_OBJECT,
      offsetof(CHOb, chb_release_stack), 0, NULL},
@@ -3348,17 +3450,27 @@
     {(char *)"ch_claim_timeout", T_DOUBLE,
      offsetof(CHOb, chb_claim_timeout), 0, NULL},
     {(char *)"ch_started", T_DOUBLE, offsetof(CHOb, chb_started), 0, NULL},
-    {(char *)"ch_cancelled", T_INT, offsetof(CHOb, chb_cancelled), 0,
+    {(char *)"ch_cancelled", T_UBYTE, offsetof(CHOb, chb_cancelled), 0,
      NULL},
-    {(char *)"ch_throw_error", T_INT, offsetof(CHOb, chb_throw_error), 0,
+    {(char *)"ch_throw_error", T_UBYTE, offsetof(CHOb, chb_throw_error), 0,
      NULL},
-    {(char *)"ch_do_release_leak_check", T_INT,
+    {(char *)"ch_do_release_leak_check", T_UBYTE,
      offsetof(CHOb, chb_leak_check), 0, NULL},
-    {(char *)"ch_pinger", T_INT, offsetof(CHOb, chb_pinger), 0, NULL},
+    {(char *)"ch_pinger", T_UBYTE, offsetof(CHOb, chb_pinger), 0, NULL},
     {NULL, 0, 0, 0, NULL},
 };
 
+PyObject *
+CH_get_log(PyObject *self_, void *closure)
+{
+    (void)closure;
+    PyObject *log = ch_log((CHOb *)self_);
+    Py_INCREF(log);
+    return log;
+}
+
 PyGetSetDef CH_getset[] = {
+    {(char *)"ch_log", CH_get_log, NULL, NULL, NULL},
     {(char *)"readable", CH_get_misused, NULL, NULL, NULL},
     {(char *)"writable", CH_get_misused, NULL, NULL, NULL},
     {NULL, NULL, NULL, NULL, NULL},
@@ -3426,8 +3538,15 @@
 ch_direct_entry(FSMOb *self, PyObject *target)
 {
     PyTypeObject *tp = Py_TYPE(self);
+#if CUEBALL_EXACT_TYPES
+    if (tp != g_handle_cls &&
+        (tp == g_slot_cls || tp == g_pool_cls ||
+         !PyType_IsSubtype(tp, &CHType)))
+        return NULL;
+#else
     if (!PyType_IsSubtype(tp, &CHType))
         return NULL;
+#endif
     for (int i = 0; i < ch_n_entries; i++) {
         ChEntry *e = &ch_entries[i];
         if (*e->ce_state != target)
@@ -3935,9 +4054,168 @@
 
 extern PyTypeObject CTType;
 
+
+PyObject *s_p_counters;
+extern PyObject *s_p_dead;
+extern PyObject *s_p_codel;
+extern PyObject *s_p_claim_log;
+
+static int
+PoolCtx_traverse(PyObject *self_, visitproc visit, void *arg)
+{
+    PoolCtx *cx = (PoolCtx *)self_;
+    Py_VISIT((PyObject *)cx->pc_idleq);
+    Py_VISIT((PyObject *)cx->pc_waiters);
+    Py_VISIT((PyObject *)cx->pc_initq);
+    Py_VISIT(cx->pc_counters);
+    Py_VISIT(cx->pc_dead);
+    Py_VISIT((PyObject *)cx->pc_lat);
+    Py_VISIT(cx->pc_log);
+    return 0;
+}
+
+static int
+PoolCtx_clear_(PyObject *self_)
+{
+    PoolCtx *cx = (PoolCtx *)self_;
+    Py_CLEAR(cx->pc_idleq);
+    Py_CLEAR(cx->pc_waiters);
+    Py_CLEAR(cx->pc_initq);
+    Py_CLEAR(cx->pc_counters);
+    Py_CLEAR(cx->pc_dead);
+    Py_CLEAR(cx->pc_lat);
+    Py_CLEAR(cx->pc_log);
+    return 0;
+}
+
+static void
+PoolCtx_dealloc(PyObject *self_)
+{
+    PyObject_GC_UnTrack(self_);
+    PoolCtx_clear_(self_);
+    PyObject_GC_Del(self_);
+}
+
+PyTypeObject PoolCtxType = {
+    PyVarObject_HEAD_INIT(NULL, 0)
+    "cueball_amd._speed._PoolCtx",
+    sizeof(PoolCtx),
+};
+
+static void
+poolctx_type_init(void)
+{
+    PoolCtxType.tp_dealloc = PoolCtx_dealloc;
+    PoolCtxType.tp_flags = Py_TPFLAGS_DEFAULT | Py_TPFLAGS_HAVE_GC;
+    PoolCtxType.tp_traverse = PoolCtx_traverse;
+    PoolCtxType.tp_clear = PoolCtx_clear_;
+}
+
+static PoolCtx *
+poolctx_alloc(void)
+{
+    PoolCtx *cx = PyObject_GC_New(PoolCtx, &PoolCtxType);
+    if (cx == NULL)
+        return NULL;
+    cx->pc_idleq = cx->pc_waiters = cx->pc_initq = NULL;
+    cx->pc_counters = cx->pc_dead = cx->pc_log = NULL;
+    cx->pc_lat = NULL;
+    cx->pc_no_codel = 0;
+    PyObject_GC_Track((PyObject *)cx);
+    return cx;
+}
+
+PoolCtx *
+pool_ctx_private(PoolCtx *base, PoolLatOb *lat, PyObject *log)
+{
+    PoolCtx *cx = poolctx_alloc();
+    if (cx == NULL)
+        return NULL;
+    if (base != NULL && base->pc_idleq != NULL) {
+        Py_INCREF((PyObject *)base->pc_idleq);
+        cx->pc_idleq = base->pc_idleq;
+        Py_INCREF((PyObject *)base->pc_waiters);
+        cx->pc_waiters = base->pc_waiters;
+        Py_INCREF((PyObject *)base->pc_initq);
+        cx->pc_initq = base->pc_initq;
+    }
+    Py_XINCREF((PyObject *)lat);
+    cx->pc_lat = lat;
+    Py_INCREF(log);
+    cx->pc_log = log;
+    return cx;
+}
+
+static PoolCtx *
+pool_ctx_make(FSMOb *pool)
+{
+    PyObject *names[8] = {s_p_idleq, s_p_waiters, s_p_initq, s_p_counters,
+                          s_p_dead, s_p_lat, s_p_claim_log, s_p_codel};
+    PyObject *v[8] = {NULL, NULL, NULL, NULL, NULL, NULL, NULL, NULL};
+    PoolCtx *cx = NULL;
+    int ok = 1;
+    for (int i = 0; i < 8 && ok; i++) {
+        if (_PyObject_LookupAttr((PyObject *)pool, names[i], &v[i]) < 0)
+            PyErr_Clear();
+        ok = v[i] != NULL;
+    }
+    if (ok && PyDict_Check(v[3]) && PyDict_Check(v[4]) &&
+        pool->f_ctx == NULL)
+        cx = poolctx_alloc();
+    if (cx != NULL) {
+        if (PyObject_TypeCheck(v[0], &NQueueType) &&
+            PyObject_TypeCheck(v[1], &NQueueType) &&
+            PyObject_TypeCheck(v[2], &NQueueType)) {
+            cx->pc_idleq = (NQueue *)v[0];
+            cx->pc_waiters = (NQueue *)v[1];
+            cx->pc_initq = (NQueue *)v[2];
+            v[0] = v[1] = v[2] = NULL;
+        }
+        cx->pc_counters = v[3];
+        cx->pc_dead = v[4];
+        v[3] = v[4] = NULL;
+        if (Py_TYPE(v[5]) == &PoolLatType) {
+            cx->pc_lat = (PoolLatOb *)v[5];
+            v[5] = NULL;
+        }
+        cx->pc_log = v[6];
+        v[6] = NULL;
+        cx->pc_no_codel = v[7] == Py_None;
+        pool->f_ctx = (PyObject *)cx;
+    } else if (PyErr_Occurred()) {
+        PyErr_Clear();
+    }
+    for (int i = 0; i < 8; i++)
+        Py_XDECREF(v[i]);
+    return (PoolCtx *)pool->f_ctx;
+}
+
+PoolCtx *
+pool_ctx(PyObject *pool)
+{
+    if (!is_fsm(pool))
+        return NULL;
+    PyObject *cx = ((FSMOb *)pool)->f_ctx;
+    if (cx != NULL)
+        return (PoolCtx *)cx;
+    return pool_ctx_make((FSMOb *)pool);
+}
+
 static void
 ct_bind_queues(TicketCore *t, PyObject *pool)
 {
+    PoolCtx *cx = pool_ctx(pool);
+    if (cx != NULL) {
+        if (cx->pc_idleq != NULL) {
+            Py_INCREF((PyObject *)cx->pc_idleq);
+            t->ct_idleq = cx->pc_idleq;
+            Py_INCREF((PyObject *)cx->pc_waiters);
+            t->ct_waiters = cx->pc_waiters;
+            Py_INCREF((PyObject *)cx->pc_initq);
+            t->ct_initq = cx->pc_initq;
+        }
+        return;
+    }
     PyObject *iq = PyObject_GetAttr(pool, s_p_idleq);
     PyObject *wq = iq ? PyObject_GetAttr(pool, s_p_waiters) : NULL;
     PyObject *nq = wq ? PyObject_GetAttr(pool, s_p_initq) : NULL;
@@ -4017,7 +4295,6 @@
     return 0;
 }
 
-PyObject *s_p_counters;
 PyObject *s_p_rebal_scheduled;
 PyObject *s_max_claim_queue;
 PyObject *s_queued_claim;
@@ -4033,7 +4310,14 @@
     if (ct_note_demand(t) < 0)
         return -1;
 
-    PyObject *counters = PyObject_GetAttr(t->ct_pool, s_p_counters);
+    PoolCtx *cx = pool_ctx(t->ct_pool);
+    PyObject *counters;
+    if (cx != NULL) {
+        counters = cx->pc_counters;
+        Py_INCREF(counters);
+    } else {
+        counters = PyObject_GetAttr(t->ct_pool, s_p_counters);
+    }
     if (counters == NULL)
         return -1;
     if (!PyDict_Check(counters)) {
@@ -4139,14 +4423,14 @@
         Py_DECREF((PyObject *)n);
         if (fsm == NULL)
             continue;
-        if (PyObject_TypeCheck(fsm, &SlotBaseType)) {
+        if (is_slot(fsm)) {
             slot_field_store(&((SlotOb *)fsm)->sl_idleq_node, Py_None);
         } else if (PyObject_SetAttr(fsm, s_p_idleq_node, Py_None) < 0) {
             Py_DECREF(fsm);
             return -1;
         }
         int isidle;
-        if (PyObject_TypeCheck(fsm, &FSMType)) {
+        if (is_fsm(fsm)) {
             PyObject *fs = ((FSMOb *)fsm)->f_state;
             isidle = (fs == s_idle ||
                       (fs != NULL &&
@@ -4180,12 +4464,16 @@
 static int
 ch_ticket_try_next(CHOb *h)
 {
-    TicketCore v = {h->chb_pool, (PyObject *)h, (NQueue *)h->chb_idleq,
-                    (NQueue *)h->chb_waiters, (NQueue *)h->chb_initq,
-                    h->chb_tk_err_on_empty};
+    PoolCtx *cx = h->chb_ctx;
+    if (cx == NULL)
+        return 0;
+    TicketCore v = {h->chb_pool, (PyObject *)h, cx->pc_idleq,
+                    cx->pc_waiters, cx->pc_initq, h->chb_tk_err_on_empty};
     PyObject *pool = v.ct_pool;
     Py_INCREF(pool);
+    Py_INCREF((PyObject *)cx);
     int r = ct_try_next(&v);
+    Py_DECREF((PyObject *)cx);
     Py_DECREF(pool);
     return r;
 }
@@ -4248,11 +4536,11 @@
     (void)kwds;
     if (!PyArg_ParseTuple(args, "OOO", &pool, &handle, &err_on_empty))
         return NULL;
-    if (!PyObject_TypeCheck(pool, &FSMType)) {
+    if (!is_fsm(pool)) {
         PyErr_SetString(PyExc_TypeError, "pool must be a native FSM");
         return NULL;
     }
-    if (!PyObject_TypeCheck(handle, &CHType)) {
+    if (!is_handle(handle)) {
         PyErr_SetString(PyExc_TypeError,
                         "handle must be a ClaimHandleBase");
         return NULL;
@@ -4293,11 +4581,18 @@
         return NULL;
     }
     PyObject *pool = args[1];
-    if (!PyObject_TypeCheck(pool, &FSMType)) {
+    if (!is_fsm(pool)) {
         PyErr_SetString(PyExc_TypeError, "pool must be a native FSM");
         return NULL;
     }
-    PyObject *counters = PyObject_GetAttr(pool, s_p_counters);
+    PoolCtx *cx = pool_ctx(pool);
+    PyObject *counters;
+    if (cx != NULL) {
+        counters = cx->pc_counters;
+        Py_INCREF(counters);
+    } else {
+        counters = PyObject_GetAttr(pool, s_p_counters);
+    }
     if (counters == NULL)
         return NULL;
     if (PyDict_Check(counters)) {
@@ -4367,7 +4662,7 @@
         return NULL;
     }
     PyObject *pool = args[1];
-    if (!PyObject_TypeCheck(pool, &FSMType)) {
+    if (!is_fsm(pool)) {
         PyErr_SetString(PyExc_TypeError, "pool must be a native FSM");
         return NULL;
     }
@@ -4390,11 +4685,13 @@
 #if CUEBALL_HANDLE_HOOKS
     {
         CHOb *h = (CHOb *)handle;
-        TicketCore q = {NULL, NULL, NULL, NULL, NULL, 0};
-        ct_bind_queues(&q, pool);
-        Py_XSETREF(h->chb_idleq, (PyObject *)q.ct_idleq);
-        Py_XSETREF(h->chb_waiters, (PyObject *)q.ct_waiters);
-        Py_XSETREF(h->chb_initq, (PyObject *)q.ct_initq);
+        if (pool_ctx(pool) == NULL) {
+            TicketCore q = {NULL, NULL, NULL, NULL, NULL, 0};
+            ct_bind_queues(&q, pool);
+            Py_XSETREF(h->chb_ctx->pc_idleq, q.ct_idleq);
+            Py_XSETREF(h->chb_ctx->pc_waiters, q.ct_waiters);
+            Py_XSETREF(h->chb_ctx->pc_initq, q.ct_initq);
+        }
         h->chb_tk_err_on_empty = err_on_empty;
         h->chb_tk_on = 1;
     }
@@ -4523,7 +4820,7 @@
 PyObject *
 slotkit_conn_err_cb(PyObject *slot, PyObject *handle)
 {
-    if (slot == NULL || !PyObject_TypeCheck(slot, &SlotBaseType))
+    if (slot == NULL || !is_slot(slot))
         return NULL;
     PyObject *kit = ((FSMOb *)slot)->f_fastkit;
     if (kit == NULL || Py_TYPE(kit) != &SlotKitType ||
@@ -4633,7 +4930,7 @@
         break;
     case KCB_CONN_ERR: {
         PyObject *hdl = ((SlotOb *)k->k_slot)->sl_handle;
-        if (hdl == NULL || !PyObject_TypeCheck(hdl, &CHType))
+        if (hdl == NULL || !is_handle(hdl))
             break;
         Py_INCREF(hdl);
         PyObject *res = conn_err_fire((CHOb *)hdl,
@@ -4721,7 +5018,7 @@
 #endif
     int armed = 0;
 #if CUEBALL_HANDLE_HOOKS
-    if (PyObject_TypeCheck(hdl, &CHType)) {
+    if (is_handle(hdl)) {
         CHOb *h = (CHOb *)hdl;
         PyObject *ls = h->base.base.ev_events == NULL ? NULL :
             PyDict_GetItemWithError(h->base.base.ev_events, s_stateChanged);
@@ -4883,7 +5180,7 @@
 {
     PyObject *slot = h->chb_slot;
     if (h->chb_bk_serial == 0 || slot == NULL ||
-        !PyObject_TypeCheck(slot, &SlotBaseType))
+        !is_slot(slot))
         return 0;
     PyObject *kit_ = ((FSMOb *)slot)->f_fastkit;
     if (kit_ == NULL || Py_TYPE(kit_) != &SlotKitType)
@@ -5343,7 +5640,7 @@
             PyObject *hdl = so->sl_handle;
             int pinger = 0;
             if (hdl != NULL && hdl != Py_None &&
-                PyObject_TypeCheck(hdl, &CHType))
+                is_handle(hdl))
                 pinger = ((CHOb *)hdl)->chb_pinger;
             if (!pinger)
                 Py_RETURN_NONE;
@@ -5357,7 +5654,14 @@
         (st == s_idle ||
          (PyUnicode_Check(st) &&
           PyUnicode_Compare(st, s_idle) == 0))) {
-        PyObject *dead = PyObject_GetAttr(d->sd_pool, s_p_dead);
+        PoolCtx *cx = pool_ctx(d->sd_pool);
+        PyObject *dead;
+        if (cx != NULL) {
+            dead = cx->pc_dead;
+            Py_INCREF(dead);
+        } else {
+            dead = PyObject_GetAttr(d->sd_pool, s_p_dead);
+        }
         if (dead == NULL)
             return NULL;
         int isdead = PyDict_Check(dead) ?
@@ -5419,7 +5723,7 @@
             PyObject *hdl = nqueue_shift_value(d->sd_waiters);
             if (hdl == NULL)
                 return NULL;
-            if (!PyObject_TypeCheck(hdl, &CHType)) {
+            if (!is_handle(hdl)) {
                 Py_DECREF(hdl);
                 continue;
             }
@@ -5531,7 +5835,7 @@
     if (!PyArg_ParseTuple(args, "OOOO", &pool, &fsm, &key, &has_codel))
         return NULL;
     if (!PyObject_TypeCheck(pool, &EmitterType) ||
-        !PyObject_TypeCheck(fsm, &SlotBaseType)) {
+        !is_slot(fsm)) {
         PyErr_SetString(PyExc_TypeError,
                         "SlotDispatch(pool, slot, key, has_codel)");
         return NULL;
@@ -5624,8 +5928,8 @@
     (void)kwds;
     if (!PyArg_ParseTuple(args, "OO", &slot, &smgr))
         return NULL;
-    if (!PyObject_TypeCheck(slot, &SlotBaseType) ||
-        !PyObject_TypeCheck(smgr, &FSMType)) {
+    if (!is_slot(slot) ||
+        !is_fsm(smgr)) {
         PyErr_SetString(PyExc_TypeError,
                         "SlotKit(slot, smgr): a SlotBase and a native "
                         "FSM required");
@@ -5733,12 +6037,23 @@
         if (cb != Py_None &&
             (opt == Py_None ||
              (PyDict_CheckExact(opt) && PyDict_GET_SIZE(opt) == 0)) &&
-            PyObject_TypeCheck(pool, &FSMType)) {
+            is_fsm(pool)) {
             PyObject *pst = ((FSMOb *)pool)->f_state;
             int open = pst != NULL &&
                 (pst == s_running_st ||
                  PyUnicode_Compare(pst, s_running_st) == 0 ||
                  PyUnicode_CompareWithASCIIString(pst, "starting") == 0);
+            PoolCtx *cx = open ? pool_ctx(pool) : NULL;
+            if (cx != NULL) {
+                if (cx->pc_no_codel) {
+                    PyObject *pargs[5] = {cm->cm_handle_cls, pool, cb,
+                                          cx->pc_log,
+                                          ((FSMOb *)pool)->f_loop};
+                    return speed_pool_claim(NULL, pargs, 5);
+                }
+                return PyObject_Vectorcall(cm->cm_func, args, nargsf,
+                                           kwnames);
+            }
             PyObject *codel = open ? PyObject_GetAttr(pool, s_p_codel)
                                    : NULL;
             if (open && codel == NULL)
@@ -5865,6 +6180,42 @@
     PyObject_GC_Track((PyObject *)cm);
     return (PyObject *)cm;
 #endif
+}
+
+static PyObject *
+speed_set_cycle_classes(PyObject *mod, PyObject *const *args,
+                        Py_ssize_t nargs)
+{
+    (void)mod;
+    if (nargs != 3) {
+        PyErr_SetString(PyExc_TypeError,
+                        "_set_cycle_classes(handle_cls, slot_cls, pool_cls)");
+        return NULL;
+    }
+    PyTypeObject *bases[3] = {&CHType, &SlotBaseType, &FSMType};
+    PyTypeObject **dst[3] = {&g_handle_cls, &g_slot_cls, &g_pool_cls};
+    for (int i = 0; i < 3; i++) {
+        if (args[i] == Py_None)
+            continue;
+        PyTypeObject *cls = (PyTypeObject *)args[i];
+        if (!PyType_Check(args[i]) || !PyType_IsSubtype(cls, bases[i]) ||
+            (i > 0 && PyType_IsSubtype(cls, &CHType)) ||
+            (i == 2 && PyType_IsSubtype(cls, &SlotBaseType))) {
+            PyErr_SetString(PyExc_TypeError,
+                "_set_cycle_classes: a ClaimHandleBase, a SlotBase and a "
+                "plain FSM subclass required");
+            return NULL;
+        }
+    }
+    for (int i = 0; i < 3; i++) {
+        if (args[i] == Py_None)
+            continue;
+        Py_INCREF(args[i]);
+        PyTypeObject *old = *dst[i];
+        *dst[i] = (PyTypeObject *)args[i];
+        Py_XDECREF((PyObject *)old);
+    }
+    Py_RETURN_NONE;
 }
 
 PyObject *
@@ -5899,6 +6250,9 @@
      METH_FASTCALL, NULL},
     {"claim_method", (PyCFunction)(void (*)(void))speed_claim_method,
      METH_FASTCALL, NULL},
+    {"_set_cycle_classes",
+     (PyCFunction)(void (*)(void))speed_set_cycle_classes, METH_FASTCALL,
+     NULL},
     {NULL, NULL, 0, NULL},
 };
 
@@ -5995,6 +6349,7 @@
     s_rebalance = PyUnicode_InternFromString("rebalance");
     s_set_unwanted = PyUnicode_InternFromString("set_unwanted");
     queue_types_init();
+    poolctx_type_init();
     ct_type_init();
     slotkit_types_init();
     codel_type_init();
@@ -6019,6 +6374,7 @@
         PyType_Ready(&SlotBaseType) < 0 ||
         PyType_Ready(&QNodeType) < 0 ||
         PyType_Ready(&NQueueType) < 0 ||
+        PyType_Ready(&PoolCtxType) < 0 ||
         PyType_Ready(&CTType) < 0 ||
         PyType_Ready(&KitCbType) < 0 ||
         PyType_Ready(&SlotKitType) < 0 ||
diff --git a/cueball_amd/connection_fsm.py b/cueball_amd/connection_fsm.py
--- a/cueball_amd/connection_fsm.py
+++ b/cueball_amd/connection_fsm.py
@@ -883,6 +883,10 @@
             raise FSMError("smgr must be stopped")
 
 
+if _native_count is not None:
+    _speed_mod._set_cycle_classes(ClaimHandle, ConnectionSlotFSM, None)
+
+
 def _do_ping_check(fsm: ConnectionSlotFSM, checker: Callable) -> None:
 
     def ping_check_adapter(err: Optional[BaseException], hdl: ClaimHandle,
diff --git a/cueball_amd/pool.py b/cueball_amd/pool.py
--- a/cueball_amd/pool.py
+++ b/cueball_amd/pool.py
@@ -1501,3 +1501,5 @@
     from ._speed import claim_method as _claim_method
     ConnectionPool.claim = _claim_method(
         ConnectionPool.__dict__["claim"], ClaimHandle)
+    from ._speed import _set_cycle_classes
+    _set_cycle_classes(None, None, ConnectionPool)
```

Measured after the change: 888,200 claims/s (median of 6 runs). +9.5%, better.
